# shgaurav1/DVG

Hardware: AMD Instinct MI355X
Metric: predicted frames/sec at 64x64, batch 64, 10-in/10-out (higher is better)
Workload: dtype f32; 1 GPU; Moving-MNIST 64x64 rollout (generate_frames.py make_gifs sample loop), vgg_64 + lstm + GP trigger sample at i%15==0, batch 64 per GPU, 10-in/10-out; model_family=vgg, batch_per_gpu=64, n_past=10, n_future=10, parallelism=replicas x1 (no data-path collective), launch=hipGraph replay, rollouts_in_flight=3, tile_policy=energy, loop_invariant_skip_halves=hoisted, upsample_conv3x3=as transposed 4x4/s2 conv, conv3x3_deep_layers=Winograd F(4x4,3x3) / F(2x2,3x3)

## Files before the change

dvg_amd/_lib.py:

```python
from __future__ import annotations

import ctypes as C
import os
import threading

_HERE = os.path.dirname(os.path.abspath(__file__))
LIB_PATH = os.environ.get("DVG_HIP_LIB") or os.path.join(_HERE, "csrc", "libdvg_hip.so")

_p = C.c_void_p
_i = C.c_int
_f = C.c_float
_d = C.c_double
_l = C.c_long

SIGNATURES = {
    "dvg_abi_version": (_i, []),
    "dvg_last_error": (C.c_char_p, []),
    "dvg_stream_capture_id": (_l, [_p]),
    "dvg_mfma_mode": (_i, []),
    "dvg_build_info": (C.c_char_p, []),
    "dvg_set_tile_policy": (None, [_i]),
    "dvg_tile_policy": (_i, []),
    "dvg_packed_row_floats": (_i, []),
    "dvg_pack_conv_weight": (_i, [_p, _p, _i, _i, _i, _i, _p]),
    "dvg_pack_convT_weight": (_i, [_p, _p, _i, _i, _i, _i, _p]),
    "dvg_unpack_conv_weight": (_i, [_p, _p, _i, _i, _i, _i, _p]),
    "dvg_unpack_convT_weight": (_i, [_p, _p, _i, _i, _i, _i, _p]),
    "dvg_conv_first_stats_rows": (_i, [_i, _i, _i, _i]),
    "dvg_pack_conv_weight_k16": (_i, [_p, _p, _i, _i, _i, _i, _i, _p]),
    "dvg_conv_splitk_v2": (_i, [_i, _i, _i, _i, _i, _i]),
    "dvg_conv_stats_rows_v2": (_i, [_i, _i, _i, _i, _i, _i, _i, _i]),
    "dvg_conv3x3_bn_act_v2": (_i, [_p, _p, _p, _p, _p, _p, _p, _p, _i, _i, _i, _i, _i, _i, _i, _i, _f, _p, _l, _p, _p, _i, _p]),
    "dvg_conv3x3_first_pair": (_i, [_p, _p, _p, _p, _p, _p, _p, _p, _p, _i, _i, _i, _i, _i, _f, _i, _p]),
    "dvg_conv4x4s2_bn_act_v2": (_i, [_p, _p, _p, _p, _p, _p, _i, _i, _i, _i, _i, _i, _f, _p, _l, _p]),
    "dvg_convT4x4s2_bn_act_v2": (_i, [_p, _p, _p, _p, _p, _p, _p, _i, _i, _i, _i, _i, _i, _i, _f, _p, _l, _p, _p, _i, _p]),
    "dvg_winograd_weight": (_i, [_p, _p, _i, _i, _i, _p]),
    "dvg_winograd_input": (_i, [_p, _p, _i, _i, _i, _i, _i, _i, _p]),
    "dvg_gemm_batched_k16": (_i, [_p, _p, _p, _i, _i, _i, _i, _i, _p]),
    "dvg_winograd_output": (_i, [_p, _p, _p, _p, _p, _i, _i, _i, _i, _i, _f, _i, _p, _i, _p]),
    "dvg_winograd_output_input": (_i, [_p, _p, _p, _p, _i, _i, _i, _i, _i, _f, _p, _p]),
    "dvg_stem_up_winograd_input": (_i, [_p, _i, _p, _i, _p, _p, _p, _i, _i, _i, _i, _f, _p]),
    "dvg_winograd_output_up_input": (_i, [_p, _p, _p, _p, _i, _i, _i, _i, _i, _f, _p]),
    "dvg_winograd_output_pool_input": (_i, [_p, _p, _p, _p, _p, _i, _i, _i, _i, _i, _f, _i, _p]),
    "dvg_conv3x3_first": (_i, [_p, _p, _p, _p, _p, _p, _i, _i, _i, _i, _i, _i, _f, _p]),
    "dvg_convT3x3_last": (_i, [_p, _p, _p, _p, _i, _i, _i, _i, _i, _i, _p]),
    "dvg_conv4x4s2_first": (_i, [_p, _p, _p, _p, _p, _p, _i, _i, _i, _i, _i, _i, _f, _p]),
    "dvg_convT4x4s2_last": (_i, [_p, _p, _p, _p, _p, _i, _i, _i, _i, _i, _i, _i, _p]),
    "dvg_moving_mnist_compose": (_i, [_p, _p, _p, _p, _i, _i, _i, _i, _i, _i, _p]),
    "dvg_clip_gather_u8": (_i, [_p, _p, _p, _l, _i, _i, _i, _i, _i, _i, _p]),
    "dvg_clip_gather_aug_u8": (_i, [_p, _p, _p, _p, _p, _l, _i, _i, _i, _i, _i, _i, _p]),
    "dvg_mnist_scale_u8": (_i, [_p, _p, _i, _i, _i, _p, _p, _p]),
    "dvg_moving_mnist_compose_u8": (_i, [_p, _p, _p, _p, _i, _i, _i, _i, _i, _i, _p]),
    "dvg_eval_frames": (_i, [_p, _p, _p, _p, _i, _i, _i, _p]),
    "dvg_eval_frames_finn": (_i, [_p, _p, _p, _p, _p, _i, _i, _i, _i, _p]),
    "dvg_pairwise_frame_mse": (_i, [_p, _p, _i, _l, _i, _l, _i, _p]),
    "dvg_frame_mosaic": (_i, [_p, _l, _p, _l, _p, _l, _i, _i, _i, _p] + [_i] * 9 + [_p, _i, _p, _i, _i, _p, _i, _i, _i, _i, _p, _p]),
    "dvg_adam_step": (_i, [_p, _p, _p, _p, _l, _f, _f, _f, _f, _f, _i, _p, _p]),
    "dvg_pixel_proj": (_i, [_p, _p, _p, _l, _i, _i, _p]),
    "dvg_convT_gather": (_i, [_p, _p, _p, _p, _i, _i, _i, _i, _i, _i, _p, _i, _p]),
    "dvg_channel_stats_rows": (_i, [_l]),
    "dvg_channel_stats": (_i, [_p, _p, _l, _i, _i, _p]),
    "dvg_bn_finalize": (_i, [_p, _i, _p, _p, _p, _p, _p, _p, _p, _p, _i, _d, _f, _f, _p, _i, _i, _p, _p]),
    "dvg_channel_stats_pivot": (_i, [_p, _p, _p, _l, _i, _i, _p]),
    "dvg_bn_finalize_pivot": (_i, [_p, _i, _p, _p, _p, _p, _p, _p, _p, _p, _p, _i, _d, _f, _f, _p, _i, _i, _p, _p]),
    "dvg_bn_running_update": (_i, [_p, _p, _i, _i, _f, _f, _f, _p, _p, _p, _i, _p]),
    "dvg_bn_act_apply": (_i, [_p, _p, _p, _p, _p, _i, _i, _i, _i, _i, _f, _i, _p]),
    "dvg_gemm_nt_bias_act": (_i, [_p, _p, _p, _p, _p, _p, _i, _i, _i, _i, _i, _i, _i, _i, _f, _i, _p]),
    "dvg_lstm_cell": (_i, [_p, _p, _p, _p, _p, _p, _p, _p, _p, _p, _i, _i, _p]),
    "dvg_lstm_cell_pre": (_i, [_p, _p, _p, _p, _p, _p, _p, _i, _i, _p]),
    "dvg_lstm_cell_bwd": (_i, [_p, _p, _p, _p, _p, _p, _p, _p, _p, _p, _i, _i, _p]),
    "dvg_lstm_cell_x": (_i, [_p, _i, _i, _p, _p, _p, _i, _p, _p, _p, _p, _i, _i, _p]),
    "dvg_gru_cell": (_i, [_p, _p, _p, _p, _p, _p, _p, _p, _i, _i, _p]),
    "dvg_gru_cell_pre": (_i, [_p, _p, _p, _p, _p, _p, _i, _i, _p]),
    "dvg_rnn_cell": (_i, [_p, _p, _p, _p, _p, _p, _p, _i, _i, _p]),
    "dvg_gru_gates_bwd": (_i, [_p, _p, _p, _p, _p, _p, _p, _i, _i, _p]),
    "dvg_stem_gemm": (_i, [_p, _i, _p, _i, _p, _p, _p, _i, _i, _i, _i, _i, _i, _f, _p]),
    "dvg_gp_precision": (_i, [_i, _i, _i]),
    "dvg_gp_bwd_precision": (_i, [_i, _i]),
    "dvg_gp_lds_bytes": (C.c_size_t, [_i, _i, _i]),
    "dvg_gp_predict": (_i, [_p] * 14 + [_i, _i, _i, _i, _f, _i, _i, _p]),
    "dvg_gp_step_group": (_i, [_i, _i, _i, _i]),
    "dvg_gp_bwd_lds_bytes": (C.c_size_t, [_i, _i]),
    "dvg_gp_bwd_chunk": (_i, [_i, _i]),
    "dvg_gemm_tn": (_i, [_p] * 5 + [_i] * 8 + [_p]),
    "dvg_gp_train_bwd": (_i, [_p] * 17 + [_i, _i, _i, _f, _i, _i, _p]),
    "dvg_sum_steps_multi": (_i, [_p, _p, _p, _i, _i, _p]),
    "dvg_gp_elbo": (_i, [_p, _p, _p, _p, _l, _l, _p, _p, _i, _i, _i, _i, _p]),
    "dvg_gp_elbo_bwd": (_i, [_p, _p, _p, _p, _l, _l, _p, _p, _p, _p, _p, _p, _p, _i, _i, _i, _i, _p]),
    "dvg_bn_act_bwd_rows": (_i, [_i, _i, _i, _i]),
    "dvg_bn_act_bwd_reduce": (_i, [_p, _p, _p, _p, _p, _p, _i, _i, _i, _i, _i, _f, _i, _p]),
    "dvg_bn_bwd_finalize": (_i, [_p, _i, _p, _p, _p, _p, _p, _p, _p, _p, _p, _i, _d, _i, _i, _i, _p]),
    "dvg_bn_act_bwd_reduce_centered": (_i, [_p, _p, _p, _p, _p, _p, _p, _i, _i, _i, _i, _i, _f, _i, _p]),
    "dvg_bn_bwd_finalize_centered": (_i, [_p, _i, _p, _p, _p, _p, _p, _p, _p, _p, _p, _i, _d, _i, _i, _i, _p]),
    "dvg_affine3_apply": (_i, [_p, _p, _p, _p, _p, _p, _l, _i, _p, _i, _i, _p]),
    "dvg_act_bwd": (_i, [_p, _p, _p, _l, _i, _f, _p]),
    "dvg_upsample2x_bwd": (_i, [_p, _p, _i, _i, _i, _i, _p]),
    "dvg_group_sum": (_i, [_p, _p, _p, _i, _i, _l, _p]),
    "dvg_colsum": (_i, [_p, _p, _i, _i, _i, _p]),
    "dvg_wgrad_finish": (_i, [_p, _i, _p, _i, _i, _i, _i, _i, _i, _i, _f, _p]),
    "dvg_k4_to_w3": (_i, [_p, _p, _i, _i, _i, _i, _f, _p]),
    "dvg_reduce_partials": (_i, [_p, _p, _i, _l, _p]),
    "dvg_conv_wgrad_splits": (_i, [_i, _i, _i, _i, _i, _i]),
    "dvg_conv_wgrad": (_i, [_i, _p, _p, _p, _p, _i, _i, _i, _i, _i, _i, _i, _p]),
    "dvg_conv_wgrad_splits_multi": (_i, [_i, _i, _i, _i, _i, _i, _i]),
    "dvg_conv_wgrad_multi": (_i, [_i, _i, _p, _p, _p, _p, _i, _i, _i, _i, _i, _i, _i, _p]),
    "dvg_winograd_wgrad_operands": (_i, [_p, _p, _p, _p, _i, _i, _i, _i, _i, _l, _l, _p]),
    "dvg_winograd_wgrad_splits": (_i, [_l, _i, _i]),
    "dvg_winograd_wgrad_gemm": (_i, [_p, _p, _p, _l, _i, _i, _p]),
    "dvg_winograd_wgrad_gemm_items": (_i, [_p, _p, _i, _l, _p, _i, _i, _p]),
    "dvg_winograd_wgrad_reduce": (_i, [_p, _i, _p, _i, _i, _p]),
    "dvg_wgrad_thin_rows": (_i, [_i, _i, _i, _i]),
    "dvg_wgrad_thin": (_i, [_p, _p, _p, _i, _i, _i, _i, _i, _i, _p]),
    "dvg_lstm_gates_bwd": (_i, [_p, _p, _p, _p, _p, _p, _p, _i, _i, _p]),
    "dvg_nchw_to_nhwc": (_i, [_p, _p, _i, _i, _i, _i, _p]),
    "dvg_nhwc_to_nchw": (_i, [_p, _p, _i, _i, _i, _i, _p]),
    "dvg_zero_tick": (_i, [_p, _l, _p, _p, _p, _p, _p]),
    "dvg_grad_sumsq_blocks": (_i, [_l]),
    "dvg_grad_sumsq": (_i, [_p, _l, _p, _p]),
    "dvg_grad_guard_finish": (_i, [_p, _i, _d, _i, _p, _p, _p]),
    "dvg_adam_step_guarded": (_i, [_p, _p, _p, _p, _l, _f, _f, _f, _f, _f, _i, _p, _p, _p, _p]),
    "dvg_ema_update_blocks": (_i, [_l]),
    "dvg_ema_update": (_i, [_p, _p, _l, _d, _p, _p, _p]),
    "dvg_lr_schedule_tick": (_i, [_i, _i, _i, _i, _d, _d, _p, _p, _p]),
    "dvg_adam_step_scheduled": (_i, [_p, _p, _p, _p, _l, _f, _f, _f, _f, _f, _i, _p, _p, _p, _p, _p]),
    "dvg_val_accumulate": (_i, [_p, _p, _p, _i, _i, _i, _p, _p, _p, _p]),
    "dvg_frame_losses_blocks": (_i, [_l]),
    "dvg_frame_losses": (_i, [_p, _p, _p, _p, _l, _i, _i, _p, _p, _p]),
    "dvg_mse_sum_grad": (_i, [_p, _p, _p, _p, _l, _f, _p]),
    "dvg_frame_losses_ext_blocks": (_i, [_i, _l, _i, _i]),
    "dvg_frame_losses_ext": (_i, [_p, _p, _p, _p, _i, _i, _l, _i, _i, _i, _f, _p, _p, _p, _p]),
    "dvg_gp_var_norms": (_i, [_p, _p, _i, _i, _p]),
    "dvg_gp_trigger_step": (_i, [_p, _i, _i, _i, _p, _i, _f, _p, _p, _p, _p, _i, _p]),
    "dvg_gp_trigger_replay": (_i, [_p, _i, _p, _i, _f, _p, _p, _p]),
    "dvg_gp_trigger_select": (_i, [_p, _p, _p, _p, _i, _i, _i, _l, _p, _p, _p, _p]),
    "dvg_debug_set_clockbuf": (None, [_p, C.c_uint]),
    "dvg_debug_set_gp_clockbuf": (None, [_p, C.c_uint]),
    "dvg_debug_set_wgrad_clockbuf": (None, [_p, C.c_uint]),
}

_lock = threading.Lock()
_lib = None


class DvgLibraryError(RuntimeError):
    pass


def lib() -> C.CDLL:
    global _lib
    if _lib is not None:
        return _lib
    with _lock:
        if _lib is not None:
            return _lib
        if not os.path.exists(LIB_PATH):
            raise DvgLibraryError(
                f"{LIB_PATH} not found: the HIP kernel library has not been built. "
                "Run `python -c 'import __graft_entry__ as g; g.build()'` (or `make -C dvg_amd/csrc`). "
                "There is no CPU/eager fallback for the DVG hot path.")
        try:
            import torch
            if torch.cuda.is_available():
                torch.cuda.init()
        except ImportError:
            pass
        try:
            handle = C.CDLL(LIB_PATH)
        except OSError as e:
            raise DvgLibraryError(f"cannot load {LIB_PATH}: {e}") from e
        for name, (res, args) in SIGNATURES.items():
            try:
                fn = getattr(handle, name)
            except AttributeError as e:
                raise DvgLibraryError(f"{LIB_PATH} lacks symbol {name}; rebuild it") from e
            fn.restype = res
            fn.argtypes = args
        _lib = handle
        return _lib


def build_info() -> dict:
    raw = lib().dvg_build_info().decode()
    d = {}
    for tok in raw.split():
        k, _, v = tok.partition("=")
        d[k] = int(v) if v.lstrip("-").isdigit() else v
    d["raw"] = raw
    d["path"] = LIB_PATH
    d["from_env"] = bool(os.environ.get("DVG_HIP_LIB"))
    shipped = {os.path.join(_HERE, "csrc", "libdvg_hip.so"), os.path.join(_HERE, "csrc", "libdvg_hip_f32mfma.so")}
    d["product"] = os.path.abspath(LIB_PATH) in shipped and d.get("variant", "") == ""
    return d


def check(code: int, what: str = "") -> None:
    if code != 0:
        msg = lib().dvg_last_error()
        raise RuntimeError(f"libdvg_hip {what} failed (code {code}): {msg.decode() if msg else '?'}")
```

dvg_amd/csrc/conv_igemm2.hip:

```cpp
#include <cstdlib>
#include <type_traits>

#include "dvg_common.h"

namespace dvg {

constexpr int DVG_GEMM_WGS_PER_CU = DVG_BF16X3 ? 3 : 4;
constexpr int DVG_GEMM128_WGS = DVG_BF16X3 ? 3 : 2;
constexpr int DVG_GEMM128_GT = DVG_BF16X3 ? 2 : 4;
constexpr int DVG_GEMM_GT = 4;
constexpr int DVG_GEMM128_MIN_WGS = 4 * 768;
[[maybe_unused]] constexpr int DVG_GEMM_NT2 = 256;
constexpr int DVG_TILE16_MIN_WGS = 256;

enum { M2_CONV3 = 0, M2_CONV4S2 = 1, M2_CONVT4S2 = 2, M2_GEMM = 3 };

struct Igemm2Params {
    const float* x;
    const float* skip;
    const float* w;
    const float* scale;
    const float* shift;
    float* y;
    float* y_pool;
    float* stats;
    int N, H, W, C1, C2, Cout, upsample, act;
    float slope;
    int tiles_y, tiles_x, tiles_n, nblk_n;
    int splitk;
    int cps;
    float* ws;
    const float* addend;
    unsigned long long* clk;
    unsigned clk_cap;
    int nb_group;
    int stage_prio;
    long w_image_stride;
    int gemm_ni;
    const int* add_map;
    int add_B;
    const float* first_frame;
    const float* first_w;
    const float* first_scale;
    const float* first_shift;
    float first_slope;
    int y_from;
};

__device__ __forceinline__ int addend_image(const int* __restrict__ add_map, int add_B, int n) {
    return add_map ? add_map[n / add_B] * add_B + n % add_B : n;
}

static unsigned long long* g_clk = nullptr;
static unsigned g_clk_cap = 0;

__device__ __attribute__((aligned(16))) float dvg_zero_slot[4] = {0.f, 0.f, 0.f, 0.f};

template <int MODE, int TI, int TH, int TW, int NT_ = 1, bool FIRST_ = false>
struct Cfg2 {
    static constexpr int NT = NT_;
    static constexpr bool FIRST = FIRST_;
    static constexpr bool GEMM = MODE == M2_GEMM;
    static constexpr int S = (MODE == M2_CONV4S2) ? 2 : 1;
    static constexpr bool PAR4 = MODE == M2_CONV4S2;
    static constexpr int SPAN = GEMM ? 1 : (PAR4 ? 2 : 3);
    static constexpr int HH = (TH - 1) + SPAN, HW = (TW - 1) + SPAN;
    static constexpr bool LAYOUT = !GEMM;
    static constexpr int HWP = !LAYOUT ? HW : (TW == 16 ? HW : (TW == 8 ? 12 : 6));
    static constexpr int IMG = (LAYOUT && TI == 4) ? (PAR4 ? 30 : 40) : HH * HWP;
    static_assert(IMG >= HH * HWP && HWP >= HW, "halo layout");
    static constexpr int HP = TI * IMG;
    static constexpr unsigned P0PACK = !LAYOUT ? 0x6420u
        : (PAR4 ? (TW == 16 ? 0x3650u : (TI == 4 ? 0x7430u : 0x6530u))
                : (TW == 16 ? 0x2640u : (TI == 4 ? 0x6530u : 0x4620u)));
    static constexpr int PK = !LAYOUT ? 1 : (PAR4 ? (TW == 16 ? 4 : 1) : (TW == 16 ? 5 : (TI == 4 ? 1 : 3)));
    static constexpr bool STORE_PERM = LAYOUT && DVG_BF16X3 != 0;
    static constexpr int hp_of(int slot) {
        return STORE_PERM ? ((slot & ~7) | (((slot & 3) << 1) | ((slot >> 2) & 1))) : slot;
    }
    static constexpr int row_c(int reg) { return 4 * (int)((P0PACK >> (4 * (reg >> 2))) & 15u) + (reg & 3); }
    static constexpr int BM = TI * TH * TW, MT = BM / 64, BN = 64 * NT;
    static constexpr int NTAPS = GEMM ? 1 : ((MODE == M2_CONV3) ? 9 : 16);
    static constexpr int GT = (MODE == M2_CONV3) ? 9 : (MODE == M2_CONV4S2 ? 4 : (GEMM ? (NT == 2 ? 2 : (BM == 128 ? DVG_GEMM128_GT : DVG_GEMM_GT)) : 4));
    static constexpr int NG = (MODE == M2_CONV4S2) ? 16 / GT : 1;
    static constexpr int CHUNKS_PER_STAGE = GEMM ? GT : 1;
    static constexpr bool X3 = DVG_BF16X3 != 0;
    static constexpr int KC = 16, LD = X3 ? (GEMM ? 24 : 28) : 20, LDB = X3 ? 24 : 20, WROW = DVG_WROW;
    static constexpr int NP = X3 ? 3 : 2, PSTEP = X3 ? 8 : 4;
    static constexpr int BLK4 = GT * 64 * WROW / 4;
    static constexpr int B_TILE4 = NT * BLK4;
    static constexpr int NLB = (B_TILE4 + 255) / 256;
    static_assert(NT == 1 || (DVG_BF16X3 != 0 && MODE == M2_GEMM && BLK4 % 256 == 0), "NT = 2: bf16-triple GEMM mode only");
    static constexpr int NLA1 = (HP * 4 + 255) / 256;
    static constexpr int NLA = NLA1 * (GEMM ? GT : 1);
    static constexpr int SLAB = NLA1 * 64 * LD;
    static constexpr int A_FLOATS = NLA * 64 * LD, B_FLOATS = GT * BN * LDB;
    static constexpr int FP_W = HW + 2, FP_FLOATS = (HH + 2) * FP_W, FIRST_FLOATS = FIRST ? FP_FLOATS : 0;
    static_assert(!FIRST || (MODE == M2_CONV3 && TI == 1 && NT == 1), "FIRST: 3x3 mode, one image per tile");
    static constexpr int LDS_BYTES = (A_FLOATS + B_FLOATS + FIRST_FLOATS) * 4;
    static constexpr bool CAN_SPLIT = !FIRST && !GEMM && TW != 16;
    static_assert(BM == 64 || BM == 128 || BM == 256, "BM");
};

template <int MODE, int TI, int TH, int TW, int NT = 1, bool FIRST = false>
__global__ __launch_bounds__(256, (MODE == M2_GEMM && TW == 8) ? DVG_GEMM_WGS_PER_CU : ((MODE == M2_GEMM && NT == 1) ? DVG_GEMM128_WGS : 2)) void conv_igemm2_kernel(const Igemm2Params p) {
    using C = Cfg2<MODE, TI, TH, TW, NT, FIRST>;
    constexpr int S = C::S, HH = C::HH, HW = C::HW, HP = C::HP, LD = C::LD, MT = C::MT, GT = C::GT, NG = C::NG,
                  BN = C::BN, NLA = C::NLA, NLA1 = C::NLA1, LDB = C::LDB, NP = C::NP, PSTEP = C::PSTEP, NLB = C::NLB;
    constexpr bool GEMM = C::GEMM, X3 = C::X3;
    extern __shared__ __attribute__((aligned(16))) float smem[];
    float* As = smem;
    float* Bs = smem + C::A_FLOATS;

    const int tid = threadIdx.x, lane = tid & 63, wave = tid >> 6;
    const int wm = wave >> 1, wn = wave & 1, l31 = lane & 31, hh = lane >> 5;

    unsigned lid = xcd_remap(blockIdx.x, gridDim.x);
    int par = 0;
    if (MODE == M2_CONVT4S2) { par = lid & 3; lid >>= 2; }
    const int split = lid % p.splitk;
    lid /= p.splitk;
    const int tiles_total = p.tiles_x * p.tiles_y * p.tiles_n;
    const unsigned lr = lid / p.nb_group;
    const int nb = (int)(lr / tiles_total) * p.nb_group + (int)(lid % p.nb_group);
    const unsigned tile_id = lr % tiles_total;
    unsigned t = tile_id;
    const int tx_i = t % p.tiles_x; t /= p.tiles_x;
    const int ty_i = t % p.tiles_y; t /= p.tiles_y;
    const int n0 = (int)t * (MODE == M2_GEMM ? p.gemm_ni : TI), y0 = ty_i * TH, x0 = tx_i * TW;
    const int yin0 = y0 * S - (GEMM ? 0 : 1), xin0 = x0 * S - (GEMM ? 0 : 1), nb0 = nb * BN;
    const float* const wbase = p.w + (GEMM ? (size_t)n0 * p.w_image_stride : 0);
    const int py = par >> 1, px = par & 1;
    const int Cin = p.C1 + p.C2;

    int a_base[MT];
#pragma unroll
    for (int mt = 0; mt < MT; ++mt) {
        const int lp = 4 * ((int)((C::P0PACK >> (4 * (l31 >> 3))) & 15u) ^ (((l31 >> 2) & 1) * C::PK)) + (l31 & 3);
        const int m = wm * (C::BM / 2) + mt * 32 + lp;
        const int ti = m / (TH * TW), r = m % (TH * TW);
        const int pos = ti * C::IMG + (r / TW) * C::HWP + r % TW;
        a_base[mt] = pos * LD + (X3 ? (hh ^ (GEMM ? (pos >> 3) & 1 : 0)) * 4 : hh * 8);
    }
    int b_base[NT];
#pragma unroll
    for (int nt = 0; nt < NT; ++nt) {
        const int col = (wn * NT + nt) * 32 + l31;
        b_base[nt] = ((col >> 6) * GT * 64 + (col & 63)) * LDB + (X3 ? (hh ^ ((l31 >> 3) & 1)) * 4 : hh * 8);
    }

    f32x16 acc[MT * NT];
#pragma unroll
    for (int mt = 0; mt < MT * NT; ++mt)
#pragma unroll
        for (int i = 0; i < 16; ++i) acc[mt][i] = 0.f;

    constexpr int NOFF = GEMM ? NLA1 : NLA;
    using aoff_t = typename std::conditional<GEMM || C::PAR4, int, long>::type;
    auto opaque = [](unsigned v) { asm("" : "+v"(v)); return v; };
    aoff_t offx[NOFF], offs[GEMM ? 1 : NLA];
    unsigned okmask = 0;
    static_assert(!C::PAR4 || NLA <= 4, "PAR4: four validity bits and two step bits per halo slot in one word");
    if (GEMM) offs[0] = 0;
#pragma unroll
    for (int i = 0; i < NLA; ++i) {
        const int idx = tid + (i % NLA1) * 256;
        const int hp = C::hp_of(idx >> 2), q = idx & 3;
        const int ti = hp / C::IMG, r = hp % C::IMG;
        const int hy = r / C::HWP, hx = r % C::HWP;
        const bool slot = hp < HP && hy < HH && hx < HW;
        if constexpr (C::PAR4) {
            const int n = n0 + ti, yy = yin0 + 2 * hy, xx = xin0 + 2 * hx;
            const bool in = slot && n < p.N;
#pragma unroll
            for (int par_ = 0; par_ < 4; ++par_) {
                const bool ok = in && (unsigned)(yy + (par_ >> 1)) < (unsigned)p.H && (unsigned)(xx + (par_ & 1)) < (unsigned)p.W;
                okmask |= ok ? (1u << (par_ * NLA + i)) : 0u;
            }
            const int cy0 = min(max(yy, 0), p.H - 1), cy1 = min(max(yy + 1, 0), p.H - 1);
            const int cx0 = min(max(xx, 0), p.W - 1), cx1 = min(max(xx + 1, 0), p.W - 1);
            okmask |= (in && cy1 != cy0) ? (1u << (16 + i)) : 0u;
            okmask |= (in && cx1 != cx0) ? (1u << (24 + i)) : 0u;
            offx[i] = in ? (int)((((long)n * p.H + cy0) * p.W + cx0) * p.C1 + q * 4) : 0;
            offs[i] = 0;
        } else {
        const int n = n0 + ti, yy = yin0 + hy, xx = xin0 + hx;
        const bool ok = slot && n < p.N && (unsigned)yy < (unsigned)p.H && (unsigned)xx < (unsigned)p.W;
        const int sh = p.upsample;
        okmask |= ok ? (1u << i) : 0u;
        if (!GEMM || i < NLA1)
            offx[GEMM ? i % NLA1 : i] = (aoff_t)(ok ? ((((long)(GEMM ? 0 : n) * (p.H >> sh) + (yy >> sh)) * (p.W >> sh) + (xx >> sh)) * p.C1 + q * 4) : 0);
        if (!GEMM) offs[i] = (ok && p.C2) ? ((((long)n * p.H + yy) * p.W + xx) * p.C2 + q * 4) : 0;
        }
    }
    auto tap_lds = [&](int grp, int tt) -> int {
        if (GEMM) return tt * C::SLAB;
        int th, tw;
        if (MODE == M2_CONV3) { th = tt / 3; tw = tt % 3; }
        else if (MODE == M2_CONV4S2) { th = tt >> 1; tw = tt & 1; }
        else { th = 1 + py - (tt >> 1); tw = 1 + px - (tt & 1); }
        return (th * C::HWP + tw) * LD;
    };
    long ld_a_off = GEMM ? (long)n0 * p.H * p.W * p.C1 : 0;
    const float* ld_w = wbase;
    float* const Fp = smem + C::A_FLOATS + C::B_FLOATS;
    f32x4 fw[FIRST ? 11 : 1];
    auto first_tile = [&](f32x4 (&ra)[NLA]) {
        if constexpr (FIRST) {
#pragma unroll
            for (int i = 0; i < NLA; ++i) {
                const int hp = min(C::hp_of((tid + i * 256) >> 2), HP - 1);
                const float* f = Fp + (hp / C::HWP) * C::FP_W + hp % C::HWP;
                f32x4 v = {0.f, 0.f, 0.f, 0.f};
#pragma unroll
                for (int t = 0; t < 9; ++t) {
                    const float px = f[(t / 3) * C::FP_W + t % 3];
#pragma unroll
                    for (int e = 0; e < 4; ++e) v[e] = fmaf(fw[t][e], px, v[e]);
                }
                const float okf = (float)((okmask >> i) & 1u);
#pragma unroll
                for (int e = 0; e < 4; ++e) {
                    const float a = v[e] * fw[9][e] + fw[10][e];
                    v[e] = fmaxf(a, a * p.first_slope) * okf;
                }
                ra[i] = v;
            }
        }
    };
    auto gload_a = [&](int c0, f32x4 (&ra)[NLA], const int par_ = 0) {
        if constexpr (FIRST) {
            const float* w = p.first_w + c0 + (tid & 3) * 4;
#pragma unroll
            for (int t = 0; t < 9; ++t) fw[t] = *reinterpret_cast<const f32x4*>(w + t * 64);
            fw[9] = *reinterpret_cast<const f32x4*>(p.first_scale + c0 + (tid & 3) * 4);
            fw[10] = *reinterpret_cast<const f32x4*>(p.first_shift + c0 + (tid & 3) * 4);
            return;
        }
        const bool from_x = GEMM || c0 < p.C1;
        const float* src = (from_x ? p.x + c0 : p.skip + (c0 - p.C1)) + (GEMM ? ld_a_off : 0);
#pragma unroll
        for (int i = 0; i < NLA; ++i) {
            if (GEMM) {
                ra[i] = *reinterpret_cast<const f32x4*>(src + offx[i % NLA1] + (i / NLA1) * 16);
            } else if (C::PAR4) {
                int off = offx[i];
                if (par_ >> 1) off += (int)opaque((okmask >> (16 + i)) & 1u) * (p.W * p.C1);
                if (par_ & 1) off += (int)opaque((okmask >> (24 + i)) & 1u) * p.C1;
                ra[i] = *reinterpret_cast<const f32x4*>(src + off);
            } else {
                const float* a = src + (from_x ? offx[GEMM ? 0 : i] : offs[GEMM ? 0 : i]);
                ra[i] = *reinterpret_cast<const f32x4*>(((okmask >> i) & 1u) ? a : dvg_zero_slot);
            }
        }
    };
    auto gload_b = [&](int chunk, int grp, f32x4 (&rb)[NLB]) {
        const float* tile;
        if (GEMM) tile = ld_w + ((size_t)nb * NT * (Cin / C::KC) + chunk) * (64 * C::WROW);
        else tile = wbase + (((size_t)chunk * (p.Cout >> 6) + nb) * C::NTAPS + (MODE == M2_CONVT4S2 ? par * 4 : grp * GT)) * (64 * C::WROW);
#pragma unroll
        for (int j = 0; j < NLB; ++j) {
            int i = tid + j * 256;
            if (C::B_TILE4 % 256) i = min(i, C::B_TILE4 - 1);
            const size_t blk = (NT > 1 && j * 256 >= C::BLK4) ? (size_t)(Cin / C::KC) * (64 * C::WROW / 4) - C::BLK4 : 0;
            rb[j] = reinterpret_cast<const f32x4*>(tile)[i + blk];
        }
    };
    auto lds_store_a = [&](f32x4 (&ra)[NLA], const int par_ = 0) {
        if constexpr (FIRST) first_tile(ra);
#pragma unroll
        for (int i = 0; i < NLA; ++i) {
            const int idx = tid + (i % NLA1) * 256;
            const int hp = C::hp_of(idx >> 2), q = idx & 3;
            if constexpr (C::PAR4) {
                const unsigned keep = 0u - opaque((okmask >> (par_ * NLA + i)) & 1u);
#pragma unroll
                for (int e = 0; e < 4; ++e) {
                    const float f = ra[i][e];
                    ra[i][e] = __builtin_bit_cast(float, __builtin_bit_cast(unsigned, f) & keep);
                }
            }
            if constexpr (X3) {
                u32x2_t h, m, l;
                unsigned t0, t1, t2;
                bf16x3_split_pair(ra[i][0], ra[i][1], t0, t1, t2);
                h[0] = t0; m[0] = t1; l[0] = t2;
                bf16x3_split_pair(ra[i][2], ra[i][3], t0, t1, t2);
                h[1] = t0; m[1] = t1; l[1] = t2;
                float* d = &As[(i / NLA1) * C::SLAB + hp * LD + ((q >> 1) ^ (GEMM ? (hp >> 3) & 1 : 0)) * 4 + (q & 1) * 2];
                *reinterpret_cast<u32x2_t*>(d) = h;
                *reinterpret_cast<u32x2_t*>(d + 8) = m;
                *reinterpret_cast<u32x2_t*>(d + 16) = l;
            } else {
                *reinterpret_cast<f32x4*>(&As[(i / NLA1) * C::SLAB + hp * LD + q * 4]) = ra[i];
            }
        }
    };
    auto lds_store_b = [&](const f32x4 (&rb)[NLB]) {
#pragma unroll
        for (int j = 0; j < NLB; ++j) {
            int i = tid + j * 256;
            if (C::B_TILE4 % 256) i = min(i, C::B_TILE4 - 1);
            if constexpr (X3) reinterpret_cast<f32x4*>(Bs)[i] = rb[j];
            else *reinterpret_cast<f32x4*>(&Bs[(i >> 2) * LDB + (i & 3) * 4]) = rb[j];
        }
    };

    constexpr int CPS = C::CHUNKS_PER_STAGE;
    const int chunk_begin = split * p.cps;
    const int chunk_end = min(Cin / C::KC, chunk_begin + p.cps);
    f32x4 ra[NLA], rb[NLB];
    unsigned long long clk0 = 0, wclk0 = 0;
    if (p.clk) {
        clk0 = clock64();
        wclk0 = wall_clock64();
    }
    if constexpr (FIRST) {
        const float* fr = p.first_frame + (size_t)n0 * p.H * p.W;
        for (int i = tid; i < C::FP_FLOATS; i += 256) {
            const int yy = yin0 - 1 + i / C::FP_W, xx = xin0 - 1 + i % C::FP_W;
            Fp[i] = ((unsigned)yy < (unsigned)p.H && (unsigned)xx < (unsigned)p.W) ? fr[(size_t)yy * p.W + xx] : 0.f;
        }
        __syncthreads();
    }
    gload_a(chunk_begin * C::KC, ra);
    gload_b(chunk_begin, 0, rb);
    lds_store_a(ra);
    lds_store_b(rb);
    __syncthreads();
    unsigned long long clk1 = 0;
    if (p.clk) clk1 = clock64();

    auto stage = [&](const int chunk, auto grp_c, auto has_next_c, const int nchunk_override = -1) __attribute__((always_inline)) {
        constexpr int grp = decltype(grp_c)::value;
        constexpr bool has_next = decltype(has_next_c)::value;
        constexpr int ngrp = (grp + 1) % NG;
        constexpr bool next_a = has_next && (ngrp == 0 || C::PAR4);
        const int nchunk = nchunk_override >= 0 ? nchunk_override : chunk + (ngrp == 0 ? CPS : 0);
        if constexpr (next_a) gload_a(nchunk * C::KC, ra, C::PAR4 ? ngrp : 0);
        if constexpr (has_next) gload_b(nchunk, ngrp, rb);

        f32x4 fa[2][MT][NP], fb[2][NT][NP];
        {
            const int ao = tap_lds(grp, 0);
#pragma unroll
            for (int j = 0; j < NP; ++j) {
#pragma unroll
                for (int mt = 0; mt < MT; ++mt)
                    fa[0][mt][j] = *reinterpret_cast<const f32x4*>(&As[a_base[mt] + ao + j * PSTEP]);
#pragma unroll
                for (int nt = 0; nt < NT; ++nt)
                    fb[0][nt][j] = *reinterpret_cast<const f32x4*>(&Bs[b_base[nt] + j * PSTEP]);
            }
        }
#pragma unroll
        for (int tt = 0; tt < GT; ++tt) {
            const int cur = tt & 1, nxt = cur ^ 1;
            constexpr bool LEAN = X3 && (NT == 2 || (GEMM && MT == 2));
            auto read_plane = [&](int j) {
                const int ao = tap_lds(grp, tt + 1);
#pragma unroll
                for (int mt = 0; mt < MT; ++mt)
                    fa[nxt][mt][j] = *reinterpret_cast<const f32x4*>(&As[a_base[mt] + ao + j * PSTEP]);
#pragma unroll
                for (int nt = 0; nt < NT; ++nt)
                    fb[nxt][nt][j] = *reinterpret_cast<const f32x4*>(&Bs[b_base[nt] + (tt + 1) * 64 * LDB + j * PSTEP]);
            };
            if (LEAN && tt + 1 < GT) read_plane(0);
            if (!LEAN && tt + 1 < GT) {
                const int ao = tap_lds(grp, tt + 1);
#pragma unroll
                for (int j = 0; j < NP; ++j) {
#pragma unroll
                    for (int mt = 0; mt < MT; ++mt)
                        fa[nxt][mt][j] = *reinterpret_cast<const f32x4*>(&As[a_base[mt] + ao + j * PSTEP]);
#pragma unroll
                    for (int nt = 0; nt < NT; ++nt)
                        fb[nxt][nt][j] = *reinterpret_cast<const f32x4*>(&Bs[b_base[nt] + (tt + 1) * 64 * LDB + j * PSTEP]);
                }
            }
            if (has_next && tt == GT - 1) {
                __syncthreads();
                if constexpr (next_a) lds_store_a(ra, C::PAR4 ? ngrp : 0);
                lds_store_b(rb);
            }
            if constexpr (X3) {
                auto mm = [&](int pa, int pb) {
#pragma unroll
                    for (int mt = 0; mt < MT; ++mt)
#pragma unroll
                        for (int nt = 0; nt < NT; ++nt)
                            acc[mt * NT + nt] = __builtin_amdgcn_mfma_f32_32x32x16_bf16(
                                __builtin_bit_cast(bf16x8_t, fa[cur][mt][pa]), __builtin_bit_cast(bf16x8_t, fb[cur][nt][pb]),
                                acc[mt * NT + nt], 0, 0, 0);
                };
                if constexpr (LEAN) {
                    mm(2, 0);
                    mm(0, 2);
                    if (tt + 1 < GT) read_plane(2);
                    mm(1, 1);
                    mm(1, 0);
                    mm(0, 1);
                    if (tt + 1 < GT) read_plane(1);
                    mm(0, 0);
                } else {
                    mm(2, 0);
                    mm(1, 1);
                    mm(0, 2);
                    mm(1, 0);
                    mm(0, 1);
                    mm(0, 0);
                }
            } else {
#pragma unroll
                for (int j = 0; j < 2; ++j)
#pragma unroll
                    for (int e = 0; e < 4; ++e)
#pragma unroll
                        for (int mt = 0; mt < MT; ++mt)
                            acc[mt] = __builtin_amdgcn_mfma_f32_32x32x2f32(fa[cur][mt][j][e], fb[cur][0][j][e], acc[mt], 0, 0, 0);
            }
            constexpr int NREAD = NP * (MT + NT), NMFMA = (X3 ? 6 : 8) * MT * NT, MPR = NMFMA >= 2 * NREAD ? 2 : 1;
            constexpr int NVMEM = (next_a ? (FIRST ? 11 : NLA) : 0) + (has_next ? NLB : 0);
            constexpr int VT0 = GT >= 9 ? 2 : 0;
            constexpr int SLOTS = (GT - 1 - VT0) > 0 ? (GT - 1 - VT0) : 1;
            constexpr int VNEED = (NVMEM + SLOTS - 1) / SLOTS;
            constexpr int VPT = VNEED > 2 ? VNEED : 2;
            constexpr int VTAPS = (NVMEM + VPT - 1) / VPT;
            if (tt == 0) __builtin_amdgcn_sched_group_barrier(0x100, NREAD, 0);
            if (LEAN && tt + 1 < GT) {
                constexpr int G = MT * NT, R = MT + NT;
#pragma unroll
                for (int r = 0; r < R; ++r) {
                    __builtin_amdgcn_sched_group_barrier(0x100, 1, 0);
                    __builtin_amdgcn_sched_group_barrier(0x008, 1, 0);
                }
                __builtin_amdgcn_sched_group_barrier(0x008, 2 * G - R, 0);
#pragma unroll
                for (int r = 0; r < R; ++r) {
                    __builtin_amdgcn_sched_group_barrier(0x100, 1, 0);
                    __builtin_amdgcn_sched_group_barrier(0x008, 1, 0);
                }
                __builtin_amdgcn_sched_group_barrier(0x008, 3 * G - R, 0);
#pragma unroll
                for (int r = 0; r < R; ++r) {
                    __builtin_amdgcn_sched_group_barrier(0x100, 1, 0);
                    __builtin_amdgcn_sched_group_barrier(0x008, 1, 0);
                }
            } else if (tt + 1 < GT) {
#pragma unroll
                for (int r = 0; r < NREAD; ++r) {
                    __builtin_amdgcn_sched_group_barrier(0x100, 1, 0);
                    __builtin_amdgcn_sched_group_barrier(0x008, MPR, 0);
                }
                if (NMFMA > MPR * NREAD) __builtin_amdgcn_sched_group_barrier(0x008, NMFMA - MPR * NREAD, 0);
            } else if (has_next) {
                constexpr int NW = (next_a ? NLA * (X3 ? 3 : 1) : 0) + NLB;
#pragma unroll
                for (int r = 0; r < NW; ++r) {
                    if (r < NMFMA) __builtin_amdgcn_sched_group_barrier(0x008, 1, 0);
                    __builtin_amdgcn_sched_group_barrier(0x200, 1, 0);
                }
                if (NMFMA > NW) __builtin_amdgcn_sched_group_barrier(0x008, NMFMA - NW, 0);
            } else {
                __builtin_amdgcn_sched_group_barrier(0x008, NMFMA, 0);
            }
            if (tt >= VT0 && tt < VT0 + VTAPS && tt + 1 < GT) __builtin_amdgcn_sched_group_barrier(0x020, VPT, 0);
        }

        if constexpr (has_next) __syncthreads();
    };
    using std::integral_constant;
    const bool prio_on = p.stage_prio != 0;
    auto set_prio = [&](int st) {
        if (!prio_on) return;
        switch (st & 3) {
            case 0: __builtin_amdgcn_s_setprio(3); break;
            case 1: __builtin_amdgcn_s_setprio(2); break;
            case 2: __builtin_amdgcn_s_setprio(1); break;
            default: __builtin_amdgcn_s_setprio(0); break;
        }
    };
    int chunk = chunk_begin, st = 0;
    if constexpr (GEMM) {
        const int spi = (chunk_end - chunk_begin) / CPS;
        const long a_img = (long)p.H * p.W * p.C1;
        const unsigned lane_off = (unsigned)(4 * hh * p.Cout + l31);
        float* const ybase = p.y + (size_t)n0 * p.H * p.W * p.Cout + nb0 + __builtin_amdgcn_readfirstlane(wn) * 32 * NT;
        const int wm_u = __builtin_amdgcn_readfirstlane(wm);
        for (int img = 0; img < p.gemm_ni; ++img) {
            for (int sg = 0; sg < spi; ++sg) {
                const bool wrap = sg == spi - 1, last = wrap && img == p.gemm_ni - 1;
                ld_a_off = (long)(n0 + img + (wrap ? 1 : 0)) * a_img;
                ld_w = wbase + (size_t)(img + (wrap ? 1 : 0)) * p.w_image_stride;
                const int nchunk = wrap ? chunk_begin : chunk_begin + (sg + 1) * CPS;
                set_prio(st++);
                if (last) stage(chunk_begin + sg * CPS, integral_constant<int, 0>{}, integral_constant<bool, false>{});
                else stage(chunk_begin + sg * CPS, integral_constant<int, 0>{}, integral_constant<bool, true>{}, nchunk);
            }
            float* const yb = ybase + (size_t)img * p.H * p.W * p.Cout;
#pragma unroll
            for (int mt = 0; mt < MT; ++mt) {
                const int mbase = wm_u * (C::BM / 2) + mt * 32;
#pragma unroll
                for (int nt = 0; nt < NT; ++nt)
#pragma unroll
                    for (int reg = 0; reg < 16; ++reg) {
                        const int mu = mbase + (reg & 3) + 8 * (reg >> 2);
                        float* const dst = (yb + (size_t)((y0 + mu / TW) * p.W + x0 + mu % TW) * p.Cout + nt * 32) + lane_off;
                        *dst = acc[mt * NT + nt][reg];
                        acc[mt * NT + nt][reg] = 0.f;
                    }
            }
        }
    } else {
    auto chunk_stages = [&](const int ch, auto last_c) __attribute__((always_inline)) {
        constexpr bool last = decltype(last_c)::value;
        set_prio(st++);
        stage(ch, integral_constant<int, 0>{}, integral_constant<bool, !(last && NG == 1)>{});
        if constexpr (NG >= 2) {
            set_prio(st++);
            stage(ch, integral_constant<int, 1>{}, integral_constant<bool, !(last && NG == 2)>{});
        }
        if constexpr (NG >= 4) {
            set_prio(st++);
            stage(ch, integral_constant<int, 2>{}, integral_constant<bool, true>{});
            set_prio(st++);
            stage(ch, integral_constant<int, 3>{}, integral_constant<bool, !last>{});
        }
        static_assert(NG == 1 || NG == 2 || NG == 4, "stages per chunk");
    };
    for (; chunk + CPS < chunk_end; chunk += CPS) chunk_stages(chunk, integral_constant<bool, false>{});
    chunk_stages(chunk, integral_constant<bool, true>{});
    }
    __builtin_amdgcn_s_setprio(0);
    unsigned long long clk_loop = 0;
    if (p.clk) clk_loop = clock64();
    auto clk_exit = [&]() {
        if (p.clk && threadIdx.x == 0 && blockIdx.x < p.clk_cap) {
            unsigned long long* d = p.clk + (size_t)blockIdx.x * 8;
            d[0] = clk0; d[1] = clk1; d[2] = clk_loop; d[3] = clock64(); d[4] = wclk0; d[5] = wall_clock64();
            unsigned xcc;
            asm volatile("s_getreg_b32 %0, hwreg(HW_REG_XCC_ID)" : "=s"(xcc));
            unsigned hwid;
            asm volatile("s_getreg_b32 %0, hwreg(HW_REG_HW_ID)" : "=s"(hwid));
            d[6] = xcc; d[7] = hwid;
        }
    };

    if constexpr (GEMM) {
        clk_exit();
        return;
    }
    int Ho, Wo;
    if (MODE == M2_CONV3 || MODE == M2_GEMM) { Ho = p.H; Wo = p.W; }
    else if (MODE == M2_CONV4S2) { Ho = p.H >> 1; Wo = p.W >> 1; }
    else { Ho = p.H * 2; Wo = p.W * 2; }
    const int c = nb0 + wn * 32 + l31;
    if (C::CAN_SPLIT && p.splitk > 1) {
        const size_t slab = (size_t)p.N * Ho * Wo * p.Cout;
        float* const wsp = p.ws + (size_t)split * slab;
#pragma unroll
        for (int mt = 0; mt < MT; ++mt)
#pragma unroll
            for (int reg = 0; reg < 16; ++reg) {
                const int m = wm * (C::BM / 2) + mt * 32 + (C::row_c(reg) ^ (hh * 4 * C::PK));
                const int tii = m / (TH * TW), r = m % (TH * TW);
                const int ty = r / TW, tx = r % TW;
                const int n = n0 + tii;
                int oy, ox;
                if (MODE == M2_CONVT4S2) { oy = 2 * (y0 + ty) + py; ox = 2 * (x0 + tx) + px; }
                else { oy = y0 + ty; ox = x0 + tx; }
                if (n < p.N) wsp[(((size_t)n * Ho + oy) * Wo + ox) * p.Cout + c] = acc[mt][reg];
            }
        clk_exit();
        return;
    }
    const float sc = p.scale ? p.scale[c] : 1.f, sf = p.shift ? p.shift[c] : 0.f;
    float s1 = 0.f, s2 = 0.f;
    float* const yb = p.y + (size_t)n0 * Ho * Wo * p.Cout + c;
    const bool want_y = !FIRST || n0 >= p.y_from;
    float* const pb = p.y_pool ? p.y_pool + (size_t)n0 * (Ho >> 1) * (Wo >> 1) * p.Cout + c : nullptr;
    const float* const ab = p.addend ? p.addend + (size_t)n0 * Ho * Wo * p.Cout + c : nullptr;
    long add_shift[TI];
#pragma unroll
    for (int t_ = 0; t_ < TI; ++t_) {
        const int n_ = min(n0 + t_, p.N - 1);
        add_shift[t_] = (ab != nullptr && p.add_map != nullptr)
                            ? (long)(addend_image(p.add_map, p.add_B, n_) - n_) * Ho * Wo * p.Cout : 0;
    }
    auto shift_of = [&](int tii) -> long {
        if (TI == 1) return add_shift[0];
        long v = add_shift[0];
#pragma unroll
        for (int t_ = 1; t_ < TI; ++t_) v = tii == t_ ? add_shift[t_] : v;
        return v;
    };
    const int hrow = hh * 4 * C::PK;
    auto epilogue = [&](auto act_c) {
        constexpr int ACT = decltype(act_c)::value;
#pragma unroll
        for (int mt = 0; mt < MT; ++mt) {
            float v[16];
            const int mbase = wm * (C::BM / 2) + mt * 32;
            const int ti0 = mbase / (TH * TW);
            if (ab != nullptr) {
                float av[16];
#pragma unroll
                for (int reg = 0; reg < 16; ++reg) {
                    const int m = mbase + (C::row_c(reg) ^ hrow);
                    const int tii = (TH * TW >= 32) ? ti0 : m / (TH * TW);
                    const int r = m % (TH * TW);
                    const int ty = r / TW, tx = r % TW;
                    int oy, ox;
                    if (MODE == M2_CONVT4S2) { oy = 2 * (y0 + ty) + py; ox = 2 * (x0 + tx) + px; }
                    else { oy = y0 + ty; ox = x0 + tx; }
                    av[reg] = (TI == 1 || n0 + tii < p.N) ? ab[(long)((tii * Ho + oy) * Wo + ox) * p.Cout + shift_of(tii)] : 0.f;
                }
#pragma unroll
                for (int reg = 0; reg < 16; ++reg) v[reg] = (acc[mt][reg] + av[reg]) * sc + sf;
            } else {
#pragma unroll
                for (int reg = 0; reg < 16; ++reg) v[reg] = acc[mt][reg] * sc + sf;
            }
#pragma unroll
            for (int reg = 0; reg < 16; ++reg) {
                const int row = C::row_c(reg) ^ hrow;
                const int m = mbase + row;
                const int tii = (TH * TW >= 32) ? ti0 : m / (TH * TW);
                const int r = m % (TH * TW);
                const int ty = r / TW, tx = r % TW;
                if (TI == 1 || n0 + tii < p.N) {
                    s1 += v[reg];
                    s2 += v[reg] * v[reg];
                    float o;
                    if constexpr (ACT == DVG_ACT_LRELU) o = v[reg] > 0.f ? v[reg] : v[reg] * p.slope;
                    else if constexpr (ACT == DVG_ACT_NONE) o = v[reg];
                    else o = apply_act(v[reg], p.act, p.slope);
                    v[reg] = o;
                    int oy, ox;
                    if (MODE == M2_CONVT4S2) { oy = 2 * (y0 + ty) + py; ox = 2 * (x0 + tx) + px; }
                    else { oy = y0 + ty; ox = x0 + tx; }
                    if (!FIRST || want_y) yb[((tii * Ho + oy) * Wo + ox) * p.Cout] = o;
                }
            }
            if (MODE == M2_CONV3 && (TW == 16 || TW == 8)) {
                if (pb != nullptr) {
                    constexpr int RY = (TW == 16 && !C::LAYOUT) ? 8 : 4;
#pragma unroll
                    for (int reg = 0; reg < 16; ++reg) {
                        const bool ty_even = (TW == 16 && !C::LAYOUT) ? ((reg >> 2) < 2) : (((reg >> 2) & 1) == 0);
                        if ((reg & 1) == 0 && ty_even) {
                            const int row = C::row_c(reg) ^ hrow;
                            const int r = (mbase + row) % (TH * TW);
                            const int ty = r / TW, tx = r % TW;
                            const float mx = fmaxf(fmaxf(v[reg], v[reg + 1]), fmaxf(v[reg + RY], v[reg + RY + 1]));
                            if (TI == 1 || n0 + ti0 < p.N)
                                pb[((ti0 * (Ho >> 1) + ((y0 + ty) >> 1)) * (Wo >> 1) + ((x0 + tx) >> 1)) * p.Cout] = mx;
                        }
                    }
                }
            }
        }
    };
    if (p.act == DVG_ACT_LRELU) epilogue(std::integral_constant<int, DVG_ACT_LRELU>{});
    else if (p.act == DVG_ACT_NONE) epilogue(std::integral_constant<int, DVG_ACT_NONE>{});
    else epilogue(std::integral_constant<int, -1>{});
    if (p.stats != nullptr) {
        float* red = smem;
        s1 += __shfl_xor(s1, 32);
        s2 += __shfl_xor(s2, 32);
        __syncthreads();
        if (wm == 1 && hh == 0) {
            red[wn * 64 + l31] = s1;
            red[wn * 64 + 32 + l31] = s2;
        }
        __syncthreads();
        if (wm == 0 && hh == 0) {
            const unsigned rowid = (MODE == M2_CONVT4S2 ? tile_id * 4 + par : tile_id);
            float* dst = p.stats + (size_t)rowid * 2 * p.Cout;
            dst[c] = s1 + red[wn * 64 + l31];
            dst[p.Cout + c] = s2 + red[wn * 64 + 32 + l31];
        }
    }
    clk_exit();
}

template <bool POOL>
__global__ __launch_bounds__(256) void splitk_finish_kernel(const float* __restrict__ ws, int S,
                                                            const float* __restrict__ scale,
                                                            const float* __restrict__ shift, float* __restrict__ y,
                                                            float* __restrict__ y_pool, float* __restrict__ stats, int N,
                                                            int H, int W, int C, int act, float slope,
                                                            int units_per_block, const float* __restrict__ addend,
                                                            const int* __restrict__ add_map, int add_B) {
    __shared__ float red[2 * 256 * 4];
    const int C4 = C >> 2;
    const int TC = C4 < 256 ? C4 : 256, TP = 256 / TC;
    const int tc = threadIdx.x % TC, tp = threadIdx.x / TC;
    const int Hu = POOL ? H >> 1 : H, Wu = POOL ? W >> 1 : W;
    const long units = (long)N * Hu * Wu, slab4 = (long)N * H * W * C4;
    const long u0 = (long)blockIdx.x * units_per_block, u1 = min(units, u0 + units_per_block);
    const int c4 = tc;
    const f32x4 sc = scale ? *reinterpret_cast<const f32x4*>(scale + c4 * 4) : f32x4{1.f, 1.f, 1.f, 1.f};
    const f32x4 sf = shift ? *reinterpret_cast<const f32x4*>(shift + c4 * 4) : f32x4{0.f, 0.f, 0.f, 0.f};
    f32x4 s1 = {0.f, 0.f, 0.f, 0.f}, s2 = {0.f, 0.f, 0.f, 0.f};
    for (long w_ = u0 + tp; w_ < u1; w_ += TP) {
        f32x4 mx;
#pragma unroll
        for (int q = 0; q < (POOL ? 4 : 1); ++q) {
            size_t off;
            if (POOL) {
                const int xp = w_ % Wu;
                long r = w_ / Wu;
                const int yp = r % Hu;
                const int n = r / Hu;
                off = (((size_t)n * H + 2 * yp + (q >> 1)) * W + 2 * xp + (q & 1)) * C4 + c4;
            } else {
                off = (size_t)w_ * C4 + c4;
            }
            f32x4 v = reinterpret_cast<const f32x4*>(ws)[off];
            {
                int s = 1;
                for (; s + 3 <= S; s += 3) {
                    f32x4 t[3];
#pragma unroll
                    for (int u = 0; u < 3; ++u) t[u] = reinterpret_cast<const f32x4*>(ws)[(size_t)(s + u) * slab4 + off];
#pragma unroll
                    for (int u = 0; u < 3; ++u)
#pragma unroll
                        for (int k = 0; k < 4; ++k) v[k] += t[u][k];
                }
                for (; s < S; ++s) {
                    const f32x4 t = reinterpret_cast<const f32x4*>(ws)[(size_t)s * slab4 + off];
#pragma unroll
                    for (int k = 0; k < 4; ++k) v[k] += t[k];
                }
            }
            if (addend != nullptr) {
                size_t aoff = off;
                if (add_map != nullptr) {
                    const long img4 = (long)H * W * C4;
                    const int n_ = (int)(off / img4);
                    aoff = off - (size_t)(n_ - addend_image(add_map, add_B, n_)) * img4;
                }
                const f32x4 t = reinterpret_cast<const f32x4*>(addend)[aoff];
#pragma unroll
                for (int k = 0; k < 4; ++k) v[k] += t[k];
            }
#pragma unroll
            for (int k = 0; k < 4; ++k) {
                const float u = v[k] * sc[k] + sf[k];
                s1[k] += u;
                s2[k] = fmaf(u, u, s2[k]);
                v[k] = apply_act(u, act, slope);
            }
            reinterpret_cast<f32x4*>(y)[off] = v;
            if (POOL) {
                if (q == 0) mx = v;
                else
#pragma unroll
                    for (int k = 0; k < 4; ++k) mx[k] = fmaxf(mx[k], v[k]);
            }
        }
        if (POOL) reinterpret_cast<f32x4*>(y_pool)[w_ * C4 + c4] = mx;
    }
    if (stats != nullptr) {
#pragma unroll
        for (int k = 0; k < 4; ++k) {
            red[(tp * TC + tc) * 4 + k] = s1[k];
            red[1024 + (tp * TC + tc) * 4 + k] = s2[k];
        }
        __syncthreads();
        if (tp == 0) {
            float* dst = stats + (size_t)blockIdx.x * 2 * C;
#pragma unroll
            for (int k = 0; k < 4; ++k) {
                float a = 0.f, b = 0.f;
                for (int r = 0; r < TP; ++r) {
                    a += red[(r * TC + tc) * 4 + k];
                    b += red[1024 + (r * TC + tc) * 4 + k];
                }
                dst[c4 * 4 + k] = a;
                dst[C + c4 * 4 + k] = b;
            }
        }
    }
}

static int finish_units_per_block(long units) {
    long upb = (units + 1023) / 1024;
    if (upb < 8) upb = 8;
    return (int)upb;
}

static int g_tile_policy = 0;
extern "C" void dvg_set_tile_policy(int energy) { g_tile_policy = energy ? 1 : 0; }
extern "C" int dvg_tile_policy(void) { return g_tile_policy; }

static int choose_splitk(long wgs, int nchunks) {
    if (wgs >= 384 || nchunks < 8) return 1;
    long s = 512 / wgs;
    if (s > 8) s = 8;
    if (s > nchunks / 4) s = nchunks / 4;
    return s < 2 ? 1 : (int)s;
}

template <int MODE, int TI, int TH, int TW, int NT = 1, bool FIRST = false>
static int launch2(Igemm2Params p, int Hg, int Wg, float* ws, long ws_floats, hipStream_t stream) {
    using C = Cfg2<MODE, TI, TH, TW, NT, FIRST>;
    if (Hg % TH || Wg % TW || p.Cout % C::BN) return fail(DVG_ERR_SHAPE, "conv_igemm2: tile does not divide shape");
    p.tiles_y = Hg / TH;
    p.tiles_x = Wg / TW;
    p.tiles_n = (p.N + TI - 1) / TI;
    if (MODE == M2_GEMM) {
        int ni = 1;
#if DVG_BF16X3
        if (TW == 8 && NT == 1) {
            const long w1 = (long)p.tiles_y * p.tiles_x * p.N * (p.Cout / C::BN), slots = 256L * DVG_GEMM_WGS_PER_CU;
            if (w1 % slots == 0 && w1 / slots >= 2 && w1 / slots <= 6 && p.N % (w1 / slots) == 0) ni = (int)(w1 / slots);
        }
#endif
        p.gemm_ni = ni;
        p.tiles_n = p.N / ni;
    }
    p.nblk_n = p.Cout / C::BN;
    p.clk = g_clk;
    p.clk_cap = g_clk_cap;
    const long wgs = (long)p.tiles_y * p.tiles_x * p.tiles_n * p.nblk_n * (MODE == M2_CONVT4S2 ? 4 : 1);
    {
        const long tiles = (long)p.tiles_y * p.tiles_x * p.tiles_n;
        const double per_xcd = (double)tiles * p.nblk_n / 8.0;
        const double wb = (double)C::NTAPS * (p.C1 + p.C2) * C::BN * 4, ib = (double)C::BM * (p.C1 + p.C2) * 4;
        int best = p.nblk_n;
        double cost = 1e300;
        for (int a = 1; a <= p.nblk_n; ++a) {
            if (p.nblk_n % a) continue;
            const double share_tiles = per_xcd / a;
            if (share_tiles > (double)tiles) continue;
            const double c = a * wb + (share_tiles < 1.0 ? 1.0 : share_tiles) * ib;
            if (c < cost) { cost = c; best = a; }
        }
        p.nb_group = best;
    }
    const int nchunks = (p.C1 + p.C2) / C::KC;
    int Ho, Wo;
    if (MODE == M2_CONV3 || MODE == M2_GEMM) { Ho = p.H; Wo = p.W; }
    else if (MODE == M2_CONV4S2) { Ho = p.H >> 1; Wo = p.W >> 1; }
    else { Ho = p.H * 2; Wo = p.W * 2; }
    const long out_floats = (long)p.N * Ho * Wo * p.Cout;
    int S = (ws != nullptr && C::CAN_SPLIT) ? choose_splitk(wgs, nchunks) : 1;
    if (S > 1 && (long)S * out_floats > ws_floats) return fail(DVG_ERR_SHAPE, "conv_igemm2: split-K workspace too small");
    p.cps = (nchunks + S - 1) / S;
    p.cps = (p.cps + C::CHUNKS_PER_STAGE - 1) / C::CHUNKS_PER_STAGE * C::CHUNKS_PER_STAGE;
    S = (nchunks + p.cps - 1) / p.cps;
    p.splitk = S;
    p.ws = ws;
    float* y_pool = p.y_pool;
    float* stats = p.stats;
    const unsigned grid = (unsigned)(wgs * S);
    p.stage_prio = (MODE == M2_CONV3 || grid <= 3 * 256) ? 1 : 0;
    static bool attr_set = false;
    if (!attr_set) {
        hipError_t e = hipFuncSetAttribute(reinterpret_cast<const void*>(&conv_igemm2_kernel<MODE, TI, TH, TW, NT, FIRST>),
                                           hipFuncAttributeMaxDynamicSharedMemorySize, C::LDS_BYTES);
        if (e != hipSuccess) return fail(DVG_ERR_HIP, "hipFuncSetAttribute: %s", hipGetErrorString(e));
        attr_set = true;
    }
    hipLaunchKernelGGL((conv_igemm2_kernel<MODE, TI, TH, TW, NT, FIRST>), dim3(grid), dim3(256), C::LDS_BYTES, stream, p);
    if (int e = check_launch("conv_igemm2")) return e;
    if (S > 1) {
        const bool pool = y_pool != nullptr;
        const long units = pool ? (long)p.N * (Ho / 2) * (Wo / 2) : (long)p.N * Ho * Wo;
        const int upb = finish_units_per_block(units);
        const unsigned fgrid = (unsigned)((units + upb - 1) / upb);
        if (pool)
            hipLaunchKernelGGL((splitk_finish_kernel<true>), dim3(fgrid), dim3(256), 0, stream, ws, S, p.scale, p.shift, p.y,
                               y_pool, stats, p.N, Ho, Wo, p.Cout, p.act, p.slope, upb, p.addend, p.add_map, p.add_B);
        else
            hipLaunchKernelGGL((splitk_finish_kernel<false>), dim3(fgrid), dim3(256), 0, stream, ws, S, p.scale, p.shift, p.y,
                               y_pool, stats, p.N, Ho, Wo, p.Cout, p.act, p.slope, upb, p.addend, p.add_map, p.add_B);
        return check_launch("splitk_finish");
    }
    return DVG_OK;
}


static int tile2(int mode, int N, int Hg, int Wg, int Cout, int* ti, int* th, int* tw) {
    const int par = mode == M2_CONVT4S2 ? 4 : 1;
    if (Hg == 4 && Wg == 4) { *ti = 4; *th = 4; *tw = 4; return 0; }
    if (Hg % 8 || Wg % 8) return -1;
    *ti = 1; *th = 8; *tw = 8;
    if (Wg % 16 == 0) {
        const long wgs = (long)N * (Hg / 8) * (Wg / 16) * (Cout / 64) * par;
        if (wgs >= (g_tile_policy ? DVG_TILE16_MIN_WGS : 512)) *tw = 16;
        if (mode == M2_GEMM && *tw == 16) {
            if (!DVG_BF16X3 || wgs < DVG_GEMM128_MIN_WGS) *tw = 8;
        }
    }
    return 0;
}

__global__ void pack_k16_kernel(const float* __restrict__ src, float* __restrict__ dst, int cout, int cin, int kh,
                                int kw, int transposed) {
    const long total = (long)cout * cin * kh * kw / 2;
    const int nblk = cout >> 6, taps = kh * kw;
    for (long i = blockIdx.x * (long)blockDim.x + threadIdx.x; i < total; i += (long)gridDim.x * blockDim.x) {
        const int k = (int)(i & 7) * 2;
        long r = i >> 3;
        const int co = r % cout; r /= cout;
        const int t = r % taps;
        const int chunk = r / taps;
        const int ci = chunk * 16 + k, a = t / kw, b = t % kw;
        const long j = transposed ? ((((long)ci * cout + co) * kh + (kh - 1 - a)) * kw + (kw - 1 - b))
                                  : ((((long)co * cin + ci) * kh + a) * kw + b);
        const long j1 = j + (transposed ? (long)cout * kh * kw : (long)kh * kw);
        int slot = t;
        if (transposed && kh == 4 && kw == 4) {
            const int py = a & 1, px = b & 1;
            slot = (py * 2 + px) * 4 + ((2 + py - a) >> 1) * 2 + ((2 + px - b) >> 1);
        } else if (kh == 4 && kw == 4) {
            slot = ((a & 1) * 2 + (b & 1)) * 4 + (a >> 1) * 2 + (b >> 1);
        }
        wrow_store_pair(dst, (((size_t)chunk * nblk + (co >> 6)) * taps + slot) * 64 + (co & 63), co & 63, k, src[j], src[j1]);
    }
    wrow_drain();
}

}

using namespace dvg;

extern "C" int dvg_mfma_mode(void) { return DVG_BF16X3 ? 1 : 0; }
extern "C" int dvg_packed_row_floats(void) { return DVG_WROW; }

extern "C" void dvg_debug_set_clockbuf(void* buf, unsigned records) {
    g_clk = (unsigned long long*)buf;
    g_clk_cap = buf ? records : 0;
}

extern "C" int dvg_pack_conv_weight_k16(const float* w, float* w_packed, int cout, int cin, int kh, int kw,
                                        int transposed, void* stream) {
    DVG_REQUIRE(w && w_packed, DVG_ERR_NULL, "dvg_pack_conv_weight_k16: NULL pointer");
    DVG_REQUIRE(cout > 0 && cout % 64 == 0 && cin > 0 && cin % 16 == 0 && kh > 0 && kw > 0, DVG_ERR_SHAPE,
                "dvg_pack_conv_weight_k16: Cin must be a multiple of 16, Cout of 64");
    const long total = (long)cout * cin * kh * kw / 2;
    long g = (total + 255) / 256;
    if (g > 4096) g = 4096;
    hipLaunchKernelGGL(pack_k16_kernel, dim3((unsigned)g), dim3(256), 0, (hipStream_t)stream, w, w_packed, cout, cin, kh,
                       kw, transposed);
    return check_launch("dvg_pack_conv_weight_k16");
}

static long v2_wgs(int mode, int N, int Hg, int Wg, int Cout, int ti, int th, int tw) {
    return (long)((N + ti - 1) / ti) * (Hg / th) * (Wg / tw) * (Cout / 64) * (mode == M2_CONVT4S2 ? 4 : 1);
}

static int v2_splits(int mode, int N, int Hg, int Wg, int Cout, int Cin, int ti, int th, int tw) {
    if (tw == 16) return 1;
    return choose_splitk(v2_wgs(mode, N, Hg, Wg, Cout, ti, th, tw), Cin / 16);
}

extern "C" int dvg_conv_splitk_v2(int mode, int N, int H, int W, int Cin, int Cout) {
    int Hg = H, Wg = W;
    if (mode == M2_CONV4S2) { Hg = H / 2; Wg = W / 2; }
    int ti, th, tw;
    if (Cin % 16 || Cout % 64 || tile2(mode, N, Hg, Wg, Cout, &ti, &th, &tw)) return -1;
    return v2_splits(mode, N, Hg, Wg, Cout, Cin, ti, th, tw);
}

extern "C" int dvg_conv_stats_rows_v2(int mode, int N, int H, int W, int Cin, int Cout, int pool, int with_workspace) {
    int Hg = H, Wg = W;
    if (mode == M2_CONV4S2) { Hg = H / 2; Wg = W / 2; }
    int ti, th, tw;
    if (tile2(mode, N, Hg, Wg, Cout, &ti, &th, &tw)) return -1;
    if (with_workspace && v2_splits(mode, N, Hg, Wg, Cout, Cin, ti, th, tw) > 1) {
        int Ho = H, Wo = W;
        if (mode == M2_CONV4S2) { Ho = H / 2; Wo = W / 2; }
        if (mode == M2_CONVT4S2) { Ho = 2 * H; Wo = 2 * W; }
        const long units = pool ? (long)N * (Ho / 2) * (Wo / 2) : (long)N * Ho * Wo;
        const int upb = finish_units_per_block(units);
        return (int)((units + upb - 1) / upb);
    }
    return ((N + ti - 1) / ti) * (Hg / th) * (Wg / tw) * (mode == M2_CONVT4S2 ? 4 : 1);
}

static int checks2(const Igemm2Params& p, const char* who) {
    DVG_REQUIRE(p.x && p.w && p.y, DVG_ERR_NULL, "%s: x/w/y must not be NULL", who);
    DVG_REQUIRE((p.skip != nullptr) == (p.C2 > 0), DVG_ERR_SHAPE, "%s: skip pointer / C2 mismatch", who);
    DVG_REQUIRE(p.N > 0 && p.H > 0 && p.W > 0, DVG_ERR_SHAPE, "%s: empty shape", who);
    DVG_REQUIRE(p.C1 > 0 && p.C1 % 16 == 0 && p.C2 % 16 == 0, DVG_ERR_SHAPE, "%s: C1=%d C2=%d must be multiples of 16",
                who, p.C1, p.C2);
    DVG_REQUIRE(p.Cout > 0 && p.Cout % 64 == 0, DVG_ERR_SHAPE, "%s: Cout=%d must be a multiple of 64", who, p.Cout);
    DVG_REQUIRE(aligned16(p.x) && aligned16(p.w) && aligned16(p.y) && aligned16(p.skip), DVG_ERR_ALIGN,
                "%s: pointers must be 16-byte aligned", who);
    DVG_REQUIRE(p.act >= DVG_ACT_NONE && p.act <= DVG_ACT_SIGMOID, DVG_ERR_SHAPE, "%s: bad act", who);
    return DVG_OK;
}

#define D2(MODE, TI_, TH_, TW_) \
    if (ti == TI_ && th == TH_ && tw == TW_)                                             \
        return launch2<MODE, TI_, TH_, TW_>(p, Hg, Wg, workspace, workspace_floats, (hipStream_t)stream);



extern "C" int dvg_conv3x3_bn_act_v2(const float* x, const float* skip, const float* w_k16, const float* scale,
                                     const float* shift, float* y, float* y_pool, float* stats, int N, int H, int W,
                                     int C1, int C2, int Cout, int upsample_x, int act, float slope,
                                     float* workspace, long workspace_floats, const float* addend,
                                     const int* addend_map, int addend_block, void* stream) {
    Igemm2Params p{x, skip, w_k16, scale, shift, y, y_pool, stats, N, H, W, C1, C2, Cout, upsample_x ? 1 : 0, act, slope,
                   0, 0, 0, 0, 0, 1, 0, nullptr};
    p.addend = addend;
    p.add_map = addend ? addend_map : nullptr;
    p.add_B = addend_block;
    DVG_REQUIRE(p.add_map == nullptr || (addend_block > 0 && N % addend_block == 0), DVG_ERR_SHAPE,
                "dvg_conv3x3_bn_act_v2: addend_block must divide N");
    if (int e = checks2(p, "dvg_conv3x3_bn_act_v2")) return e;
    DVG_REQUIRE(aligned16(addend) && (addend == nullptr || y_pool == nullptr), DVG_ERR_SHAPE,
                "dvg_conv3x3_bn_act_v2: addend must be 16-byte aligned and excludes the pooled output");
    DVG_REQUIRE(H % 8 == 0 && W % 8 == 0, DVG_ERR_SHAPE, "dvg_conv3x3_bn_act_v2: H=%d W=%d must be multiples of 8", H, W);
    int Hg = H, Wg = W, ti, th, tw;
    DVG_REQUIRE(tile2(M2_CONV3, N, Hg, Wg, Cout, &ti, &th, &tw) == 0 && ti == 1, DVG_ERR_SHAPE,
                "dvg_conv3x3_bn_act_v2: no tile for %dx%d", H, W);
    D2(M2_CONV3, 1, 8, 16)
    D2(M2_CONV3, 1, 8, 8)
    return fail(DVG_ERR_SHAPE, "dvg_conv3x3_bn_act_v2: no kernel");
}

extern "C" int dvg_conv3x3_first_pair(const float* frame, const float* w0, const float* scale0, const float* shift0,
                                      const float* w1_k16, const float* scale1, const float* shift1, float* y, float* y_pool,
                                      int N, int H, int W, int Cout, int act, float slope, int y_from, void* stream) {
    DVG_REQUIRE(frame && w0 && scale0 && shift0, DVG_ERR_NULL, "dvg_conv3x3_first_pair: NULL pointer");
    DVG_REQUIRE(y_from >= 0 && y_from <= N && (y_from == 0 || y_pool != nullptr) && (y != nullptr || y_from == N), DVG_ERR_SHAPE,
                "dvg_conv3x3_first_pair: y_from=%d needs 0 <= y_from <= N, a pooled output when > 0, y unless == N", y_from);
    float* const y_biased = y ? y - (size_t)y_from * H * W * Cout : y_pool;
    Igemm2Params p{frame , nullptr, w1_k16, scale1, shift1, y_biased, y_pool, nullptr, N, H, W, 64, 0, Cout, 0,
                   act, slope, 0, 0, 0, 0, 0, 1, 0, nullptr};
    p.first_frame = frame; p.first_w = w0; p.first_scale = scale0; p.first_shift = shift0; p.first_slope = 0.2f;
    p.y_from = y_from;
    if (int e = checks2(p, "dvg_conv3x3_first_pair")) return e;
    DVG_REQUIRE(H % 8 == 0 && W % 16 == 0 && (long)N * (H / 8) * (W / 16) * (Cout / 64) >= 512, DVG_ERR_SHAPE,
                "dvg_conv3x3_first_pair: H %% 8, W %% 16 and >= 512 workgroups needed (N=%d H=%d W=%d Cout=%d)", N, H, W, Cout);
    return launch2<M2_CONV3, 1, 8, 16, 1, true>(p, H, W, nullptr, 0, (hipStream_t)stream);
}

extern "C" int dvg_conv4x4s2_bn_act_v2(const float* x, const float* w_k16, const float* scale, const float* shift,
                                       float* y, float* stats, int N, int H, int W, int Cin, int Cout, int act,
                                       float slope, float* workspace, long workspace_floats, void* stream) {
    Igemm2Params p{x, nullptr, w_k16, scale, shift, y, nullptr, stats, N, H, W, Cin, 0, Cout, 0, act, slope, 0, 0, 0, 0, 0,
                   1, 0, nullptr};
    if (int e = checks2(p, "dvg_conv4x4s2_bn_act_v2")) return e;
    DVG_REQUIRE(H % 2 == 0 && W % 2 == 0, DVG_ERR_SHAPE, "dvg_conv4x4s2_bn_act_v2: odd input");
    DVG_REQUIRE((long)N * H * W * Cin < (1L << 31), DVG_ERR_SHAPE,
                "dvg_conv4x4s2_bn_act_v2: input of %d x %d x %d x %d floats too large (32-bit offsets)", N, H, W, Cin);
    int Hg = H / 2, Wg = W / 2, ti, th, tw;
    DVG_REQUIRE(tile2(M2_CONV4S2, N, Hg, Wg, Cout, &ti, &th, &tw) == 0, DVG_ERR_SHAPE,
                "dvg_conv4x4s2_bn_act_v2: unsupported map %dx%d", H, W);
    D2(M2_CONV4S2, 1, 8, 16)
    D2(M2_CONV4S2, 1, 8, 8)
    D2(M2_CONV4S2, 4, 4, 4)
    return fail(DVG_ERR_SHAPE, "dvg_conv4x4s2_bn_act_v2: no kernel");
}

extern "C" int dvg_convT4x4s2_bn_act_v2(const float* x, const float* skip, const float* w_k16, const float* scale,
                                        const float* shift, float* y, float* stats, int N, int H, int W, int C1,
                                        int C2, int Cout, int act, float slope, float* workspace, long workspace_floats,
                                        const float* addend, const int* addend_map, int addend_block, void* stream) {
    Igemm2Params p{x, skip, w_k16, scale, shift, y, nullptr, stats, N, H, W, C1, C2, Cout, 0, act, slope, 0, 0, 0, 0, 0,
                   1, 0, nullptr};
    p.addend = addend;
    p.add_map = addend ? addend_map : nullptr;
    p.add_B = addend_block;
    DVG_REQUIRE(p.add_map == nullptr || (addend_block > 0 && N % addend_block == 0), DVG_ERR_SHAPE,
                "dvg_convT4x4s2_bn_act_v2: addend_block must divide N");
    if (int e = checks2(p, "dvg_convT4x4s2_bn_act_v2")) return e;
    DVG_REQUIRE(aligned16(addend), DVG_ERR_ALIGN, "dvg_convT4x4s2_bn_act_v2: addend must be 16-byte aligned");
    int Hg = H, Wg = W, ti, th, tw;
    DVG_REQUIRE(tile2(M2_CONVT4S2, N, Hg, Wg, Cout, &ti, &th, &tw) == 0, DVG_ERR_SHAPE,
                "dvg_convT4x4s2_bn_act_v2: unsupported map %dx%d", H, W);
    D2(M2_CONVT4S2, 1, 8, 16)
    D2(M2_CONVT4S2, 1, 8, 8)
    D2(M2_CONVT4S2, 4, 4, 4)
    return fail(DVG_ERR_SHAPE, "dvg_convT4x4s2_bn_act_v2: no kernel");
}

extern "C" int dvg_gemm_batched_k16(const float* x, const float* w_k16, float* y, int NB, int H, int W, int Cin, int Cout,
                                    void* stream) {
    Igemm2Params p{x, nullptr, w_k16, nullptr, nullptr, y, nullptr, nullptr, NB, H, W, Cin, 0, Cout, 0, DVG_ACT_NONE, 0.f,
                   0, 0, 0, 0, 0, 1, 0, nullptr};
    if (int e = checks2(p, "dvg_gemm_batched_k16")) return e;
    DVG_REQUIRE(Cin % (16 * DVG_GEMM_GT) == 0 && H % 8 == 0 && W % 8 == 0, DVG_ERR_SHAPE,
                "dvg_gemm_batched_k16: Cin=%d must be a multiple of %d, H=%d W=%d multiples of 8", Cin, 16 * DVG_GEMM_GT, H, W);
    DVG_REQUIRE((long)H * W * Cin < (1L << 31), DVG_ERR_SHAPE, "dvg_gemm_batched_k16: image of %d x %d x %d floats too large", H, W, Cin);
    p.w_image_stride = (long)Cin / 16 * Cout * DVG_WROW;
    float* workspace = nullptr;
    const long workspace_floats = 0;
    int Hg = H, Wg = W, ti, th, tw;
    DVG_REQUIRE(tile2(M2_GEMM, NB, Hg, Wg, Cout, &ti, &th, &tw) == 0 && ti == 1, DVG_ERR_SHAPE,
                "dvg_gemm_batched_k16: no tile for %dx%d", H, W);
#if DVG_BF16X3
    if (g_tile_policy && Cout % 128 == 0 && Wg % 16 == 0 && (long)NB * (Hg / 8) * (Wg / 16) * (Cout / 128) >= DVG_GEMM_NT2)
        return launch2<M2_GEMM, 1, 8, 16, 2>(p, Hg, Wg, workspace, workspace_floats, (hipStream_t)stream);
#endif
    D2(M2_GEMM, 1, 8, 16)
    D2(M2_GEMM, 1, 8, 8)
    return fail(DVG_ERR_SHAPE, "dvg_gemm_batched_k16: no kernel");
}
```

dvg_amd/fused.py:

```python
from __future__ import annotations

import collections
import contextlib
import functools
import os
import types
import weakref

import torch
import torch.nn as nn

from . import _derived, ops, weights
from ._derived import derived, version_key as _ver
from .ops import ACT_LRELU, ACT_NONE, ACT_SIGMOID, ACT_TANH, MODE_CONV3, MODE_CONV4S2, MODE_CONVT4S2


WINOGRAD = int(os.environ.get("DVG_WINOGRAD", "4"))
if WINOGRAD not in (0, 2, 4):
    raise RuntimeError("DVG_WINOGRAD must be 0, 2 or 4")


_WINO_MIN_C = 64
_WINO_MAX_HW = 32


WINOGRAD_LAYER_OVERRIDE = {}


def winograd_tile(n, c, h, w, cout) -> int:
    if WINOGRAD_LAYER_OVERRIDE:
        forced = WINOGRAD_LAYER_OVERRIDE.get((c, h, cout))
        if forced is not None:
            return forced if (forced == 0 or ops.winograd_ok(n, c, h, w, cout, forced)) else 0
    if WINOGRAD >= 4 and c >= _WINO_MIN_C and h <= _WINO_MAX_HW and w <= _WINO_MAX_HW and ops.winograd_ok(n, c, h, w, cout, 4):
        return 4
    if WINOGRAD >= 2 and c >= 256 and ops.winograd_ok(n, c, h, w, cout, 2) and \
            ((h <= 8 and w <= 8) or (h <= 16 and w <= 16 and cout >= 256)):
        return 2
    return 0


UPCONV_WINOGRAD = True
_UPCONV_WINO_MAX = 16


def folded_affine(conv: nn.Module, bn: nn.BatchNorm2d):
    def build():
        with torch.no_grad():
            inv = torch.rsqrt(bn.running_var + bn.eps)
            scale = (bn.weight * inv) if bn.weight is not None else inv
            bias = conv.bias if conv.bias is not None else torch.zeros_like(bn.running_mean)
            shift = (bias - bn.running_mean) * scale
            if bn.bias is not None:
                shift = shift + bn.bias
            return scale.contiguous(), shift.contiguous()

    return derived(bn, "fold", (conv.bias, bn.weight, bn.bias, bn.running_mean, bn.running_var), build)


def _needs_grad(*ts) -> bool:
    return torch.is_grad_enabled() and any(
        t is not None and (t.t if isinstance(t, ops.SharedBlocks) else t).requires_grad for t in ts)


def _no_shared(skip, who):
    if isinstance(skip, ops.SharedBlocks):
        raise RuntimeError(f"{who}: shared skip blocks (time-batched decoder calls) are a training-path operand (autograd)")


def _bias(conv):
    return conv.bias.detach() if conv.bias is not None else None


Block = collections.namedtuple("Block", "raw mode finish cat dgrad")


def _raw_conv3(x, skip, wp, b, *, up=False, stats=False, addend=None):
    return ops.conv3x3(x, skip, wp, None, b, upsample=up, act=ACT_NONE, stats=stats, addend=addend)


def _raw_convT4s2(x, skip, wp, b, *, up=False, stats=False, addend=None):
    if up:
        raise RuntimeError("convT4s2: no fused upsampling")
    return ops.convT4x4s2(x, skip, wp, None, b, act=ACT_NONE, stats=stats, addend=addend)


def _raw_plain(name):
    def raw(x, skip, w, b, *, up=False, stats=False, addend=None):
        if skip is not None or up or addend is not None:
            raise RuntimeError(f"{name}: neither a concat conv nor an upsampling one")
        return getattr(ops, name)(x, w, None, b, act=ACT_NONE, stats=stats)
    return raw


def _dgrad_conv3(du, weight, lo, hi):
    n, c, h, w = du.shape
    m = winograd_tile(n, c, h, w, hi - lo)
    if m:
        return ops.conv3x3_winograd(du, weights.winograd(weight, m, lo, hi, dgrad=True), None, None, act=ACT_NONE)
    return ops.conv3x3(du, None, weights.packed(weight, True, lo, hi, 1), None, None, act=ACT_NONE)


def _dgrad_conv4s2(du, weight, lo, hi):
    return ops.convT4x4s2(du, None, weights.packed(weight, True, lo, hi, 1), None, None, act=ACT_NONE)


def _dgrad_convT4s2(du, weight, lo, hi):
    return ops.conv4x4s2(du, weights.packed(weight, False, lo, hi, 0), None, None, act=ACT_NONE)


BLOCKS = {
    "conv3": Block(_raw_conv3, MODE_CONV3, (0, 3, 3), 1, _dgrad_conv3),
    "conv4s2": Block(_raw_plain("conv4x4s2"), MODE_CONV4S2, (0, 4, 4), 1, _dgrad_conv4s2),
    "convT4s2": Block(_raw_convT4s2, MODE_CONVT4S2, (1, 4, 4), 0, _dgrad_convT4s2),
    "conv3_first": Block(_raw_plain("conv3x3_first"), None, (0, 3, 3), 1, None),
    "conv4s2_first": Block(_raw_plain("conv4x4s2_first"), None, (0, 4, 4), 1, None),
}


def block_weight(kind, weight, lo=None, hi=None):
    blk = BLOCKS[kind]
    return weight if blk.mode is None else weights.packed(weight, bool(blk.finish[0]), lo, hi, blk.cat)


def _skip_half(kind, skip, ps):
    return BLOCKS[kind].raw(skip, None, ps, None)


_scope = types.SimpleNamespace(passes=1, groups=None, trace=None, share=None)


@contextlib.contextmanager
def _scoped(result=None, **fields):
    prev = {k: getattr(_scope, k) for k in fields}
    vars(_scope).update(fields)
    try:
        yield result
    finally:
        vars(_scope).update(prev)


def bn_passes(k: int):
    return _scoped(passes=int(k))


def bn_momentum(bn, passes=None) -> float:
    m = bn.momentum if bn.momentum is not None else 0.1
    return 1.0 - (1.0 - m) ** (_scope.passes if passes is None else passes)


def bn_passes_now() -> int:
    return _scope.passes


_GROUP_STATS_RECOMPUTE = False


def bn_groups(groups: int, passes=(1, 1, 1)):
    return _scoped(groups=(int(groups),) + tuple(int(k) for k in passes) if groups > 1 else None)


def bn_groups_now() -> int:
    return _scope.groups[0] if _scope.groups else 1


def group_stats(st, u):
    g = bn_groups_now()
    if g == 1:
        return st
    if st is not None and getattr(st, "grouped", 0) == g:
        return st
    ti = getattr(st, "tile_images", 0) if st is not None else 0
    if ti and not _GROUP_STATS_RECOMPUTE and st.shape[0] % g == 0 and (u.shape[0] // g) % ti == 0:
        return st
    u2 = u if u.dim() == 2 else u.permute(0, 2, 3, 1).reshape(-1, u.shape[1])
    return ops.channel_stats(u2, g)


def bn_counter(bn):
    return bn.num_batches_tracked if (bn.track_running_stats and bn.num_batches_tracked is not None) else None


def bn_trace():
    trace = types.SimpleNamespace(entries=[])
    return _scoped(trace, trace=trace.entries)


def replay_bn_trace(entries) -> None:
    for bn, stats, count, passes, groups in entries:
        with _scoped(trace=None, groups=groups, passes=passes):
            _train_bn(bn, stats, count, synced=True)


_SYNC_BN = None


def set_sync_bn(dist=None, group=None) -> None:
    global _SYNC_BN
    if dist is None or not dist.is_initialized() or dist.get_world_size(group) <= 1:
        _SYNC_BN = None
    else:
        _SYNC_BN = (dist, group, dist.get_world_size(group))
    ops.set_sync_bn_state(_SYNC_BN)


def sync_bn_world() -> int:
    return _SYNC_BN[2] if _SYNC_BN is not None else 1


def _train_bn(bn: nn.BatchNorm2d, stats, count, save=False, synced=False):
    grouped, passes = _scope.groups, _scope.passes
    g = grouped[0] if grouped else 1
    if _SYNC_BN is not None and not synced:
        stats = ops.sync_partial_rows(stats, g)
        count = count * _SYNC_BN[2]
    if _scope.trace is not None:
        _scope.trace.append((bn, stats, count, passes, grouped))
    if grouped:
        _, p0, p1, p2 = grouped
        if passes != 1 or count % g:
            raise RuntimeError("grouped BatchNorm: bn_passes must be 1 and the groups must divide the batch")
        momentum, passes, momenta = 0.0, p0 + p2 + (g - 2) * p1, tuple(bn_momentum(bn, k) for k in (p0, p1, p2))
    else:
        momentum, momenta = bn_momentum(bn), None
    return ops.bn_finalize(stats, bn.weight.detach() if bn.weight is not None else None,
                           bn.bias.detach() if bn.bias is not None else None,
                           bn.running_mean if bn.track_running_stats else None,
                           bn.running_var if bn.track_running_stats else None, count // g, bn.eps, momentum, save=save,
                           num_batches_tracked=bn_counter(bn), passes=passes, groups=g, group_momenta=momenta)



SKIP_HOIST = os.environ.get("DVG_SKIP_HOIST", "1") != "0"
UPCONV_AS_CONVT = os.environ.get("DVG_UPCONV_AS_CONVT", "1") != "0"
_skip_seen = {}


_frozen = {}


def clear_skip_hoist_cache():
    _skip_seen.clear()
    _frozen.clear()


_derived.register("skip_hoist", clear_skip_hoist_cache, _skip_seen.values, skip_keyed=(_skip_seen, _frozen))


def declare_frozen_skips(skips) -> None:
    if not SKIP_HOIST:
        return
    for dead in [k for k, e in _frozen.items() if e[0]() is None]:
        del _frozen[dead]
    for s in skips:
        _frozen[id(s)] = (weakref.ref(s), s._version)


def share_skip_halves():
    return _scoped(share={})


def skip_share_scope():
    return _scope.share


def precompute_skip_half(conv, skip, kind: str) -> None:
    if not SKIP_HOIST or skip is None:
        return
    ctot = conv.weight.shape[BLOCKS[kind].cat]
    s = _skip_half(kind, skip, block_weight(kind, conv.weight, ctot - skip.shape[1], ctot))
    _skip_seen[(id(conv), id(skip))] = [weakref.ref(skip), skip._version, _ver(conv.weight), 1, s]


def _hoisted_skip(conv, x, skip, partial_fn, force=False):
    if skip is None or (not SKIP_HOIST and not force):
        return None
    k = (id(conv), id(skip))
    wkey = _ver(conv.weight)
    ent = _skip_seen.get(k)
    if ent is None or ent[0]() is not skip or ent[1] != skip._version or ent[2] != wkey:
        for dead in [kk for kk, e in _skip_seen.items() if e[0]() is None]:
            del _skip_seen[dead]
        if len(_skip_seen) > 64:
            _skip_seen.clear()
        _skip_seen[k] = ent = [weakref.ref(skip), skip._version, wkey, 1, None]
        fz = _frozen.get(id(skip))
        if not force and (fz is None or fz[0]() is not skip or fz[1] != skip._version):
            return None
    else:
        ent[3] += 1
    px, ps = weights.split_packed(conv.weight, x.shape[1], isinstance(conv, nn.ConvTranspose2d))
    if ent[4] is None:
        ent[4] = partial_fn(ps)
    return px, ent[4]


WINOGRAD_CHAIN = os.environ.get("DVG_WINOGRAD_CHAIN", "1") != "0"


_CHAIN_LEVEL = int(os.environ.get("DVG_WINOGRAD_CHAIN", "3"))


def _chain_to(conv_next, n, c, h, w, pool=False):
    if not (WINOGRAD_CHAIN and WINOGRAD >= 4 and conv_next is not None and not conv_next.training
            and isinstance(conv_next, nn.Conv2d) and conv_next.weight.shape[1] == c and tuple(conv_next.kernel_size) == (3, 3)):
        return False
    if pool:
        return (_CHAIN_LEVEL >= 2 and winograd_tile(n, c, h // 2, w // 2, conv_next.weight.shape[0]) == 4
                and ops.winograd_pool_chain_ok(n, c, h, w))
    if h > 16 and _CHAIN_LEVEL < 2:
        return False
    return winograd_tile(n, c, h, w, conv_next.weight.shape[0]) == 4 and ops.winograd_chain_ok(n, c, h, w)


def _from(res, y_from):
    if not y_from:
        return res
    y, yp = res
    return (y[y_from:] if y_from < y.shape[0] else None), yp


def _hoist_ready(conv, skip) -> bool:
    if not SKIP_HOIST or skip is None:
        return False
    ent = _skip_seen.get((id(conv), id(skip)))
    if ent is not None and ent[0]() is skip and ent[1] == skip._version and ent[2] == _ver(conv.weight):
        return True
    fz = _frozen.get(id(skip))
    return fz is not None and fz[0]() is skip and fz[1] == skip._version


def _chain_up_to(next_up, n, c, h, w, stem=False) -> bool:
    if next_up is None or torch.is_grad_enabled():
        return False
    conv_n, bn_n, skip_n = next_up
    if not (WINOGRAD_CHAIN and _CHAIN_LEVEL >= 3 and WINOGRAD >= 4 and UPCONV_WINOGRAD and isinstance(conv_n, nn.Conv2d)
            and tuple(conv_n.kernel_size) == (3, 3) and not conv_n.training and not bn_n.training and skip_n is not None
            and not isinstance(skip_n, ops.SharedBlocks)):
        return False
    if conv_n.weight.shape[1] - skip_n.shape[1] != c or tuple(skip_n.shape) != (n, skip_n.shape[1], 2 * h, 2 * w):
        return False
    return (2 * h <= _UPCONV_WINO_MAX and winograd_tile(n, c, 2 * h, 2 * w, conv_n.weight.shape[0]) == 4
            and ((h, w) == (4, 4) if stem else ops.winograd_up_chain_ok(n, c, h, w)) and _hoist_ready(conv_n, skip_n))


def _hand_over(next_conv, next_up, n, c, h, w, pool=False):
    if _chain_to(next_conv, n, c, h, w, pool):
        return True
    return "up" if not pool and _chain_up_to(next_up, n, c, h, w) else False


def _bn_act_train(bn, u, st, *, act, slope=0.2, pool=False):
    n, _, h, w = u.shape
    sc, sh = _train_bn(bn, group_stats(st, u), n * h * w)
    return ops.bn_act_apply(u, sc, sh, act=act, slope=slope, pool=pool, inplace=True)


def _train_block(kind, conv, bn, x, skip=None, *, up=False, act, slope, pool=False):
    u, st = BLOCKS[kind].raw(x, skip, block_weight(kind, conv.weight), _bias(conv), up=up, stats=True)
    return _bn_act_train(bn, u, st, act=act, slope=slope, pool=pool)


def conv3_bn_act(conv, bn, x, skip=None, *, upsample=False, pool=False, act=ACT_LRELU, slope=0.2, next_conv=None, y_from=0,
                 next_up=None):
    if y_from and (not pool or bn.training or _needs_grad(x, skip, conv.weight, bn.weight)):
        raise RuntimeError("conv3_bn_act: y_from is an eval-mode, no-grad option of the pooled form")
    if isinstance(x, ops.WinoV) and x.up:
        hs = None if (bn.training or not upsample or pool) else \
            _hoisted_skip(conv, x, skip, functools.partial(_skip_half, "conv3", skip), force=True)
        if hs is None:
            raise RuntimeError("conv3_bn_act: an upsampled WinoV needs the eval-mode concat conv with its skip half hoisted")
        sc, sh = folded_affine(conv, bn)
        n, c1, h, w = x.shape
        cout = conv.weight.shape[0]
        return ops.conv3x3_winograd(x, weights.winograd(conv.weight, 4, 0, c1), sc, sh, act=act, slope=slope, upsample=True,
                                    addend=hs[1], to_v=_hand_over(next_conv, None, n, cout, h, w))
    if isinstance(x, ops.WinoV):
        if bn.training or skip is not None or upsample:
            raise RuntimeError("conv3_bn_act: a WinoV input needs an eval-mode plain 3x3 layer")
        sc, sh = folded_affine(conv, bn)
        n, c, h, w = x.shape
        cout = conv.weight.shape[0]
        if winograd_tile(n, c, h, w, cout) != 4:
            raise RuntimeError("conv3_bn_act: WinoV handed to a layer that is not F(4x4,3x3)")
        return ops.conv3x3_winograd(x, weights.winograd(conv.weight, 4), sc, sh, act=act, slope=slope, pool=pool,
                                    to_v=_hand_over(next_conv, next_up, n, cout, h, w, pool), y_from=y_from)
    if _needs_grad(x, skip, conv.weight, bn.weight):
        from .autograd import conv_block_autograd
        return conv_block_autograd("conv3", conv, bn, x, skip, upsample=upsample, pool=pool, act=act, slope=slope)
    _no_shared(skip, "conv3_bn_act")
    if not bn.training:
        sc, sh = folded_affine(conv, bn)
        if not pool:
            hs = _hoisted_skip(conv, x, skip, functools.partial(_skip_half, "conv3", skip))
            if hs is not None:
                if upsample and UPCONV_WINOGRAD:
                    n_, c1_, hx_, wx_ = x.shape
                    cout_ = conv.weight.shape[0]
                    if 2 * hx_ <= _UPCONV_WINO_MAX and winograd_tile(n_, c1_, 2 * hx_, 2 * wx_, cout_) == 4:
                        to_v = not torch.is_grad_enabled() and _hand_over(next_conv, None, n_, cout_, 2 * hx_, 2 * wx_)
                        return ops.conv3x3_winograd(x, weights.winograd(conv.weight, 4, 0, c1_), sc, sh, act=act, slope=slope,
                                                    upsample=True, addend=hs[1], to_v=to_v)
                if upsample and UPCONV_AS_CONVT:
                    return ops.convT4x4s2(x, None, weights.k4_packed(conv.weight, x.shape[1]), sc, sh, act=act, slope=slope,
                                          addend=hs[1])
                return ops.conv3x3(x, None, hs[0], sc, sh, upsample=upsample, act=act, slope=slope, addend=hs[1])
        if skip is None and not upsample:
            n, c, h, w = x.shape
            cout = conv.weight.shape[0]
            m = winograd_tile(n, c, h, w, cout)
            if m:
                to_v = m == 4 and not torch.is_grad_enabled() and _hand_over(next_conv, next_up, n, cout, h, w, pool)
                return ops.conv3x3_winograd(x, weights.winograd(conv.weight, m), sc, sh, act=act, slope=slope, pool=pool,
                                            to_v=to_v, y_from=y_from)
        return _from(ops.conv3x3(x, skip, weights.packed(conv.weight), sc, sh, upsample=upsample, act=act, slope=slope,
                                 pool=pool), y_from)
    return _train_block("conv3", conv, bn, x, skip, up=upsample, act=act, slope=slope, pool=pool)


def conv3_first_bn_act(conv, bn, x_nchw, *, act=ACT_LRELU, slope=0.2):
    if _needs_grad(x_nchw, conv.weight, bn.weight):
        from .autograd import conv_block_autograd
        return conv_block_autograd("conv3_first", conv, bn, x_nchw, None, act=act, slope=slope)
    if not bn.training:
        sc, sh = folded_affine(conv, bn)
        return ops.conv3x3_first(x_nchw, conv.weight, sc, sh, act=act, slope=slope)
    return _train_block("conv3_first", conv, bn, x_nchw, act=act, slope=slope)


FIRST_PAIR = True


def first_pair_applies(conv0, bn0, conv1, bn1, x_nchw) -> bool:
    if not FIRST_PAIR or bn0.training or bn1.training or _needs_grad(x_nchw, conv0.weight, bn0.weight, conv1.weight, bn1.weight):
        return False
    n, nc, h, w = x_nchw.shape
    return conv0.out_channels == 64 and conv1.in_channels == 64 and ops.first_pair_ok(n, nc, h, w, conv1.out_channels)


def conv3_first_pair(conv0, bn0, conv1, bn1, x_nchw, *, pool=False, slope=0.2, y_from=0):
    sc0, sh0 = folded_affine(conv0, bn0)
    sc1, sh1 = folded_affine(conv1, bn1)
    return ops.conv3x3_first_pair(x_nchw, weights.first_pair_taps(conv0.weight), sc0, sh0, weights.packed(conv1.weight), sc1, sh1,
                                  slope=slope, pool=pool, y_from=y_from)


def conv4s2_bn_act(conv, bn, x, *, act=ACT_LRELU, slope=0.2):
    if _needs_grad(x, conv.weight, bn.weight):
        from .autograd import conv_block_autograd
        return conv_block_autograd("conv4s2", conv, bn, x, None, act=act, slope=slope)
    if not bn.training:
        sc, sh = folded_affine(conv, bn)
        return ops.conv4x4s2(x, weights.packed(conv.weight), sc, sh, act=act, slope=slope)
    return _train_block("conv4s2", conv, bn, x, act=act, slope=slope)


def conv4s2_first_bn_act(conv, bn, x_nchw, *, act=ACT_LRELU, slope=0.2):
    if _needs_grad(x_nchw, conv.weight, bn.weight):
        from .autograd import conv_block_autograd
        return conv_block_autograd("conv4s2_first", conv, bn, x_nchw, None, act=act, slope=slope)
    if not bn.training:
        sc, sh = folded_affine(conv, bn)
        return ops.conv4x4s2_first(x_nchw, conv.weight, sc, sh, act=act, slope=slope)
    return _train_block("conv4s2_first", conv, bn, x_nchw, act=act, slope=slope)


def convT4s2_bn_act(conv, bn, x, skip=None, *, act=ACT_LRELU, slope=0.2):
    if _needs_grad(x, skip, conv.weight, bn.weight):
        from .autograd import conv_block_autograd
        return conv_block_autograd("convT4s2", conv, bn, x, skip, act=act, slope=slope)
    _no_shared(skip, "convT4s2_bn_act")
    if not bn.training:
        sc, sh = folded_affine(conv, bn)
        hs = _hoisted_skip(conv, x, skip, functools.partial(_skip_half, "convT4s2", skip))
        if hs is not None:
            return ops.convT4x4s2(x, None, hs[0], sc, sh, act=act, slope=slope, addend=hs[1])
        return ops.convT4x4s2(x, skip, weights.packed(conv.weight, True), sc, sh, act=act, slope=slope)
    return _train_block("convT4s2", conv, bn, x, skip, act=act, slope=slope)


def head_bn_tanh(conv, bn, x):
    if _needs_grad(x, conv.weight, bn.weight):
        from .autograd import dense_block_autograd
        return dense_block_autograd("head", conv, bn, x, act=ACT_TANH)
    n, c, h, w = x.shape
    if (h, w) != tuple(conv.kernel_size):
        raise RuntimeError(f"encoder head expects a {conv.kernel_size} map, got {(h, w)}")
    gw = weights.gemm_operand(conv.weight, "head")
    a = x.permute(0, 2, 3, 1).reshape(n, h * w * c)
    k = a.shape[1]
    splitk = max(1, min(64, k // 128))
    if not bn.training:
        sc, sh = folded_affine(conv, bn)
        return ops.gemm_nt(a, gw, sc, sh, act=ACT_TANH, splitk=splitk)
    u = ops.gemm_nt(a, gw, None, _bias(conv), act=ACT_NONE, splitk=splitk)
    u4 = u.view(n, 1, 1, u.shape[1]).permute(0, 3, 1, 2)
    return _bn_act_train(bn, u4, ops.channel_stats(u, bn_groups_now()), act=ACT_TANH).reshape(n, u.shape[1])


def stem_bn_act(conv, bn, vec, *, act=ACT_LRELU, slope=0.2, next_up=None):
    if _needs_grad(vec, conv.weight, bn.weight):
        from .autograd import dense_block_autograd
        return dense_block_autograd("stem", conv, bn, vec, act=act, slope=slope)
    dim, cout, kh, kw = conv.weight.shape
    vec = vec.reshape(-1, dim)
    n = vec.shape[0]
    gw = weights.gemm_operand(conv.weight, "stem")
    if not bn.training:
        sc, sh = folded_affine(conv, bn)
        wt = weights.gemm_operand(conv.weight, "stem_t")
        if wt is not None and (kh, kw) == (4, 4) and cout % 16 == 0 and _chain_up_to(next_up, n, cout, 4, 4, stem=True):
            return ops.stem_up_winograd_input(vec, wt, dim, sc, sh, cout, act=act, slope=slope)
    out = ops.nhwc_empty(n, cout, kh, kw, vec.device)
    out2d = out.permute(0, 2, 3, 1).reshape(n, kh * kw * cout)
    if not bn.training:
        if wt is not None:
            ops.stem_gemm(vec, wt, dim, sc, sh, out2d, period=cout, act=act, slope=slope)
        else:
            ops.gemm_nt(vec, gw, sc, sh, act=act, slope=slope, period=cout, out=out2d)
        return out
    ops.gemm_nt(vec, gw, None, _bias(conv), act=ACT_NONE, period=cout, out=out2d)
    return _bn_act_train(bn, out, ops.channel_stats(out2d.view(n * kh * kw, cout), bn_groups_now()), act=act, slope=slope)


def convT3_last(conv, x, *, act=ACT_SIGMOID):
    if _needs_grad(x, conv.weight):
        from .autograd import last_layer_autograd
        return last_layer_autograd("convT3", conv, x, None, act=act)
    return ops.convT_last_two_step(x, None, conv.weight, _bias(conv), conv.weight.shape[1], 3, act=act)


def convT4s2_last(conv, x, skip, *, act=ACT_TANH):
    if _needs_grad(x, skip, conv.weight):
        from .autograd import last_layer_autograd
        return last_layer_autograd("convT4s2", conv, x, skip, act=act)
    _no_shared(skip, "convT4s2_last")
    return ops.convT_last_two_step(x, skip, conv.weight, _bias(conv), conv.weight.shape[1], 4, act=act)
```

dvg_amd/models/backbones.py:

```python
from __future__ import annotations

import torch
import torch.nn as nn

from .. import fused, ops
from ..ops import ACT_SIGMOID, ACT_TANH

_VGG_ENC = {
    64: [[("nc", 64), (64, 64)], [(64, 128), (128, 128)], [(128, 256), (256, 256), (256, 256)],
         [(256, 512), (512, 512), (512, 512)]],
    128: [[("nc", 64), (64, 64)], [(64, 128), (128, 128)], [(128, 256), (256, 256), (256, 256)],
          [(256, 512), (512, 512), (512, 512)], [(512, 512), (512, 512), (512, 512)]],
}
_VGG_DEC = {
    64: [[(1024, 512), (512, 512), (512, 256)], [(512, 256), (256, 256), (256, 128)], [(256, 128), (128, 64)],
         [(128, 64)]],
    128: [[(1024, 512), (512, 512), (512, 512)], [(1024, 512), (512, 512), (512, 256)],
          [(512, 256), (256, 256), (256, 128)], [(256, 128), (128, 64)], [(128, 64)]],
}
_DCGAN_ENC = {64: [("nc", 64), (64, 128), (128, 256), (256, 512)],
              128: [("nc", 64), (64, 128), (128, 256), (256, 512), (512, 512)]}
_DCGAN_DEC = {64: [(1024, 256), (512, 128), (256, 64)], 128: [(1024, 512), (1024, 256), (512, 128), (256, 64)]}


def _skip_nhwc(s):
    if isinstance(s, ops.SharedBlocks):
        return s.like(ops.to_nhwc(s.t))
    return ops.to_nhwc(s)


def _frame(x: torch.Tensor) -> torch.Tensor:
    if x.dim() != 4:
        raise RuntimeError(f"expected a (B,C,H,W) frame batch, got {tuple(x.shape)}")
    return x


class vgg_layer(nn.Module):

    def __init__(self, nin, nout):
        super().__init__()
        self.main = nn.Sequential(nn.Conv2d(nin, nout, 3, 1, 1), nn.BatchNorm2d(nout), nn.LeakyReLU(0.2, inplace=True))

    def forward(self, input):
        conv, bn = self.main[0], self.main[1]
        if conv.in_channels % 32:
            return fused.conv3_first_bn_act(conv, bn, _frame(input))
        return fused.conv3_bn_act(conv, bn, ops.to_nhwc(input))


class dcgan_conv(nn.Module):

    def __init__(self, nin, nout):
        super().__init__()
        self.main = nn.Sequential(nn.Conv2d(nin, nout, 4, 2, 1), nn.BatchNorm2d(nout), nn.LeakyReLU(0.2, inplace=True))

    def forward(self, input):
        conv, bn = self.main[0], self.main[1]
        if conv.in_channels % 32:
            return fused.conv4s2_first_bn_act(conv, bn, _frame(input))
        return fused.conv4s2_bn_act(conv, bn, ops.to_nhwc(input))


class dcgan_upconv(nn.Module):

    def __init__(self, nin, nout):
        super().__init__()
        self.main = nn.Sequential(nn.ConvTranspose2d(nin, nout, 4, 2, 1), nn.BatchNorm2d(nout),
                                  nn.LeakyReLU(0.2, inplace=True))

    def forward(self, input, skip=None):
        return fused.convT4s2_bn_act(self.main[0], self.main[1], ops.to_nhwc(input),
                                     None if skip is None else ops.to_nhwc(skip))


def _head(dim):
    return nn.Sequential(nn.Conv2d(512, dim, 4, 1, 0), nn.BatchNorm2d(dim), nn.Tanh())


def _stem(dim):
    return nn.Sequential(nn.ConvTranspose2d(dim, 512, 4, 1, 0), nn.BatchNorm2d(512), nn.LeakyReLU(0.2, inplace=True))


class VggEncoder(nn.Module):
    RES = 64

    def __init__(self, dim, nc=1):
        super().__init__()
        self.dim = dim
        plan = _VGG_ENC[self.RES]
        for s, stage in enumerate(plan, start=1):
            setattr(self, f"c{s}", nn.Sequential(*[vgg_layer(nc if a == "nc" else a, b) for a, b in stage]))
        setattr(self, f"c{len(plan) + 1}", _head(dim))
        self.mp = nn.MaxPool2d(kernel_size=2, stride=2, padding=0)

    def _stages(self):
        n = 1
        while hasattr(self, f"c{n + 1}"):
            n += 1
        return [getattr(self, f"c{s}") for s in range(1, n)], getattr(self, f"c{n}")

    def features(self, input, skips_from=0):
        stages, head = self._stages()
        skips = []
        h = _frame(input)
        k = int(skips_from)
        if k and (self.training or torch.is_grad_enabled()):
            raise RuntimeError("encoder: skips_from is an eval-mode, no-grad option")
        for si, stage in enumerate(stages):
            layers = list(stage)
            if si == 0 and len(layers) == 2 and fused.first_pair_applies(layers[0].main[0], layers[0].main[1],
                                                                         layers[1].main[0], layers[1].main[1], h):
                full, h = fused.conv3_first_pair(layers[0].main[0], layers[0].main[1], layers[1].main[0], layers[1].main[1], h,
                                                 pool=True, y_from=k)
                skips.append(full)
                continue
            for li, layer in enumerate(layers):
                conv, bn = layer.main[0], layer.main[1]
                last = li == len(layers) - 1
                if conv.in_channels % 32:
                    h = fused.conv3_first_bn_act(conv, bn, h)
                elif last:
                    nxt = stages[si + 1][0].main[0] if si + 1 < len(stages) else None
                    full, h = fused.conv3_bn_act(conv, bn, h, pool=True, next_conv=nxt, y_from=k)
                    skips.append(full)
                else:
                    h = fused.conv3_bn_act(conv, bn, h, next_conv=layers[li + 1].main[0])
        return fused.head_bn_tanh(head[0], head[1], h), skips

    def forward(self, input):
        h, skips = self.features(input)
        return h.view(-1, self.dim), skips

    def encode(self, input, skips_from=0):
        h, skips = self.features(input, skips_from)
        return h.view(-1, self.dim), skips


class VggDecoder(nn.Module):
    RES = 64

    def __init__(self, dim, nc=1):
        super().__init__()
        self.dim = dim
        plan = _VGG_DEC[self.RES]
        self.upc1 = _stem(dim)
        for s, stage in enumerate(plan, start=2):
            mods = [vgg_layer(a, b) for a, b in stage]
            if s == len(plan) + 1:
                mods += [nn.ConvTranspose2d(64, nc, 3, 1, 1), nn.Sigmoid()]
            setattr(self, f"upc{s}", nn.Sequential(*mods))
        self.up = nn.UpsamplingNearest2d(scale_factor=2)

    def forward(self, input):
        vec, skip = input
        n = 1
        while hasattr(self, f"upc{n + 1}"):
            n += 1
        sks = {s: _skip_nhwc(skip[n - s]) for s in range(2, n + 1)}
        fl = self.upc2[0]
        d = fused.stem_bn_act(self.upc1[0], self.upc1[1], vec,
                              next_up=(fl.main[0], fl.main[1], sks[2]) if isinstance(fl, vgg_layer) and n > 2 else None)
        for s in range(2, n + 1):
            sk = sks[s]
            first = True
            mods = list(getattr(self, f"upc{s}"))
            for li, layer in enumerate(mods):
                if isinstance(layer, vgg_layer):
                    nxt = mods[li + 1] if li + 1 < len(mods) and isinstance(mods[li + 1], vgg_layer) and s < n else None
                    nup = None
                    if nxt is None and li == len(mods) - 1 and s < n:
                        fl = getattr(self, f"upc{s + 1}")[0]
                        nup = (fl.main[0], fl.main[1], sks[s + 1])
                    if first:
                        d = fused.conv3_bn_act(layer.main[0], layer.main[1], d, sk, upsample=True,
                                               next_conv=None if nxt is None else nxt.main[0], next_up=nup)
                        first = False
                    else:
                        d = fused.conv3_bn_act(layer.main[0], layer.main[1], d,
                                               next_conv=None if nxt is None else nxt.main[0], next_up=nup)
                elif isinstance(layer, nn.ConvTranspose2d):
                    d = fused.convT3_last(layer, d, act=ACT_SIGMOID)
        return d

    @torch.no_grad()
    def precompute_frozen_skips(self, skip) -> None:
        n = 1
        while hasattr(self, f"upc{n + 1}"):
            n += 1
        for s in range(2, n + 1):
            first = next(l for l in getattr(self, f"upc{s}") if isinstance(l, vgg_layer))
            fused.precompute_skip_half(first.main[0], ops.to_nhwc(skip[n - s]), "conv3")


class VggGaussianEncoder(VggEncoder):

    def __init__(self, dim, output_size, nc=1):
        super().__init__(dim, nc)
        self.output_size = output_size
        self.mu_net = nn.Linear(dim, output_size)
        self.logvar_net = nn.Linear(dim, output_size)

    def reparameterize(self, mu, logvar):
        from .lstm import reparameterize
        return reparameterize(mu, logvar)

    def forward(self, input):
        from .lstm import linear
        h, skips = self.features(input)
        h = h.view(-1, self.dim)
        mu = linear(self.mu_net, h)
        logvar = linear(self.logvar_net, h)
        return self.reparameterize(mu, logvar), mu, logvar, skips


class DcganEncoder(nn.Module):
    RES = 64

    def __init__(self, dim, nc=1):
        super().__init__()
        self.dim = dim
        plan = _DCGAN_ENC[self.RES]
        for s, (a, b) in enumerate(plan, start=1):
            setattr(self, f"c{s}", dcgan_conv(nc if a == "nc" else a, b))
        setattr(self, f"c{len(plan) + 1}", _head(dim))

    def forward(self, input):
        return self.encode(input)

    def encode(self, input, skips_from=0):
        n = 1
        while hasattr(self, f"c{n + 1}"):
            n += 1
        h = _frame(input)
        k = int(skips_from)
        skips = []
        for s in range(1, n):
            layer = getattr(self, f"c{s}")
            conv, bn = layer.main[0], layer.main[1]
            h = fused.conv4s2_first_bn_act(conv, bn, h) if conv.in_channels % 32 else fused.conv4s2_bn_act(conv, bn, h)
            skips.append(h if not k else (h[k:] if k < h.shape[0] else None))
        head = getattr(self, f"c{n}")
        return fused.head_bn_tanh(head[0], head[1], h).view(-1, self.dim), skips


class DcganDecoder(nn.Module):
    RES = 64
    FINAL_ACT = ACT_TANH

    def __init__(self, dim, nc=1):
        super().__init__()
        self.dim = dim
        plan = _DCGAN_DEC[self.RES]
        self.upc1 = _stem(dim)
        for s, (a, b) in enumerate(plan, start=2):
            setattr(self, f"upc{s}", dcgan_upconv(a, b))
        final_act = nn.Tanh() if self.FINAL_ACT == ACT_TANH else nn.Sigmoid()
        setattr(self, f"upc{len(plan) + 2}", nn.Sequential(nn.ConvTranspose2d(128, nc, 4, 2, 1), final_act))

    def forward(self, input):
        vec, skip = input
        n = 1
        while hasattr(self, f"upc{n + 1}"):
            n += 1
        d = fused.stem_bn_act(self.upc1[0], self.upc1[1], vec)
        for s in range(2, n):
            layer = getattr(self, f"upc{s}")
            d = fused.convT4s2_bn_act(layer.main[0], layer.main[1], d, _skip_nhwc(skip[n - s]))
        last = getattr(self, f"upc{n}")
        act = ACT_SIGMOID if isinstance(last[1], nn.Sigmoid) else ACT_TANH
        return fused.convT4s2_last(last[0], d, _skip_nhwc(skip[0]), act=act)

    @torch.no_grad()
    def precompute_frozen_skips(self, skip) -> None:
        n = 1
        while hasattr(self, f"upc{n + 1}"):
            n += 1
        for s in range(2, n):
            fused.precompute_skip_half(getattr(self, f"upc{s}").main[0], ops.to_nhwc(skip[n - s]), "convT4s2")
        ops.precompute_skip_proj(ops.to_nhwc(skip[0]), getattr(self, f"upc{n}")[0].weight, 4)
```

dvg_amd/ops/__init__.py:

```python
from ._core import (
    ACT_NONE, ACT_LRELU, ACT_TANH, ACT_SIGMOID, MODE_CONV3, MODE_CONV4S2, MODE_CONVT4S2, _stream, KernelTimer,
    set_timer, _run, _p, _dev_f32, nhwc_empty, is_nhwc, to_nhwc, to_nchw, tile_policy,
)
from .conv import (
    pack_conv_weight, pack_convT_weight, packed_row_floats, pack_igemm_weight, _wp_dims, unpack_conv_weight,
    unpack_convT_weight, _splitk_ws, _SPLITK_WS, evict_captured_workspaces, _stats_buf, _tile_images, SharedBlocks,
    _MAP_CACHE, shared_map, group_sum, _check_addend, conv3x3, CONV4S2_MAX_FLOATS, conv4x4s2, convT4x4s2,
)
from .winograd import (
    winograd_weight, winograd_ok, WinoV, winograd_chain_ok, winograd_up_chain_ok, winograd_pool_chain_ok,
    conv3x3_winograd, stem_up_winograd_input,
)
from .edge import (
    conv3x3_first, first_pair_ok, conv3x3_first_pair, convT3x3_last, conv4x4s2_first, convT4x4s2_last, pixel_proj,
    _SKIP_PROJ_CACHE, clear_skip_proj_cache, _cached_skip_proj, _last_wmat, _last_wmat_cached,
    precompute_skip_proj, convT_last_two_step, eval_frames, eval_frames_finn, pairwise_frame_mse, moving_mnist_compose, clip_gather, clip_gather_aug, CLIP_MAX_SHIFT,
    mnist_scale_u8, moving_mnist_compose_u8, frame_mosaic, QUANT_TRUNC, QUANT_NEAREST,
    MOSAIC_BLACK, MOSAIC_RED, MOSAIC_GREEN, MOSAIC_SEL_NONE, MOSAIC_SEL_BEST, MOSAIC_SEL_PICK, MOSAIC_CELL_INTS,
)
from .dense import (
    gemm_nt, lstm_cell, lstm_cell_pre, lstm_cell_bwd, lstm_cell_x, stem_gemm, transpose2d, colsum, GEMM_TN_MAX_ROWS,
    gemm_tn, lstm_gates_bwd, gru_cell, gru_cell_pre, rnn_cell, gru_gates_bwd,
)
from .norm import (
    channel_stats, set_sync_bn_state, sync_bn_state, sync_partial_rows, bn_finalize, bn_act_apply, bn_act_bwd,
)
from .gp import (
    gp_predict, gp_var_norms, gp_trigger_step, gp_trigger_replay, gp_trigger_select, gp_elbo, gp_elbo_bwd,
    sum_steps, gp_step_group, gp_train_bwd,
)
from .backward import (
    _LOSS_W, frame_losses, FRAME_LOSS_KINDS, frame_losses_ext, mse_sum_grad, conv_wgrad_partial, conv_wgrad_partial_multi, winograd_wgrad_ok,
    winograd_wgrad_partial_multi, wgrad_finish, k4_to_w3, conv_wgrad, wgrad_thin, act_bwd, upsample2x_bwd, adam_step, adam_step_guarded,
)
from .guard import grad_sumsq_blocks, grad_sumsq, grad_guard_finish
from .ema import ema_update_blocks, ema_update
from .lr_schedule import LR_KINDS, lr_schedule_tick
from .validate import val_accumulators, val_accumulate
from .._lib import check, lib
```

dvg_amd/ops/conv.py:

```python
from __future__ import annotations

import torch

from .._derived import register
from .._lib import check, lib
from ._core import ACT_LRELU, MODE_CONV3, MODE_CONV4S2, MODE_CONVT4S2, _dev_f32, _p, _run, _stream, is_nhwc, nhwc_empty


def pack_conv_weight(w: torch.Tensor) -> torch.Tensor:
    _dev_f32(w, "pack_conv_weight")
    w = w.detach().contiguous()
    co, ci, kh, kw = w.shape
    out = torch.empty((kh * kw, co, ci), device=w.device, dtype=torch.float32)
    check(lib().dvg_pack_conv_weight(_p(w), _p(out), co, ci, kh, kw, _stream()), "pack_conv_weight")
    return out


def pack_convT_weight(w: torch.Tensor) -> torch.Tensor:
    _dev_f32(w, "pack_convT_weight")
    w = w.detach().contiguous()
    ci, co, kh, kw = w.shape
    out = torch.empty((kh * kw, co, ci), device=w.device, dtype=torch.float32)
    check(lib().dvg_pack_convT_weight(_p(w), _p(out), ci, co, kh, kw, _stream()), "pack_convT_weight")
    return out


def packed_row_floats() -> int:
    return int(lib().dvg_packed_row_floats())


def pack_igemm_weight(w: torch.Tensor, transposed: bool = False) -> torch.Tensor:
    _dev_f32(w, "pack_igemm_weight")
    w = w.detach().contiguous()
    if transposed:
        ci, co, kh, kw = w.shape
    else:
        co, ci, kh, kw = w.shape
    out = torch.empty((ci // 16, kh * kw, co, packed_row_floats()), device=w.device, dtype=torch.float32)
    check(lib().dvg_pack_conv_weight_k16(_p(w), _p(out), co, ci, kh, kw, int(transposed), _stream()), "pack_k16")
    return out


def _wp_dims(wp: torch.Tensor):
    if wp.dim() != 4 or wp.shape[3] != packed_row_floats():
        raise RuntimeError(f"packed igemm weight must be [Cin/16][taps][Cout][{packed_row_floats()}], got {tuple(wp.shape)}")
    return wp.shape[1], wp.shape[2], wp.shape[0] * 16


def unpack_conv_weight(wp: torch.Tensor, kh: int, kw: int) -> torch.Tensor:
    t, co, ci = wp.shape
    out = torch.empty((co, ci, kh, kw), device=wp.device, dtype=torch.float32)
    check(lib().dvg_unpack_conv_weight(_p(wp.contiguous()), _p(out), co, ci, kh, kw, _stream()), "unpack_conv_weight")
    return out


def unpack_convT_weight(wp: torch.Tensor, kh: int, kw: int) -> torch.Tensor:
    t, co, ci = wp.shape
    out = torch.empty((ci, co, kh, kw), device=wp.device, dtype=torch.float32)
    check(lib().dvg_unpack_convT_weight(_p(wp.contiguous()), _p(out), ci, co, kh, kw, _stream()),
          "unpack_convT_weight")
    return out


def _splitk_ws(mode, n, h, w, cin, cout, out_numel, device):
    s = lib().dvg_conv_splitk_v2(mode, n, h, w, cin, cout)
    if s <= 1:
        return None
    stream = torch.cuda.current_stream(device).cuda_stream
    key = (device.index if device.index is not None else torch.cuda.current_device(), stream, s * out_numel,
           lib().dvg_stream_capture_id(stream))
    ws = _SPLITK_WS.get(key)
    if ws is None:
        if len(_SPLITK_WS) > 256:
            _SPLITK_WS.clear()
        ws = _SPLITK_WS[key] = torch.empty(s * out_numel, device=device, dtype=torch.float32)
    return ws


_SPLITK_WS = {}
register("splitk_ws", _SPLITK_WS.clear, _SPLITK_WS.values)


def evict_captured_workspaces() -> None:
    for k in [k for k in _SPLITK_WS if k[-1] != 0]:
        del _SPLITK_WS[k]


def _stats_buf(rows: int, cout: int, device, tile_images: int = 0):
    if rows <= 0:
        raise RuntimeError("unsupported shape for fused BN statistics")
    st = torch.empty((rows, 2, cout), device=device, dtype=torch.float32)
    st.tile_images = tile_images
    return st


def _tile_images(mode, n, h, w, cin, cout, gh, gw, ws):
    if ws is not None and lib().dvg_conv_splitk_v2(mode, n, h, w, cin, cout) != 1:
        return 0
    return 4 if (gh, gw) == (4, 4) else 1


class SharedBlocks:
    __slots__ = ("t", "block", "map_dev", "map_host")

    def __init__(self, t, block, map_dev, map_host):
        self.t, self.block, self.map_dev, self.map_host = t, int(block), map_dev, tuple(map_host)

    @property
    def blocks(self):
        return self.t.shape[0] // self.block

    @property
    def groups(self):
        return len(self.map_host)

    def like(self, t):
        return SharedBlocks(t, self.block, self.map_dev, self.map_host)


_MAP_CACHE = {}
register("group_maps", _MAP_CACHE.clear, _MAP_CACHE.values)


def shared_map(map_host, device):
    key = (tuple(map_host), str(device))
    m = _MAP_CACHE.get(key)
    if m is None:
        if torch.cuda.is_current_stream_capturing():
            raise RuntimeError("shared_map: a new group map cannot be created while a hipGraph is being captured")
        m = _MAP_CACHE[key] = torch.tensor(list(map_host), dtype=torch.int32, device=device)
    return m


def group_sum(src, shared: "SharedBlocks"):
    _dev_f32(src, "group_sum")
    g, blk = shared.groups, shared.block
    if src.shape[0] != g * blk:
        raise RuntimeError(f"group_sum: {src.shape[0]} images are not {g} groups of {blk}")
    per_image = src.numel() // src.shape[0]
    if src.stride(0) != per_image:
        src = src.contiguous()
    dst = torch.empty_strided((shared.blocks * blk,) + tuple(src.shape[1:]), src.stride(), device=src.device,
                              dtype=torch.float32)
    elems = src.numel() // g
    check(lib().dvg_group_sum(_p(src), _p(shared.map_dev), _p(dst), g, shared.blocks, elems, _stream()), "group_sum")
    return dst


def _check_addend(addend, y, excluded):
    if addend is None:
        return None, None, 0
    if excluded:
        raise RuntimeError("addend excludes the pooled output")
    if isinstance(addend, SharedBlocks):
        t = addend.t
        _dev_f32(t, "addend")
        if (tuple(t.shape[1:]) != tuple(y.shape[1:]) or t.stride() != y.stride() or
                y.shape[0] != addend.groups * addend.block):
            raise RuntimeError(f"shared addend {tuple(t.shape)} x {addend.groups} groups does not match {tuple(y.shape)}")
        return t, addend.map_dev, addend.block
    _dev_f32(addend, "addend")
    if tuple(addend.shape) != tuple(y.shape) or addend.stride() != y.stride():
        raise RuntimeError(f"addend {tuple(addend.shape)} must match the output {tuple(y.shape)} (NHWC in memory)")
    return addend, None, 0


def conv3x3(x, skip, wp, scale, shift, *, upsample=False, act=ACT_LRELU, slope=0.2, pool=False, stats=False,
            addend=None):
    _dev_f32(x, "conv3x3.x")
    assert is_nhwc(x), "conv3x3: x must be NHWC in memory"
    n, c1, hx, wx = x.shape
    h, w = (hx * 2, wx * 2) if upsample else (hx, wx)
    c2 = 0
    if skip is not None:
        _dev_f32(skip, "conv3x3.skip")
        assert is_nhwc(skip), "conv3x3: skip must be NHWC in memory"
        c2 = skip.shape[1]
        if tuple(skip.shape) != (n, c2, h, w):
            raise RuntimeError(f"conv3x3: skip shape {tuple(skip.shape)} does not match {(n, c2, h, w)}")
    taps, cout, cin = _wp_dims(wp)
    if taps != 9 or cin != c1 + c2:
        raise RuntimeError(f"conv3x3: packed weight {tuple(wp.shape)} does not match Cin={c1 + c2}")
    y = nhwc_empty(n, cout, h, w, x.device)
    yp = nhwc_empty(n, cout, h // 2, w // 2, x.device) if pool else None
    addend, amap, ablk = _check_addend(addend, y, pool)
    ws = _splitk_ws(MODE_CONV3, n, h, w, cin, cout, y.numel(), x.device)
    if stats:
        rows = lib().dvg_conv_stats_rows_v2(MODE_CONV3, n, h, w, cin, cout, int(pool), int(ws is not None))
    st = _stats_buf(rows, cout, x.device, _tile_images(MODE_CONV3, n, h, w, cin, cout, h, w, ws)) if stats else None
    fl, by = 2.0 * n * h * w * cout * 9 * cin, 4.0 * (x.numel() + (skip.numel() if c2 else 0) + n * h * w * cout +
                                                      wp.numel())
    _run("conv3x3_igemm", fl, by, lib().dvg_conv3x3_bn_act_v2, _p(x), _p(skip), _p(wp), _p(scale), _p(shift), _p(y),
         _p(yp), _p(st), n, h, w, c1, c2, cout, int(upsample), act, slope, _p(ws), 0 if ws is None else ws.numel(),
         _p(addend), _p(amap), ablk, _stream())
    out = (y, yp) if pool else y
    return (out, st) if stats else out


CONV4S2_MAX_FLOATS = 1 << 31


def conv4x4s2(x, wp, scale, shift, *, act=ACT_LRELU, slope=0.2, stats=False):
    _dev_f32(x, "conv4x4s2.x")
    assert is_nhwc(x)
    n, cin, h, w = x.shape
    taps, cout, cin_w = _wp_dims(wp)
    if taps != 16 or cin_w != cin:
        raise RuntimeError(f"conv4x4s2: packed weight {tuple(wp.shape)} does not match Cin={cin}")
    y = nhwc_empty(n, cout, h // 2, w // 2, x.device)
    if x.numel() >= CONV4S2_MAX_FLOATS:
        per = (CONV4S2_MAX_FLOATS - 1) // (cin * h * w)
        per -= per % 8
        if per <= 0:
            raise RuntimeError(f"conv4x4s2: one image of {cin} x {h} x {w} exceeds the kernel's 32-bit offsets")
        runs = -(-n // per)
        per = min(per, -(-(-(-n // runs)) // 8) * 8)
        sts = []
        for lo in range(0, n, per):
            r = conv4x4s2(x[lo:lo + per], wp, scale, shift, act=act, slope=slope, stats=stats)
            y[lo:lo + per].copy_(r[0] if stats else r)
            if stats:
                sts.append(r[1])
        if not stats:
            return y
        st = torch.cat(sts)
        ti = {t.tile_images for t in sts}
        st.tile_images = ti.pop() if len(ti) == 1 else 0
        return y, st
    ws = _splitk_ws(MODE_CONV4S2, n, h, w, cin, cout, y.numel(), x.device)
    if stats:
        rows = lib().dvg_conv_stats_rows_v2(MODE_CONV4S2, n, h, w, cin, cout, 0, int(ws is not None))
    st = _stats_buf(rows, cout, x.device, _tile_images(MODE_CONV4S2, n, h, w, cin, cout, h // 2, w // 2, ws)) if stats else None
    fl, by = 2.0 * n * (h // 2) * (w // 2) * cout * 16 * cin, 4.0 * (x.numel() + y.numel() + wp.numel())
    _run("conv4x4s2_igemm", fl, by, lib().dvg_conv4x4s2_bn_act_v2, _p(x), _p(wp), _p(scale), _p(shift), _p(y), _p(st),
         n, h, w, cin, cout, act, slope, _p(ws), 0 if ws is None else ws.numel(), _stream())
    return (y, st) if stats else y


def convT4x4s2(x, skip, wp, scale, shift, *, act=ACT_LRELU, slope=0.2, stats=False, addend=None):
    _dev_f32(x, "convT4x4s2.x")
    assert is_nhwc(x)
    n, c1, h, w = x.shape
    c2 = 0
    if skip is not None:
        assert is_nhwc(skip)
        c2 = skip.shape[1]
        if tuple(skip.shape) != (n, c2, h, w):
            raise RuntimeError("convT4x4s2: skip shape mismatch")
    taps, cout, cin = _wp_dims(wp)
    if taps != 16 or cin != c1 + c2:
        raise RuntimeError(f"convT4x4s2: packed weight {tuple(wp.shape)} does not match Cin={c1 + c2}")
    y = nhwc_empty(n, cout, 2 * h, 2 * w, x.device)
    addend, amap, ablk = _check_addend(addend, y, False)
    ws = _splitk_ws(MODE_CONVT4S2, n, h, w, cin, cout, y.numel(), x.device)
    if stats:
        rows = lib().dvg_conv_stats_rows_v2(MODE_CONVT4S2, n, h, w, cin, cout, 0, int(ws is not None))
    st = _stats_buf(rows, cout, x.device, _tile_images(MODE_CONVT4S2, n, h, w, cin, cout, h, w, ws)) if stats else None
    fl = 2.0 * n * h * w * cout * 16 * cin
    by = 4.0 * (x.numel() + (skip.numel() if c2 else 0) + y.numel() + wp.numel())
    _run("convT4x4s2_igemm", fl, by, lib().dvg_convT4x4s2_bn_act_v2, _p(x), _p(skip), _p(wp), _p(scale), _p(shift),
         _p(y), _p(st), n, h, w, c1, c2, cout, act, slope, _p(ws), 0 if ws is None else ws.numel(), _p(addend),
         _p(amap), ablk, _stream())
    return (y, st) if stats else y
```

dvg_amd/ops/edge.py:

```python
from __future__ import annotations

import numpy as np
import torch

from .._derived import derived, register
from .._lib import check, lib
from ._core import ACT_LRELU, ACT_SIGMOID, ACT_TANH, _dev_f32, _p, _run, _stream, is_nhwc, nhwc_empty
from .conv import SharedBlocks, _stats_buf, _wp_dims


def conv3x3_first(x_nchw, w, scale, shift, *, act=ACT_LRELU, slope=0.2, stats=False):
    _dev_f32(x_nchw, "conv3x3_first.x")
    x = x_nchw if x_nchw.is_contiguous() else x_nchw.contiguous()
    n, nc, h, wd = x.shape
    w = w.detach()
    cout = w.shape[0]
    if tuple(w.shape) != (cout, nc, 3, 3) or not w.is_contiguous():
        raise RuntimeError("conv3x3_first: weight must be contiguous (Cout,nc,3,3)")
    y = nhwc_empty(n, cout, h, wd, x.device)
    st = _stats_buf(lib().dvg_conv_first_stats_rows(3, n, h, wd), cout, x.device, 1) if stats else None
    _run("conv3x3_first", 2.0 * n * h * wd * cout * 9 * nc, 4.0 * (x.numel() + n * h * wd * cout),
         lib().dvg_conv3x3_first, _p(x), _p(w), _p(scale), _p(shift), _p(y), _p(st), n, h, wd, nc, cout, act, slope,
         _stream())
    return (y, st) if stats else y


def first_pair_ok(n, nc, h, w, cout) -> bool:
    return nc == 1 and h % 8 == 0 and w % 16 == 0 and cout % 64 == 0 and n * (h // 8) * (w // 16) * (cout // 64) >= 512


def conv3x3_first_pair(x_nchw, w0, scale0, shift0, wp1, scale1, shift1, *, act=ACT_LRELU, slope=0.2, pool=False, y_from=0):
    _dev_f32(x_nchw, "conv3x3_first_pair.x")
    x = x_nchw if x_nchw.is_contiguous() else x_nchw.contiguous()
    n, nc, h, wd = x.shape
    taps, cout, cin = _wp_dims(wp1)
    w0 = w0.detach()
    if nc != 1 or tuple(w0.shape) != (9, 64) or not w0.is_contiguous() or (taps, cin) != (9, 64) or \
            not first_pair_ok(n, nc, h, wd, cout):
        raise RuntimeError(f"conv3x3_first_pair: unsupported shapes x {tuple(x.shape)} w0 {tuple(w0.shape)} wp1 {tuple(wp1.shape)}")
    if not 0 <= y_from <= n or (y_from and not pool):
        raise RuntimeError("conv3x3_first_pair: y_from needs the pooled output and 0 <= y_from <= N")
    y = nhwc_empty(n - y_from, cout, h, wd, x.device) if y_from < n else None
    yp = nhwc_empty(n, cout, h // 2, wd // 2, x.device) if pool else None
    flops = 2.0 * n * h * wd * (64 * 9 + cout * 9 * 64)
    _run("conv3x3_igemm", flops, 4.0 * (x.numel() + (0 if y is None else y.numel()) + (0 if yp is None else yp.numel()) + wp1.numel()),
         lib().dvg_conv3x3_first_pair, _p(x), _p(w0), _p(scale0), _p(shift0), _p(wp1), _p(scale1), _p(shift1), _p(y), _p(yp),
         n, h, wd, cout, act, slope, y_from, _stream(), alg_flops=flops)
    return (y, yp) if pool else y


def convT3x3_last(x, w, bias, nc, *, act=ACT_SIGMOID):
    _dev_f32(x, "convT3x3_last.x")
    assert is_nhwc(x)
    n, cin, h, wd = x.shape
    w = w.detach()
    if tuple(w.shape) != (cin, nc, 3, 3) or not w.is_contiguous():
        raise RuntimeError("convT3x3_last: weight must be contiguous (Cin,nc,3,3)")
    y = torch.empty((n, nc, h, wd), device=x.device, dtype=torch.float32)
    _run("convT3x3_last", 2.0 * n * h * wd * cin * 9 * nc, 4.0 * (x.numel() + y.numel()),
         lib().dvg_convT3x3_last, _p(x), _p(w), _p(bias), _p(y), n, h, wd, cin, nc, act, _stream())
    return y


def conv4x4s2_first(x_nchw, w, scale, shift, *, act=ACT_LRELU, slope=0.2, stats=False):
    _dev_f32(x_nchw, "conv4x4s2_first.x")
    x = x_nchw if x_nchw.is_contiguous() else x_nchw.contiguous()
    n, nc, h, wd = x.shape
    w = w.detach()
    cout = w.shape[0]
    if tuple(w.shape) != (cout, nc, 4, 4) or not w.is_contiguous():
        raise RuntimeError("conv4x4s2_first: weight must be contiguous (Cout,nc,4,4)")
    y = nhwc_empty(n, cout, h // 2, wd // 2, x.device)
    st = _stats_buf(lib().dvg_conv_first_stats_rows(4, n, h, wd), cout, x.device, 1) if stats else None
    _run("conv4x4s2_first", 2.0 * n * (h // 2) * (wd // 2) * cout * 16 * nc, 4.0 * (x.numel() + y.numel()),
         lib().dvg_conv4x4s2_first, _p(x), _p(w), _p(scale), _p(shift), _p(y), _p(st), n, h, wd, nc, cout, act, slope,
         _stream())
    return (y, st) if stats else y


def convT4x4s2_last(x, skip, w, bias, nc, *, act=ACT_TANH):
    _dev_f32(x, "convT4x4s2_last.x")
    assert is_nhwc(x)
    n, c1, h, wd = x.shape
    c2 = 0
    if skip is not None:
        assert is_nhwc(skip)
        c2 = skip.shape[1]
    w = w.detach()
    if tuple(w.shape) != (c1 + c2, nc, 4, 4) or not w.is_contiguous():
        raise RuntimeError("convT4x4s2_last: weight must be contiguous (Cin,nc,4,4)")
    y = torch.empty((n, nc, 2 * h, 2 * wd), device=x.device, dtype=torch.float32)
    _run("convT4x4s2_last", 2.0 * n * h * wd * (c1 + c2) * 16 * nc,
         4.0 * (x.numel() + (skip.numel() if c2 else 0) + y.numel()), lib().dvg_convT4x4s2_last, _p(x), _p(skip),
         _p(w), _p(bias), _p(y), n, h, wd, c1, c2, nc, act, _stream())
    return y


def pixel_proj(x, wm):
    assert is_nhwc(x)
    n, c, h, wd = x.shape
    t = wm.shape[0]
    d = torch.empty((n * h * wd, t), device=x.device, dtype=torch.float32)
    _run("pixel_proj", 2.0 * n * h * wd * c * t, 4.0 * (x.numel() + d.numel()), lib().dvg_pixel_proj, _p(x), _p(wm),
         _p(d), n * h * wd, c, t, _stream())
    return d


_SKIP_PROJ_CACHE = {}


def clear_skip_proj_cache():
    _SKIP_PROJ_CACHE.clear()


register("skip_proj", clear_skip_proj_cache, _SKIP_PROJ_CACHE.values, skip_keyed=(_SKIP_PROJ_CACHE,))


def _cached_skip_proj(skip, wm_fn, w):
    import weakref
    key = id(skip)
    ent = _SKIP_PROJ_CACHE.get(key)
    if ent is not None and ent[0]() is skip and ent[1] == skip._version and ent[2] == id(w) and ent[3] == w._version:
        return ent[4]
    d2 = pixel_proj(skip, wm_fn())
    if len(_SKIP_PROJ_CACHE) > 8:
        _SKIP_PROJ_CACHE.clear()
    _SKIP_PROJ_CACHE[key] = (weakref.ref(skip), skip._version, id(w), w._version, d2)
    return d2


def _last_wmat(wpart, t):
    return wpart.permute(2, 3, 1, 0).reshape(t, wpart.shape[0]).contiguous()


def _last_wmat_cached(w, lo, hi, t):
    return derived(w, ("wmat", lo, hi), (w,), lambda: _last_wmat(w.detach()[lo:hi], t))


def precompute_skip_proj(skip, w, ks: int) -> None:
    wdet = w.detach()
    c1 = wdet.shape[0] - skip.shape[1]
    t = ks * ks * wdet.shape[1]
    _cached_skip_proj(skip, lambda: _last_wmat_cached(w, c1, wdet.shape[0], t), w)


def convT_last_two_step(x, skip, w, bias, nc, ks, *, act):
    assert is_nhwc(x)
    n, c1, h, wd = x.shape
    wdet = w.detach()
    t = ks * ks * nc
    d1 = pixel_proj(x, _last_wmat_cached(w, 0, c1, t))
    d2 = None
    d2_map, d2_blk = None, 0
    if isinstance(skip, SharedBlocks):
        d2 = pixel_proj(skip.t, _last_wmat_cached(w, c1, wdet.shape[0], t))
        d2_map, d2_blk = skip.map_dev, skip.block
        if n != skip.groups * skip.block:
            raise RuntimeError("convT_last_two_step: shared skip does not match the batch")
    elif skip is not None:
        d2 = _cached_skip_proj(skip, lambda: _last_wmat_cached(w, c1, wdet.shape[0], t), w)
    s = 2 if ks == 4 else 1
    y = torch.empty((n, nc, s * h, s * wd), device=x.device, dtype=torch.float32)
    _run("convT_gather", 0.0, 4.0 * (d1.numel() * (2 if skip is not None else 1) + y.numel()), lib().dvg_convT_gather,
         _p(d1), _p(d2), _p(bias), _p(y), ks, n, h, wd, nc, act, _p(d2_map), d2_blk, _stream())
    return y


def eval_frames(gt, pred):
    _dev_f32(gt, "eval_frames.gt")
    _dev_f32(pred, "eval_frames.pred")
    if gt.shape != pred.shape or gt.dim() != 4:
        raise RuntimeError(f"eval_frames: shapes {tuple(gt.shape)} vs {tuple(pred.shape)}")
    gt = gt if gt.is_contiguous() else gt.contiguous()
    pred = pred if pred.is_contiguous() else pred.contiguous()
    b, c, h, w = gt.shape
    out = torch.empty((2, b, c), device=gt.device, dtype=torch.float32)
    _run("eval_frames", 0.0, 8.0 * gt.numel(), lib().dvg_eval_frames, _p(gt), _p(pred), _p(out[0]), _p(out[1]), b * c, h,
         w, _stream())
    return out[0].mean(1), out[1].mean(1)


def eval_frames_finn(gt, pred):
    _dev_f32(gt, "eval_frames_finn.gt")
    _dev_f32(pred, "eval_frames_finn.pred")
    if gt.shape != pred.shape or gt.dim() not in (4, 5):
        raise RuntimeError(f"eval_frames_finn: shapes {tuple(gt.shape)} vs {tuple(pred.shape)}")
    gt = gt if gt.is_contiguous() else gt.contiguous()
    pred = pred if pred.is_contiguous() else pred.contiguous()
    lead, (c, h, w) = tuple(gt.shape[:-3]), gt.shape[-3:]
    n = gt.numel() // (c * h * w)
    out = torch.empty((2, n, c), device=gt.device, dtype=torch.float32)
    mse = torch.empty(n, device=gt.device, dtype=torch.float32)
    _run("eval_frames_finn", 0.0, 8.0 * gt.numel(), lib().dvg_eval_frames_finn, _p(gt), _p(pred), _p(out[0]), _p(out[1]),
         _p(mse), n, c, h, w, _stream())
    if c == 1:
        return out[0].view(lead), out[1].view(lead), mse.view(lead)
    return out[0].mean(1).view(lead), out[1].mean(1).view(lead), mse.view(lead)


def pairwise_frame_mse(samples, lo=None, hi=None):
    _dev_f32(samples, "pairwise_frame_mse.samples")
    if samples.dim() != 6 or samples.numel() == 0 or not samples.is_contiguous():
        raise RuntimeError(f"pairwise_frame_mse: samples {tuple(samples.shape)} must be a contiguous non-empty (S,T,B,C,H,W) tensor")
    s, t, b = samples.shape[:3]
    d = samples[0, 0, 0].numel()
    lo, hi = 0 if lo is None else int(lo), t if hi is None else int(hi)
    if not 0 <= lo < hi <= t:
        raise RuntimeError(f"pairwise_frame_mse: step range [{lo}, {hi}) of {t} steps")
    if d >= 1 << 31 or (hi - lo) * b >= 1 << 31:
        raise RuntimeError(f"pairwise_frame_mse: {hi - lo}x{b} frames of {d} floats exceed the kernel's 32-bit counts")
    out = torch.empty((hi - lo, b, s, s), device=samples.device, dtype=torch.float32)
    n = (hi - lo) * b
    _run("pairwise_frame_mse", 3.0 * n * d * (s * (s - 1) // 2), 4.0 * n * d * s + 4.0 * out.numel(),
         lib().dvg_pairwise_frame_mse, _p(samples[0, lo]), _p(out), s, t * b * d, n, d, d, _stream())
    return out


QUANT_TRUNC, QUANT_NEAREST = 0, 1
MOSAIC_BLACK, MOSAIC_RED, MOSAIC_GREEN = 0, 1, 2
MOSAIC_SEL_NONE, MOSAIC_SEL_BEST, MOSAIC_SEL_PICK = 0, 1, 2
MOSAIC_CELL_INTS = 8


def frame_mosaic(sources, cells, *, nc, H, W, F, R, Cc, cell_h, cell_w, pad_y=0, pad_x=0, oy=0, ox=0, best=None,
                 picks=None, labels=None, quant=QUANT_TRUNC):
    srcs = list(sources) + [None] * (3 - len(sources))
    if len(srcs) != 3:
        raise RuntimeError("frame_mosaic: at most three sources")
    dev, counts = None, []
    for i, s in enumerate(srcs):
        if s is None:
            counts.append(0)
            continue
        _dev_f32(s, f"frame_mosaic.sources[{i}]")
        if not s.is_contiguous() or s.numel() == 0 or s.numel() % (nc * H * W):
            raise RuntimeError(f"frame_mosaic: source {i} {tuple(s.shape)} is not a contiguous run of {nc}x{H}x{W} images")
        counts.append(s.numel() // (nc * H * W))
        dev = s.device
    if dev is None:
        raise RuntimeError("frame_mosaic: no source")

    def aux(t, dtype, dim, name):
        if t is None:
            return
        if not t.is_cuda or t.dtype != dtype or t.dim() != dim or not t.is_contiguous() or t.numel() == 0:
            raise RuntimeError(f"frame_mosaic: {name} must be a contiguous {dim}-D {dtype} device tensor")
    best, picks = (None if t is None else t.contiguous() for t in (best, picks))
    aux(best, torch.int64, 1, "best")
    aux(picks, torch.int32, 2, "picks")
    aux(labels, torch.uint8, 3, "labels")
    if not cells.is_cuda or cells.dtype != torch.int32 or not cells.is_contiguous() or \
            cells.numel() != F * R * Cc * MOSAIC_CELL_INTS:
        raise RuntimeError(f"frame_mosaic: cells must be a contiguous int32 device tensor of {F}x{R}x{Cc}x{MOSAIC_CELL_INTS}")
    gh, gw = R * cell_h + (R - 1) * pad_y, Cc * cell_w + (Cc - 1) * pad_x
    out = torch.empty((F, gh, gw, 3), device=dev, dtype=torch.uint8)
    read = 4.0 * nc * H * W * F * R * Cc
    _run("frame_mosaic", 0.0, read + out.numel(), lib().dvg_frame_mosaic, _p(srcs[0]), counts[0], _p(srcs[1]), counts[1],
         _p(srcs[2]), counts[2], nc, H, W, _p(cells), F, R, Cc, cell_h, cell_w, pad_y, pad_x, oy, ox, _p(best),
         0 if best is None else best.shape[0], _p(picks), 0 if picks is None else picks.shape[0],
         0 if picks is None else picks.shape[1], _p(labels), *((0, 0, 0) if labels is None else labels.shape), quant,
         _p(out), _stream())
    return out


def moving_mnist_compose(sprites, ids, pos, seq_len, image_size):
    _dev_f32(sprites, "moving_mnist_compose.sprites")
    if ids.dtype != torch.int32 or pos.dtype != torch.int32 or not ids.is_cuda or not pos.is_cuda:
        raise RuntimeError("moving_mnist_compose: ids / pos must be int32 device tensors")
    ids, pos, sprites = ids.contiguous(), pos.contiguous(), sprites.contiguous()
    b, nd = ids.shape
    if tuple(pos.shape) != (b, nd, seq_len, 2):
        raise RuntimeError(f"moving_mnist_compose: pos shape {tuple(pos.shape)}")
    out = torch.empty((seq_len, b, 1, image_size, image_size), device=sprites.device, dtype=torch.float32)
    check(lib().dvg_moving_mnist_compose(_p(sprites), _p(ids), _p(pos), _p(out), sprites.shape[0], seq_len, b, nd,
                                         image_size, sprites.shape[1], _stream()), "dvg_moving_mnist_compose")
    return out


def clip_gather(pool, first, T, C):
    if not pool.is_cuda or pool.dtype != torch.uint8 or pool.dim() != 4 or not pool.is_contiguous():
        raise RuntimeError("clip_gather: pool must be a contiguous (n_frames,H,W,pool_c) uint8 GPU tensor - no CPU fallback")
    n, h, w, pc = pool.shape
    if not (isinstance(first, torch.Tensor) and first.is_cuda):
        first = torch.as_tensor(first)
        if first.dtype != torch.int64 or first.dim() != 1 or first.numel() == 0:
            raise RuntimeError("clip_gather: first must be a non-empty 1-D int64 sequence")
        if T < 1 or int(first.min()) < 0 or int(first.max()) + T > n:
            raise RuntimeError(f"clip_gather: clips of {T} frames at [{int(first.min())}, {int(first.max())}] leave the "
                               f"pool of {n} frames")
        first = first.to(pool.device)
    if first.dtype != torch.int64 or first.dim() != 1 or not first.is_contiguous() or first.device != pool.device:
        raise RuntimeError("clip_gather: first must be a contiguous 1-D int64 tensor on the pool's device")
    b = first.shape[0]
    out = torch.empty((max(T, 0), b, C, h, w), device=pool.device, dtype=torch.float32)
    _run("clip_gather", 0.0, float(T * b * h * w * pc) + 4.0 * out.numel(), lib().dvg_clip_gather_u8, _p(pool), _p(first),
         _p(out), n, T, b, C, h, w, pc, _stream())
    return out


CLIP_MAX_SHIFT = 16


def clip_gather_aug(pool, first, geom, photo, T, C):
    if not pool.is_cuda or pool.dtype != torch.uint8 or pool.dim() != 4 or not pool.is_contiguous():
        raise RuntimeError("clip_gather_aug: pool must be a contiguous (n_frames,H,W,pool_c) uint8 GPU tensor - no CPU fallback")
    n, h, w, pc = pool.shape

    def on_device(t):
        return isinstance(t, torch.Tensor) and t.is_cuda

    def host_array(t):
        return np.ascontiguousarray(t.numpy() if isinstance(t, torch.Tensor) else t)
    host = {}
    if not on_device(first):
        f = host_array(first)
        if f.dtype != np.int64 or f.ndim != 1 or f.size == 0:
            raise RuntimeError("clip_gather_aug: first must be a non-empty 1-D int64 sequence")
        if T < 1 or int(f.min()) < 0 or int(f.max()) + T > n:
            raise RuntimeError(f"clip_gather_aug: clips of {T} frames at [{int(f.min())}, {int(f.max())}] leave the pool of "
                               f"{n} frames")
        host["first"] = f
    if not on_device(geom):
        g = host_array(geom)
        if g.dtype != np.int32 or g.ndim != 2 or g.shape[1] != 4 or g.size == 0:
            raise RuntimeError("clip_gather_aug: geom must be a non-empty (B,4) int32 array [hflip, reverse, dy, dx]")
        if int(g[:, 2:].min()) < -CLIP_MAX_SHIFT or int(g[:, 2:].max()) > CLIP_MAX_SHIFT:
            raise RuntimeError(f"clip_gather_aug: a shift (dy, dx) beyond +-{CLIP_MAX_SHIFT} pixels")
        host["geom"] = g
    if not on_device(photo):
        ph = host_array(photo)
        if ph.dtype != np.float32 or ph.ndim != 2 or ph.shape[1] != 2 or ph.size == 0:
            raise RuntimeError("clip_gather_aug: photo must be a non-empty (B,2) float32 array [gain, bias]")
        if not np.isfinite(ph).all():
            raise RuntimeError("clip_gather_aug: gain / bias must be finite")
        host["photo"] = ph
    if len(host) == 3:
        a, b_ = host["first"].nbytes, host["first"].nbytes + host["geom"].nbytes
        buf = np.empty(b_ + host["photo"].nbytes, np.uint8)
        buf[:a], buf[a:b_], buf[b_:] = (host[k].reshape(-1).view(np.uint8) for k in ("first", "geom", "photo"))
        packed = torch.from_numpy(buf).to(pool.device)
        first, geom, photo = packed[:a].view(torch.int64), packed[a:b_].view(torch.int32).view(-1, 4), \
            packed[b_:].view(torch.float32).view(-1, 2)
    else:
        first, geom, photo = (torch.from_numpy(host[k]).to(pool.device) if k in host else t
                              for k, t in (("first", first), ("geom", geom), ("photo", photo)))
    if first.dtype != torch.int64 or first.dim() != 1 or not first.is_contiguous() or first.device != pool.device:
        raise RuntimeError("clip_gather_aug: first must be a contiguous 1-D int64 tensor on the pool's device")
    b = first.shape[0]
    if geom.dtype != torch.int32 or tuple(geom.shape) != (b, 4) or not geom.is_contiguous() or geom.device != pool.device:
        raise RuntimeError(f"clip_gather_aug: geom must be a contiguous ({b},4) int32 tensor on the pool's device")
    if photo.dtype != torch.float32 or tuple(photo.shape) != (b, 2) or not photo.is_contiguous() or photo.device != pool.device:
        raise RuntimeError(f"clip_gather_aug: photo must be a contiguous ({b},2) float32 tensor on the pool's device")
    out = torch.empty((max(T, 0), b, C, h, w), device=pool.device, dtype=torch.float32)
    _run("clip_gather_aug", 0.0, float(T * b * h * w * pc) + 4.0 * out.numel(), lib().dvg_clip_gather_aug_u8, _p(pool), _p(first),
         _p(geom), _p(photo), _p(out), n, T, b, C, h, w, pc, _stream())
    return out


def mnist_scale_u8(raw, out_size=32, tables=None):
    from .. import mnist
    if not raw.is_cuda or raw.dtype != torch.uint8 or raw.dim() != 3 or raw.shape[1] != raw.shape[2] or not raw.is_contiguous() \
            or raw.shape[0] == 0:
        raise RuntimeError("mnist_scale_u8: raw must be a contiguous non-empty (n,s,s) uint8 GPU tensor - no CPU fallback")
    n, s, _ = raw.shape
    if s > out_size or out_size > 64:
        raise RuntimeError(f"mnist_scale_u8: {s} -> {out_size}: only up-scaling to at most 64 is restated")
    if tables is None:
        tables = [torch.from_numpy(t).to(raw.device) for t in mnist.resize_tables(s, out_size)]
    xmin, coef = tables
    if any(t.dtype != torch.int32 or t.device != raw.device or not t.is_contiguous() for t in tables) or \
            tuple(xmin.shape) != (out_size,) or tuple(coef.shape) != (out_size, mnist.TAPS):
        raise RuntimeError("mnist_scale_u8: tables must be int32 (out,) and (out,3) tensors on raw's device")
    out = torch.empty((n, out_size, out_size), device=raw.device, dtype=torch.uint8)
    _run("mnist_scale_u8", 0.0, float(raw.numel() + out.numel()), lib().dvg_mnist_scale_u8, _p(raw), _p(out), n, s, out_size,
         _p(xmin), _p(coef), _stream())
    return out


def moving_mnist_compose_u8(sprites, ids, pos, seq_len, image_size):
    if not sprites.is_cuda or sprites.dtype != torch.uint8 or sprites.dim() != 3 or sprites.shape[1] != sprites.shape[2] \
            or not sprites.is_contiguous():
        raise RuntimeError("moving_mnist_compose_u8: sprites must be a contiguous (N,D,D) uint8 GPU tensor - no CPU fallback")
    n, d, _ = sprites.shape
    if not (isinstance(ids, torch.Tensor) and ids.is_cuda):
        ids, pos = torch.as_tensor(ids), torch.as_tensor(pos)
        if ids.numel() == 0 or pos.numel() == 0 or int(ids.min()) < 0 or int(ids.max()) >= n:
            raise RuntimeError(f"moving_mnist_compose_u8: ids outside the pool of {n} digits")
        if int(pos.min()) < 0 or int(pos.max()) > image_size - d:
            raise RuntimeError(f"moving_mnist_compose_u8: pos outside [0, {image_size - d}]: a digit would leave the canvas")
        if ids.dtype != torch.int32 or pos.dtype != torch.int32:
            raise RuntimeError("moving_mnist_compose_u8: ids / pos must be int32")
        ids, pos = ids.to(sprites.device), pos.to(sprites.device)
    if ids.dtype != torch.int32 or not isinstance(pos, torch.Tensor) or pos.dtype != torch.int32 or ids.dim() != 2 \
            or ids.device != sprites.device or pos.device != sprites.device:
        raise RuntimeError("moving_mnist_compose_u8: ids (B,ND) / pos must be int32 tensors on the pool's device")
    ids, pos = ids.contiguous(), pos.contiguous()
    b, nd = ids.shape
    if tuple(pos.shape) != (b, nd, seq_len, 2):
        raise RuntimeError(f"moving_mnist_compose_u8: pos shape {tuple(pos.shape)}")
    out = torch.empty((seq_len, b, 1, image_size, image_size), device=sprites.device, dtype=torch.float32)
    check(lib().dvg_moving_mnist_compose_u8(_p(sprites), _p(ids), _p(pos), _p(out), n, seq_len, b, nd, image_size, d,
                                            _stream()), "dvg_moving_mnist_compose_u8")
    return out
```

include/dvg_hip.h:

```cpp
#ifndef DVG_HIP_H
#define DVG_HIP_H

#include <stddef.h>
#include <stdint.h>

#ifdef __cplusplus
extern "C" {
#endif

#define DVG_OK 0
#define DVG_ERR_SHAPE 1
#define DVG_ERR_NULL 2
#define DVG_ERR_HIP 3
#define DVG_ERR_ALIGN 4

#define DVG_ACT_NONE 0
#define DVG_ACT_LRELU 1
#define DVG_ACT_TANH 2
#define DVG_ACT_SIGMOID 3

int dvg_abi_version(void);
const char* dvg_last_error(void);
long dvg_stream_capture_id(void* stream);

int dvg_pack_conv_weight(const float* w_oihw, float* w_packed, int cout, int cin, int kh, int kw, void* stream);

int dvg_pack_convT_weight(const float* w_iohw, float* w_packed, int cin, int cout, int kh, int kw, void* stream);

int dvg_unpack_conv_weight(const float* w_packed, float* w_oihw, int cout, int cin, int kh, int kw, void* stream);
int dvg_unpack_convT_weight(const float* w_packed, float* w_iohw, int cin, int cout, int kh, int kw, void* stream);

#define DVG_MODE_CONV3 0
#define DVG_MODE_CONV4S2 1
#define DVG_MODE_CONVT4S2 2
int dvg_conv_first_stats_rows(int ks, int N, int H, int W);

int dvg_mfma_mode(void);
int dvg_packed_row_floats(void);
const char* dvg_build_info(void);
void dvg_set_tile_policy(int energy);
int dvg_tile_policy(void);
int dvg_pack_conv_weight_k16(const float* w, float* w_packed, int cout, int cin, int kh, int kw, int transposed, void* stream);
int dvg_conv_splitk_v2(int mode, int N, int H, int W, int Cin, int Cout);
int dvg_conv_stats_rows_v2(int mode, int N, int H, int W, int Cin, int Cout, int pool, int with_workspace);
int dvg_conv3x3_bn_act_v2(const float* x, const float* skip, const float* w_k16, const float* scale, const float* shift, float* y,
                          float* y_pool, float* stats, int N, int H, int W, int C1, int C2, int Cout, int upsample_x, int act,
                          float slope, float* workspace, long workspace_floats, const float* addend,
                          const int* addend_map, int addend_block, void* stream);
int dvg_conv3x3_first_pair(const float* frame, const float* w0, const float* scale0, const float* shift0,
                           const float* w1_k16, const float* scale1, const float* shift1, float* y, float* y_pool,
                           int N, int H, int W, int Cout, int act, float slope,
                           int y_from ,
                           void* stream);
int dvg_conv4x4s2_bn_act_v2(const float* x, const float* w_k16, const float* scale, const float* shift, float* y, float* stats,
                            int N, int H, int W, int Cin, int Cout, int act, float slope, float* workspace, long workspace_floats,
                            void* stream);
int dvg_convT4x4s2_bn_act_v2(const float* x, const float* skip, const float* w_k16,
                             const float* scale, const float* shift, float* y, float* stats,
                             int N, int H, int W, int C1, int C2, int Cout, int act, float slope,
                             float* workspace, long workspace_floats, const float* addend,
                             const int* addend_map , int addend_block, void* stream);

int dvg_winograd_weight(const float* w_oihw, float* u_k16, int cout, int cin, int m, void* stream);
int dvg_winograd_input(const float* x, float* v, int N, int H, int W, int C, int m, int upsample, void* stream);
int dvg_gemm_batched_k16(const float* x, const float* w_k16, float* y, int NB, int H, int W, int Cin, int Cout,
                         void* stream);
int dvg_winograd_output(const float* mm, const float* scale, const float* shift, float* y, float* y_pool, int N, int H,
                        int W, int C, int act, float slope, int m, const float* addend,
                        int y_from , void* stream);
int dvg_winograd_output_input(const float* mm, const float* scale, const float* shift, float* v_next, int N, int H, int W,
                              int C, int act, float slope, const float* addend ,
                              void* stream);
int dvg_stem_up_winograd_input(const float* vec, int ldv, const float* w_kn, int KP, const float* scale, const float* shift,
                               float* v_next, int M, int C, int K, int act, float slope, void* stream);
int dvg_winograd_output_up_input(const float* mm, const float* scale, const float* shift, float* v_next, int N, int H, int W,
                                 int C, int act, float slope, void* stream);
int dvg_winograd_output_pool_input(const float* m, const float* scale, const float* shift, float* y, float* v_next, int N,
                                   int H, int W, int C, int act, float slope, int y_from, void* stream);

int dvg_conv3x3_first(const float* x_nchw, const float* w_oihw, const float* scale, const float* shift, float* y, float* stats,
                      int N, int H, int W, int nc, int Cout, int act, float slope, void* stream);

int dvg_convT3x3_last(const float* x, const float* w_iohw, const float* bias, float* y_nchw, int N, int H, int W, int Cin,
                      int nc, int act, void* stream);

int dvg_conv4x4s2_first(const float* x_nchw, const float* w_oihw, const float* scale, const float* shift, float* y, float* stats,
                        int N, int H, int W, int nc, int Cout, int act, float slope, void* stream);

int dvg_convT4x4s2_last(const float* x, const float* skip, const float* w_iohw, const float* bias, float* y_nchw, int N, int H,
                        int W, int C1, int C2, int nc, int act, void* stream);

int dvg_pixel_proj(const float* in, const float* w, float* out, long P, int C, int T, void* stream);

int dvg_convT_gather(const float* d1, const float* d2, const float* bias, float* y_nchw, int ks,
                     int N, int H, int W, int nc, int act,
                     const int* d2_map ,
                     int d2_block, void* stream);


int dvg_channel_stats_rows(long rows);
int dvg_channel_stats(const float* u, float* stats_partial, long rows, int C, int groups, void* stream);
int dvg_channel_stats_pivot(const float* u, float* stats_partial, const float* pivot, long rows, int C, int groups,
                            void* stream);

int dvg_bn_finalize(const float* stats_partial, int nrows, const float* gamma,
                    const float* beta, float* scale, float* shift, float* running_mean,
                    float* running_var, float* save_mean, float* save_invstd,
                    int C, double count, float eps, float momentum,
                    int64_t* num_batches_tracked , int nbt_inc, int groups,
                    float* group_var, void* stream);
int dvg_bn_finalize_pivot(const float* stats_partial, int nrows, const float* pivot, const float* gamma,
                          const float* beta, float* scale, float* shift, float* running_mean, float* running_var,
                          float* save_mean, float* save_invstd, int C, double count, float eps, float momentum,
                          int64_t* num_batches_tracked, int nbt_inc, int groups, float* group_var, void* stream);
int dvg_bn_running_update(const float* mean, const float* unbiased_var, int groups, int C, float mom_first, float mom_mid,
                          float mom_last, float* running_mean, float* running_var, int64_t* num_batches_tracked,
                          int nbt_inc, void* stream);

int dvg_bn_act_apply(const float* u, const float* scale, const float* shift, float* y,
                     float* y_pool, int N, int H, int W, int C, int act, float slope,
                     int group_images, void* stream);

int dvg_gemm_nt_bias_act(const float* a, const float* w, const float* scale, const float* shift, float* out, float* workspace,
                         int M, int N, int K, int lda, int ldo, int period, int splitk, int act, float slope,
                         int accumulate , void* stream);

int dvg_lstm_cell(const float* x, const float* h, const float* c, const float* w_ih, const float* w_hh, const float* b_ih,
                  const float* b_hh, float* h_out, float* c_out, float* gates_out, int B, int H, void* stream);

int dvg_lstm_cell_pre(const float* pre, const float* h, const float* c, const float* w_hh, float* h_out,
                      float* c_out, float* gates_out, int B, int H, void* stream);
int dvg_lstm_cell_bwd(const float* dh_a, const float* dh_b, const float* dc, const float* gates,
                      const float* c_prev, const float* c_new, const float* w_hh_t, float* dG, float* dc_prev,
                      float* dh_prev, int B, int H, void* stream);

int dvg_lstm_cell_x(const float* x, int ldx, int Kx, const float* h, const float* c, const float* w_x, int Kxp,
                    const float* w_hh, const float* bias, float* h_out, float* c_out, int B, int H, void* stream);

int dvg_gru_cell(const float* x, const float* h, const float* w_ih, const float* w_hh, const float* b_ih, const float* b_hh,
                 float* h_out, float* acts_out, int B, int H, void* stream);
int dvg_gru_cell_pre(const float* pre, const float* h, const float* w_hh, const float* b_hn, float* h_out, float* acts_out,
                     int B, int H, void* stream);
int dvg_rnn_cell(const float* x, const float* h, const float* w_ih, const float* w_hh, const float* b_ih, const float* b_hh,
                 float* h_out, int B, int H, void* stream);
int dvg_gru_gates_bwd(const float* dh_a, const float* dh_b, const float* acts, const float* h_prev, float* dGi, float* dGh,
                      float* dh_prev, int B, int H, void* stream);

int dvg_stem_gemm(const float* vec, int ldv, const float* w_kn, int KP, const float* scale, const float* shift,
                  float* out, int ldo, int M, int N, int K, int period, int act, float slope, void* stream);


int dvg_gp_precision(int B, int M, int need_cov);
size_t dvg_gp_lds_bytes(int B, int M, int need_cov);
int dvg_gp_predict(const float* h, const float* z, const float* var_mean, const float* chol_var, const float* mean_const,
                   const float* outputscale, const float* lengthscale, const float* noise, const float* eps, float* mean,
                   float* var, float* sample, float* cov, float* kl, int B, int D, int M, int train_mode, float jitter,
                   int param_period ,
                   int step_group ,
                   void* stream);
int dvg_gp_step_group(int B, int S, int P, int M);


int dvg_bn_act_bwd_rows(int N, int H, int W, int pool);
int dvg_bn_act_bwd_reduce(const float* dy, const float* dyp, const float* y, const float* u,
                          float* dp, float* partial, int N, int H, int W, int C, int act,
                          float slope, int groups, void* stream);
int dvg_bn_act_bwd_reduce_centered(const float* dy, const float* dyp, const float* y, const float* u, const float* mean,
                                   float* dp, float* partial, int N, int H, int W, int C, int act, float slope,
                                   int groups, void* stream);
int dvg_bn_bwd_finalize(const float* partial, int nrows, const float* gamma, const float* mean,
                        const float* invstd, float* coefA, float* coefB, float* coefC,
                        float* dgamma, float* dbeta, float* dbias, int C, double count,
                        int train, int accumulate , int groups, void* stream);
int dvg_bn_bwd_finalize_centered(const float* partial, int nrows, const float* gamma, const float* mean,
                                 const float* invstd, float* coefA, float* coefB, float* coefC,
                                 float* dgamma, float* dbeta, float* dbias, int C, double count,
                                 int train, int accumulate, int groups, void* stream);
int dvg_affine3_apply(const float* dp, const float* u, const float* A, const float* B,
                      const float* Cc, float* du, long n, int C, float* sum, int sum_mode,
                      int groups , void* stream);
int dvg_group_sum(const float* src, const int* map, float* dst, int groups, int blocks, long block_elems, void* stream);
int dvg_act_bwd(const float* dy, const float* y, float* dpre, long n, int act, float slope,
                void* stream);
int dvg_upsample2x_bwd(const float* dxu, float* dx, int N, int H, int W, int C, void* stream);
int dvg_colsum(const float* a, float* out, int rows, int C, int accumulate , void* stream);
int dvg_reduce_partials(const float* partial, float* out, int S, long n, void* stream);

int dvg_conv_wgrad_splits(int mode, int N, int H, int W, int Cin, int Cout);
int dvg_conv_wgrad(int mode, const float* x, const float* skip, const float* dout,
                   float* partial, int N, int H, int W, int C1, int C2, int Cout,
                   int upsample_x, void* stream);
int dvg_conv_wgrad_splits_multi(int mode, int N, int H, int W, int Cin, int Cout, int items);
int dvg_conv_wgrad_multi(int mode, int items, const float* const* x, const float* const* skip,
                         const float* const* dout, float* partial, int N, int H, int W, int C1, int C2,
                         int Cout, int upsample_x, void* stream);

int dvg_winograd_wgrad_operands(const float* x, const float* dy, float* v, float* dm, int N, int H, int W, int Cin,
                                int Cout, long t_total, long t_off, void* stream);
int dvg_winograd_wgrad_splits(long t_total, int Cin, int Cout);
int dvg_winograd_wgrad_gemm(const float* dm, const float* v, float* partial, long t_total, int Cin, int Cout, void* stream);
int dvg_winograd_wgrad_gemm_items(const float* dm, const float* const* v_items, int items, long tiles_per_item,
                                  float* partial, int Cin, int Cout, void* stream);
int dvg_winograd_wgrad_reduce(const float* partial, int S, float* packed, int Cin, int Cout, void* stream);

int dvg_wgrad_finish(const float* partial, int S, float* dst, int kind, int kh, int kw, int cout, int cin, int ctot,
                     int c_lo, float beta, void* stream);
int dvg_k4_to_w3(const float* dk4_packed, float* dw, int cout, int c1, int ctot, int c_lo, float beta, void* stream);

int dvg_wgrad_thin_rows(int ks, int N, int Hi, int Wi);
int dvg_wgrad_thin(const float* inp_nchw, const float* dout_nhwc, float* partial, int ks, int N,
                   int Hi, int Wi, int nc, int C, void* stream);

int dvg_moving_mnist_compose(const float* sprites, const int* ids, const int* pos, float* out, int n_sprites, int T,
                             int B, int num_digits, int image_size, int digit_size, void* stream);

int dvg_clip_gather_u8(const uint8_t* pool, const int64_t* first, float* out, int64_t n_frames, int T, int B, int C, int H,
                       int W, int pool_c, void* stream);
int dvg_clip_gather_aug_u8(const uint8_t* pool, const int64_t* first, const int32_t* geom, const float* photo, float* out,
                           int64_t n_frames, int T, int B, int C, int H, int W, int pool_c, void* stream);

int dvg_mnist_scale_u8(const uint8_t* raw, uint8_t* out, int n, int in_size, int out_size, const int* xmin, const int* coef,
                       void* stream);

int dvg_moving_mnist_compose_u8(const uint8_t* sprites, const int* ids, const int* pos, float* out, int n_sprites, int T,
                                int B, int num_digits, int image_size, int digit_size, void* stream);

int dvg_eval_frames(const float* gt, const float* pred, float* ssim, float* psnr, int n_images, int H, int W,
                    void* stream);

int dvg_eval_frames_finn(const float* gt, const float* pred, float* ssim, float* psnr, float* mse, int n_frames, int C, int H,
                         int W, void* stream);

int dvg_pairwise_frame_mse(const float* samples, float* out, int S, long sample_stride, int frames, long frame_stride, int D,
                           void* stream);

#define DVG_MOSAIC_CELL_INTS 8
#define DVG_MOSAIC_BLACK 0
#define DVG_MOSAIC_RED 1
#define DVG_MOSAIC_GREEN 2
#define DVG_MOSAIC_SEL_NONE 0
#define DVG_MOSAIC_SEL_BEST 1
#define DVG_MOSAIC_SEL_PICK 2
#define DVG_QUANT_TRUNC 0
#define DVG_QUANT_NEAREST 1
int dvg_frame_mosaic(const float* src0, long n0, const float* src1, long n1, const float* src2, long n2, int nc, int H,
                     int W, const int* cells, int F, int R, int Cc, int cell_h, int cell_w, int pad_y, int pad_x, int oy,
                     int ox, const long* best, int n_best, const int* picks, int n_pick_rows, int pick_k,
                     const unsigned char* labels, int n_labels, int lh, int lw, int quant, unsigned char* out,
                     void* stream);

int dvg_adam_step(float* param, const float* grad, float* exp_avg, float* exp_avg_sq, long n, float lr, float beta1,
                  float beta2, float eps, float weight_decay, int step, const int* step_dev, void* stream);

int dvg_gemm_tn(const float* a, const float* b, float* out, float* colsum0, float* colsum1, int R, int M, int N,
                int lda, int ldb, int ldo, int accumulate, int colsum_accumulate, void* stream);
int dvg_lstm_gates_bwd(const float* dh, const float* dc, const float* gates, const float* c_prev, const float* c_new, float* dG,
                       float* dc_prev, int B, int H, void* stream);

int dvg_gp_bwd_precision(int B, int M);
size_t dvg_gp_bwd_lds_bytes(int B, int M);
int dvg_gp_bwd_chunk(int B, int M);
int dvg_gp_train_bwd(const float* h, const float* z, const float* var_mean, const float* chol_var, const float* mean_const,
                     const float* outputscale, const float* lengthscale, const float* gmean, const float* gvar, const float* gkl,
                     float* dh, float* dz, float* dm, float* dls, float* dc, float* ds, float* dell, int B, int D, int M,
                     float jitter, int param_period ,
                     int step_group ,
                     void* stream);
int dvg_sum_steps_multi(const float* const* src, float* const* dst, const long* n, int count, int S, void* stream);

int dvg_gp_elbo(const float* mean, const float* var, const float* kl, const float* target, long t_stride_d,
                long t_stride_b, const float* raw_noise, float* elbo, int B, int D, int num_data,
                int noise_period , void* stream);
int dvg_gp_elbo_bwd(const float* mean, const float* var, const float* kl, const float* target, long t_stride_d, long t_stride_b,
                    const float* raw_noise, const float* gelbo, float* gmean, float* gvar, float* gkl, float* gtarget,
                    float* graw_noise, int B, int D, int num_data, int noise_period, void* stream);

int dvg_nchw_to_nhwc(const float* x, float* y, int N, int C, int H, int W, void* stream);
int dvg_nhwc_to_nchw(const float* x, float* y, int N, int C, int H, int W, void* stream);

void dvg_debug_set_clockbuf(void* buf, unsigned records);
void dvg_debug_set_gp_clockbuf(void* buf, unsigned records);
void dvg_debug_set_wgrad_clockbuf(void* buf, unsigned records);

int dvg_gp_var_norms(const float* var, float* norms, int D, int B, void* stream);
int dvg_gp_trigger_step(const float* var, int D, int B, int col, float* ctx, int window, float coef, int* flag, float* values,
                        float* thresholds, int* flags, int slot, void* stream);
int dvg_gp_trigger_replay(const float* values, int n, const float* ctx0, int window, float coef, int* flags, float* thresholds,
                          void* stream);
int dvg_gp_trigger_select(const int* flag, const float* sample_db, const float* h_pred, float* vec, int D, int B, int n_state,
                          long state_elems, const float* const* state_old, const float* const* state_new,
                          float* const* state_out, void* stream);

int dvg_frame_losses_blocks(long elems);
int dvg_frame_losses(const float* pred, const float* target, float* sums, float* dpred, long n, int S, int K, const float* w,
                     float* partial, void* stream);
int dvg_mse_sum_grad(const float* a, const float* b, float* sum, float* da, long n, float scale, void* stream);

int dvg_frame_losses_ext_blocks(int S, long planes, int H, int W);
int dvg_frame_losses_ext(const float* pred, const float* target, float* sums, float* dpred, int S, int K, long planes, int H, int W,
                         int kind, float eps, const float* w_pix, const float* w_gdl, float* partial, void* stream);

int dvg_zero_tick(float* g, long n, int* t0, int* t1, int* t2, int* t3, void* stream);

int dvg_grad_sumsq_blocks(long n);
int dvg_grad_sumsq(const float* g, long n, double* partials, void* stream);
int dvg_grad_guard_finish(const double* partials, int nblocks, double max_norm, int skip, float* stat, int* counters, void* stream);
int dvg_adam_step_guarded(float* param, const float* grad, float* exp_avg, float* exp_avg_sq, long n, float lr, float beta1, float beta2,
                          float eps, float weight_decay, int step, const int* step_dev, const float* stat, int* skips_dev, void* stream);
int dvg_lr_schedule_tick(int kind, int W, int N, int K, double R, double G, int* iter_dev, float* scale_dev, void* stream);
int dvg_adam_step_scheduled(float* param, const float* grad, float* exp_avg, float* exp_avg_sq, long n, float lr, float beta1,
                            float beta2, float eps, float weight_decay, int step, const int* step_dev, const float* stat,
                            int* skips_dev, const float* lr_scale_dev, void* stream);

int dvg_ema_update_blocks(long n);
int dvg_ema_update(float* ema, const float* param, long n, double decay, const int* updates_dev, double* partials, void* stream);

int dvg_val_accumulate(const float* ssim, const float* psnr, const float* mse, int B, int S, int T, double* acc, long long* cnt,
                       int* best, void* stream);

#ifdef __cplusplus
}
#endif
#endif
```

Measured before the change: 51550 frames/s.

## Fuse last-layer pixel projection into the upsampling transposed-conv epilogue

Adds a PROJ variant of the transposed 4x4/s2 implicit-GEMM kernel. It stages the 64-channel activated output tile in LDS and multiplies it by the last layer's 9*nc x 64 projection matrix with MFMA, writing only the projected per-pixel vectors. This avoids writing and re-reading the full 64-channel 64x64 decoder activation and removes a separate pixel_proj launch. Separately, the hoisted skip half of a concat conv3 now uses the Winograd path when applicable. Risks include the extra LDS and register pressure from the projection weights, and split-K being disabled for this variant.

```diff
diff --git a/dvg_amd/_lib.py b/dvg_amd/_lib.py
--- a/dvg_amd/_lib.py
+++ b/dvg_amd/_lib.py
@@ -34,6 +34,7 @@
     "dvg_conv3x3_first_pair": (_i, [_p, _p, _p, _p, _p, _p, _p, _p, _p, _i, _i, _i, _i, _i, _f, _i, _p]),
     "dvg_conv4x4s2_bn_act_v2": (_i, [_p, _p, _p, _p, _p, _p, _i, _i, _i, _i, _i, _i, _f, _p, _l, _p]),
     "dvg_convT4x4s2_bn_act_v2": (_i, [_p, _p, _p, _p, _p, _p, _p, _i, _i, _i, _i, _i, _i, _i, _f, _p, _l, _p, _p, _i, _p]),
+    "dvg_convT4x4s2_bn_act_proj": (_i, [_p, _p, _p, _p, _p, _p, _i, _i, _i, _i, _i, _i, _i, _f, _p, _p, _i, _p]),
     "dvg_winograd_weight": (_i, [_p, _p, _i, _i, _i, _p]),
     "dvg_winograd_input": (_i, [_p, _p, _i, _i, _i, _i, _i, _i, _p]),
     "dvg_gemm_batched_k16": (_i, [_p, _p, _p, _i, _i, _i, _i, _i, _p]),
diff --git a/dvg_amd/csrc/conv_igemm2.hip b/dvg_amd/csrc/conv_igemm2.hip
--- a/dvg_amd/csrc/conv_igemm2.hip
+++ b/dvg_amd/csrc/conv_igemm2.hip
@@ -45,6 +45,9 @@
     const float* first_shift;
     float first_slope;
     int y_from;
+    const float* proj_w;
+    float* proj_out;
+    int proj_T;
 };
 
 __device__ __forceinline__ int addend_image(const int* __restrict__ add_map, int add_B, int n) {
@@ -56,10 +59,11 @@
 
 __device__ __attribute__((aligned(16))) float dvg_zero_slot[4] = {0.f, 0.f, 0.f, 0.f};
 
-template <int MODE, int TI, int TH, int TW, int NT_ = 1, bool FIRST_ = false>
+template <int MODE, int TI, int TH, int TW, int NT_ = 1, bool FIRST_ = false, bool PROJ_ = false>
 struct Cfg2 {
     static constexpr int NT = NT_;
     static constexpr bool FIRST = FIRST_;
+    static constexpr bool PROJ = PROJ_;
     static constexpr bool GEMM = MODE == M2_GEMM;
     static constexpr int S = (MODE == M2_CONV4S2) ? 2 : 1;
     static constexpr bool PAR4 = MODE == M2_CONV4S2;
@@ -98,13 +102,15 @@
     static constexpr int FP_W = HW + 2, FP_FLOATS = (HH + 2) * FP_W, FIRST_FLOATS = FIRST ? FP_FLOATS : 0;
     static_assert(!FIRST || (MODE == M2_CONV3 && TI == 1 && NT == 1), "FIRST: 3x3 mode, one image per tile");
     static constexpr int LDS_BYTES = (A_FLOATS + B_FLOATS + FIRST_FLOATS) * 4;
-    static constexpr bool CAN_SPLIT = !FIRST && !GEMM && TW != 16;
+    static constexpr bool CAN_SPLIT = !FIRST && !GEMM && TW != 16 && !PROJ;
     static_assert(BM == 64 || BM == 128 || BM == 256, "BM");
+    static_assert(!PROJ || (MODE == M2_CONVT4S2 && TI == 1 && NT == 1 && !FIRST && BM * 64 <= A_FLOATS + B_FLOATS),
+                  "PROJ: transposed-conv mode, one image per tile, the staged tile fits the stage buffers");
 };
 
-template <int MODE, int TI, int TH, int TW, int NT = 1, bool FIRST = false>
+template <int MODE, int TI, int TH, int TW, int NT = 1, bool FIRST = false, bool PROJ = false>
 __global__ __launch_bounds__(256, (MODE == M2_GEMM && TW == 8) ? DVG_GEMM_WGS_PER_CU : ((MODE == M2_GEMM && NT == 1) ? DVG_GEMM128_WGS : 2)) void conv_igemm2_kernel(const Igemm2Params p) {
-    using C = Cfg2<MODE, TI, TH, TW, NT, FIRST>;
+    using C = Cfg2<MODE, TI, TH, TW, NT, FIRST, PROJ>;
     constexpr int S = C::S, HH = C::HH, HW = C::HW, HP = C::HP, LD = C::LD, MT = C::MT, GT = C::GT, NG = C::NG,
                   BN = C::BN, NLA = C::NLA, NLA1 = C::NLA1, LDB = C::LDB, NP = C::NP, PSTEP = C::PSTEP, NLB = C::NLB;
     constexpr bool GEMM = C::GEMM, X3 = C::X3;
@@ -597,6 +603,24 @@
         return v;
     };
     const int hrow = hh * 4 * C::PK;
+    [[maybe_unused]] float* const Ps = smem;
+    [[maybe_unused]] constexpr int PNT = 3;
+    [[maybe_unused]] const int i16 = lane & 15, kq = lane >> 4;
+    [[maybe_unused]] f32x4 pw[PROJ ? PNT : 1][PROJ ? 4 : 1];
+    constexpr bool PW_EARLY = TW == 16;
+    auto load_pw = [&]() {
+        if constexpr (PROJ) {
+#pragma unroll
+            for (int nt = 0; nt < PNT; ++nt)
+#pragma unroll
+                for (int j = 0; j < 4; ++j)
+                    pw[nt][j] = *reinterpret_cast<const f32x4*>(p.proj_w + min(nt * 16 + i16, p.proj_T - 1) * 64 + 16 * j + 4 * kq);
+        }
+    };
+    if constexpr (PROJ) {
+        if (PW_EARLY) load_pw();
+        __syncthreads();
+    }
     auto epilogue = [&](auto act_c) {
         constexpr int ACT = decltype(act_c)::value;
 #pragma unroll
@@ -641,7 +665,8 @@
                     int oy, ox;
                     if (MODE == M2_CONVT4S2) { oy = 2 * (y0 + ty) + py; ox = 2 * (x0 + tx) + px; }
                     else { oy = y0 + ty; ox = x0 + tx; }
-                    if (!FIRST || want_y) yb[((tii * Ho + oy) * Wo + ox) * p.Cout] = o;
+                    if constexpr (PROJ) Ps[m * 64 + ((((wn * 32 + l31) >> 2) ^ (m & 15)) << 2) + (l31 & 3)] = o;
+                    else if (!FIRST || want_y) yb[((tii * Ho + oy) * Wo + ox) * p.Cout] = o;
                 }
             }
             if (MODE == M2_CONV3 && (TW == 16 || TW == 8)) {
@@ -666,6 +691,42 @@
     if (p.act == DVG_ACT_LRELU) epilogue(std::integral_constant<int, DVG_ACT_LRELU>{});
     else if (p.act == DVG_ACT_NONE) epilogue(std::integral_constant<int, DVG_ACT_NONE>{});
     else epilogue(std::integral_constant<int, -1>{});
+    if constexpr (PROJ) {
+        if (!PW_EARLY) load_pw();
+        __syncthreads();
+        const int T = p.proj_T;
+#pragma unroll
+        for (int it = 0; it < C::BM / 64; ++it) {
+            const int tile = wave + 4 * it;
+            const float* const prow = Ps + (tile * 16 + i16) * 64;
+            f32x4 a[4];
+#pragma unroll
+            for (int j = 0; j < 4; ++j) a[j] = *reinterpret_cast<const f32x4*>(prow + (((4 * j + kq) ^ i16) << 2));
+            const int m0 = tile * 16 + 4 * kq;
+            long orow[4];
+#pragma unroll
+            for (int r = 0; r < 4; ++r) {
+                const int oy = 2 * (y0 + (m0 + r) / TW) + py, ox = 2 * (x0 + (m0 + r) % TW) + px;
+                orow[r] = (((long)n0 * Ho + oy) * Wo + ox) * T;
+            }
+#pragma unroll
+            for (int nt = 0; nt < PNT; ++nt) {
+                if (nt * 16 >= T) break;
+                f32x4 d = {0.f, 0.f, 0.f, 0.f};
+#pragma unroll
+                for (int j = 0; j < 4; ++j)
+#pragma unroll
+                    for (int e = 0; e < 4; ++e) d = __builtin_amdgcn_mfma_f32_16x16x4f32(a[j][e], pw[nt][j][e], d, 0, 0, 0);
+                const int col = nt * 16 + i16;
+                if (col < T) {
+#pragma unroll
+                    for (int r = 0; r < 4; ++r) p.proj_out[orow[r] + col] = d[r];
+                }
+            }
+        }
+        clk_exit();
+        return;
+    }
     if (p.stats != nullptr) {
         float* red = smem;
         s1 += __shfl_xor(s1, 32);
@@ -806,9 +867,9 @@
     return s < 2 ? 1 : (int)s;
 }
 
-template <int MODE, int TI, int TH, int TW, int NT = 1, bool FIRST = false>
+template <int MODE, int TI, int TH, int TW, int NT = 1, bool FIRST = false, bool PROJ = false>
 static int launch2(Igemm2Params p, int Hg, int Wg, float* ws, long ws_floats, hipStream_t stream) {
-    using C = Cfg2<MODE, TI, TH, TW, NT, FIRST>;
+    using C = Cfg2<MODE, TI, TH, TW, NT, FIRST, PROJ>;
     if (Hg % TH || Wg % TW || p.Cout % C::BN) return fail(DVG_ERR_SHAPE, "conv_igemm2: tile does not divide shape");
     p.tiles_y = Hg / TH;
     p.tiles_x = Wg / TW;
@@ -862,12 +923,12 @@
     p.stage_prio = (MODE == M2_CONV3 || grid <= 3 * 256) ? 1 : 0;
     static bool attr_set = false;
     if (!attr_set) {
-        hipError_t e = hipFuncSetAttribute(reinterpret_cast<const void*>(&conv_igemm2_kernel<MODE, TI, TH, TW, NT, FIRST>),
+        hipError_t e = hipFuncSetAttribute(reinterpret_cast<const void*>(&conv_igemm2_kernel<MODE, TI, TH, TW, NT, FIRST, PROJ>),
                                            hipFuncAttributeMaxDynamicSharedMemorySize, C::LDS_BYTES);
         if (e != hipSuccess) return fail(DVG_ERR_HIP, "hipFuncSetAttribute: %s", hipGetErrorString(e));
         attr_set = true;
     }
-    hipLaunchKernelGGL((conv_igemm2_kernel<MODE, TI, TH, TW, NT, FIRST>), dim3(grid), dim3(256), C::LDS_BYTES, stream, p);
+    hipLaunchKernelGGL((conv_igemm2_kernel<MODE, TI, TH, TW, NT, FIRST, PROJ>), dim3(grid), dim3(256), C::LDS_BYTES, stream, p);
     if (int e = check_launch("conv_igemm2")) return e;
     if (S > 1) {
         const bool pool = y_pool != nullptr;
@@ -1085,6 +1146,35 @@
     return fail(DVG_ERR_SHAPE, "dvg_convT4x4s2_bn_act_v2: no kernel");
 }
 
+extern "C" int dvg_convT4x4s2_bn_act_proj(const float* x, const float* w_k16, const float* scale, const float* shift,
+                                          const float* proj_w, float* proj_out, int T, int N, int H, int W, int C1, int Cout,
+                                          int act, float slope, const float* addend, const int* addend_map, int addend_block,
+                                          void* stream) {
+    const char* who = "dvg_convT4x4s2_bn_act_proj";
+    DVG_REQUIRE(x && w_k16 && proj_w && proj_out, DVG_ERR_NULL, "%s: x / w / proj_w / proj_out must not be NULL", who);
+    DVG_REQUIRE(N > 0 && H > 0 && W > 0, DVG_ERR_SHAPE, "%s: empty shape", who);
+    DVG_REQUIRE(C1 > 0 && C1 % 16 == 0, DVG_ERR_SHAPE, "%s: C1=%d must be a multiple of 16", who, C1);
+    DVG_REQUIRE(Cout == 64, DVG_ERR_SHAPE, "%s: Cout=%d must be 64 (one column block holds every channel of a pixel)", who, Cout);
+    DVG_REQUIRE(T >= 1 && T <= 48, DVG_ERR_SHAPE, "%s: T=%d must be in 1..48", who, T);
+    DVG_REQUIRE(aligned16(x) && aligned16(w_k16) && aligned16(proj_w) && aligned16(addend), DVG_ERR_ALIGN,
+                "%s: pointers must be 16-byte aligned", who);
+    DVG_REQUIRE(act >= DVG_ACT_NONE && act <= DVG_ACT_SIGMOID, DVG_ERR_SHAPE, "%s: bad act", who);
+    Igemm2Params p{x, nullptr, w_k16, scale, shift, nullptr, nullptr, nullptr, N, H, W, C1, 0, Cout, 0, act, slope, 0, 0, 0, 0, 0,
+                   1, 0, nullptr};
+    p.addend = addend;
+    p.add_map = addend ? addend_map : nullptr;
+    p.add_B = addend_block;
+    DVG_REQUIRE(p.add_map == nullptr || (addend_block > 0 && N % addend_block == 0), DVG_ERR_SHAPE, "%s: addend_block must divide N", who);
+    p.proj_w = proj_w;
+    p.proj_out = proj_out;
+    p.proj_T = T;
+    int ti, th, tw;
+    DVG_REQUIRE(tile2(M2_CONVT4S2, N, H, W, Cout, &ti, &th, &tw) == 0 && ti == 1, DVG_ERR_SHAPE,
+                "%s: unsupported map %dx%d (multiples of 8 needed)", who, H, W);
+    if (tw == 16) return launch2<M2_CONVT4S2, 1, 8, 16, 1, false, true>(p, H, W, nullptr, 0, (hipStream_t)stream);
+    return launch2<M2_CONVT4S2, 1, 8, 8, 1, false, true>(p, H, W, nullptr, 0, (hipStream_t)stream);
+}
+
 extern "C" int dvg_gemm_batched_k16(const float* x, const float* w_k16, float* y, int NB, int H, int W, int Cin, int Cout,
                                     void* stream) {
     Igemm2Params p{x, nullptr, w_k16, nullptr, nullptr, y, nullptr, nullptr, NB, H, W, Cin, 0, Cout, 0, DVG_ACT_NONE, 0.f,
diff --git a/dvg_amd/fused.py b/dvg_amd/fused.py
--- a/dvg_amd/fused.py
+++ b/dvg_amd/fused.py
@@ -123,7 +123,12 @@
     return weight if blk.mode is None else weights.packed(weight, bool(blk.finish[0]), lo, hi, blk.cat)
 
 
-def _skip_half(kind, skip, ps):
+def _skip_half(kind, skip, ps, conv=None):
+    if kind == "conv3" and conv is not None and not conv.training and not torch.is_grad_enabled():
+        n, c, h, w = skip.shape
+        ctot = conv.weight.shape[1]
+        if winograd_tile(n, c, h, w, conv.weight.shape[0]) == 4:
+            return ops.conv3x3_winograd(skip, weights.winograd(conv.weight, 4, ctot - c, ctot), None, None, act=ACT_NONE)
     return BLOCKS[kind].raw(skip, None, ps, None)
 
 
@@ -233,6 +238,7 @@
 
 SKIP_HOIST = os.environ.get("DVG_SKIP_HOIST", "1") != "0"
 UPCONV_AS_CONVT = os.environ.get("DVG_UPCONV_AS_CONVT", "1") != "0"
+LAST_PROJ_FUSED = True
 _skip_seen = {}
 
 
@@ -268,7 +274,7 @@
     if not SKIP_HOIST or skip is None:
         return
     ctot = conv.weight.shape[BLOCKS[kind].cat]
-    s = _skip_half(kind, skip, block_weight(kind, conv.weight, ctot - skip.shape[1], ctot))
+    s = _skip_half(kind, skip, block_weight(kind, conv.weight, ctot - skip.shape[1], ctot), conv)
     _skip_seen[(id(conv), id(skip))] = [weakref.ref(skip), skip._version, _ver(conv.weight), 1, s]
 
 
@@ -361,13 +367,22 @@
     return _bn_act_train(bn, u, st, act=act, slope=slope, pool=pool)
 
 
+def _last_proj_applies(next_last, conv, x) -> bool:
+    if not LAST_PROJ_FUSED or next_last is None or torch.is_grad_enabled() or not isinstance(next_last, nn.ConvTranspose2d):
+        return False
+    w = next_last.weight
+    return (conv.weight.shape[0] == 64 and w.shape[0] == 64 and tuple(w.shape[2:]) == (3, 3) and 9 * w.shape[1] <= ops.PROJ_MAX_T
+            and tuple(next_last.stride) == (1, 1) and tuple(next_last.padding) == (1, 1) and x.shape[2] % 8 == 0
+            and x.shape[3] % 8 == 0)
+
+
 def conv3_bn_act(conv, bn, x, skip=None, *, upsample=False, pool=False, act=ACT_LRELU, slope=0.2, next_conv=None, y_from=0,
-                 next_up=None):
+                 next_up=None, next_last=None):
     if y_from and (not pool or bn.training or _needs_grad(x, skip, conv.weight, bn.weight)):
         raise RuntimeError("conv3_bn_act: y_from is an eval-mode, no-grad option of the pooled form")
     if isinstance(x, ops.WinoV) and x.up:
         hs = None if (bn.training or not upsample or pool) else \
-            _hoisted_skip(conv, x, skip, functools.partial(_skip_half, "conv3", skip), force=True)
+            _hoisted_skip(conv, x, skip, functools.partial(_skip_half, "conv3", skip, conv=conv), force=True)
         if hs is None:
             raise RuntimeError("conv3_bn_act: an upsampled WinoV needs the eval-mode concat conv with its skip half hoisted")
         sc, sh = folded_affine(conv, bn)
@@ -392,7 +407,7 @@
     if not bn.training:
         sc, sh = folded_affine(conv, bn)
         if not pool:
-            hs = _hoisted_skip(conv, x, skip, functools.partial(_skip_half, "conv3", skip))
+            hs = _hoisted_skip(conv, x, skip, functools.partial(_skip_half, "conv3", skip, conv=conv))
             if hs is not None:
                 if upsample and UPCONV_WINOGRAD:
                     n_, c1_, hx_, wx_ = x.shape
@@ -402,6 +417,12 @@
                         return ops.conv3x3_winograd(x, weights.winograd(conv.weight, 4, 0, c1_), sc, sh, act=act, slope=slope,
                                                     upsample=True, addend=hs[1], to_v=to_v)
                 if upsample and UPCONV_AS_CONVT:
+                    if _last_proj_applies(next_last, conv, x):
+                        w_last = next_last.weight
+                        d = ops.convT4x4s2_proj(x, weights.k4_packed(conv.weight, x.shape[1]), sc, sh,
+                                                ops._last_wmat_cached(w_last, 0, 64, 9 * w_last.shape[1]), act=act, slope=slope,
+                                                addend=hs[1])
+                        return ops.LastProj(d, (x.shape[0], 64, 2 * x.shape[2], 2 * x.shape[3]), w_last)
                     return ops.convT4x4s2(x, None, weights.k4_packed(conv.weight, x.shape[1]), sc, sh, act=act, slope=slope,
                                           addend=hs[1])
                 return ops.conv3x3(x, None, hs[0], sc, sh, upsample=upsample, act=act, slope=slope, addend=hs[1])
@@ -524,6 +545,8 @@
 
 
 def convT3_last(conv, x, *, act=ACT_SIGMOID):
+    if isinstance(x, ops.LastProj):
+        return ops.convT_last_two_step(x, None, conv.weight, _bias(conv), conv.weight.shape[1], 3, act=act)
     if _needs_grad(x, conv.weight):
         from .autograd import last_layer_autograd
         return last_layer_autograd("convT3", conv, x, None, act=act)
diff --git a/dvg_amd/models/backbones.py b/dvg_amd/models/backbones.py
--- a/dvg_amd/models/backbones.py
+++ b/dvg_amd/models/backbones.py
@@ -172,8 +172,9 @@
                         fl = getattr(self, f"upc{s + 1}")[0]
                         nup = (fl.main[0], fl.main[1], sks[s + 1])
                     if first:
+                        nlast = mods[li + 1] if li + 1 < len(mods) and isinstance(mods[li + 1], nn.ConvTranspose2d) else None
                         d = fused.conv3_bn_act(layer.main[0], layer.main[1], d, sk, upsample=True,
-                                               next_conv=None if nxt is None else nxt.main[0], next_up=nup)
+                                               next_conv=None if nxt is None else nxt.main[0], next_up=nup, next_last=nlast)
                         first = False
                     else:
                         d = fused.conv3_bn_act(layer.main[0], layer.main[1], d,
diff --git a/dvg_amd/ops/__init__.py b/dvg_amd/ops/__init__.py
--- a/dvg_amd/ops/__init__.py
+++ b/dvg_amd/ops/__init__.py
@@ -6,6 +6,7 @@
     pack_conv_weight, pack_convT_weight, packed_row_floats, pack_igemm_weight, _wp_dims, unpack_conv_weight,
     unpack_convT_weight, _splitk_ws, _SPLITK_WS, evict_captured_workspaces, _stats_buf, _tile_images, SharedBlocks,
     _MAP_CACHE, shared_map, group_sum, _check_addend, conv3x3, CONV4S2_MAX_FLOATS, conv4x4s2, convT4x4s2,
+    PROJ_MAX_T, convT4x4s2_proj,
 )
 from .winograd import (
     winograd_weight, winograd_ok, WinoV, winograd_chain_ok, winograd_up_chain_ok, winograd_pool_chain_ok,
@@ -14,7 +15,7 @@
 from .edge import (
     conv3x3_first, first_pair_ok, conv3x3_first_pair, convT3x3_last, conv4x4s2_first, convT4x4s2_last, pixel_proj,
     _SKIP_PROJ_CACHE, clear_skip_proj_cache, _cached_skip_proj, _last_wmat, _last_wmat_cached,
-    precompute_skip_proj, convT_last_two_step, eval_frames, eval_frames_finn, pairwise_frame_mse, moving_mnist_compose, clip_gather, clip_gather_aug, CLIP_MAX_SHIFT,
+    precompute_skip_proj, LastProj, convT_last_two_step, eval_frames, eval_frames_finn, pairwise_frame_mse, moving_mnist_compose, clip_gather, clip_gather_aug, CLIP_MAX_SHIFT,
     mnist_scale_u8, moving_mnist_compose_u8, frame_mosaic, QUANT_TRUNC, QUANT_NEAREST,
     MOSAIC_BLACK, MOSAIC_RED, MOSAIC_GREEN, MOSAIC_SEL_NONE, MOSAIC_SEL_BEST, MOSAIC_SEL_PICK, MOSAIC_CELL_INTS,
 )
diff --git a/dvg_amd/ops/conv.py b/dvg_amd/ops/conv.py
--- a/dvg_amd/ops/conv.py
+++ b/dvg_amd/ops/conv.py
@@ -262,3 +262,37 @@
          _p(y), _p(st), n, h, w, c1, c2, cout, act, slope, _p(ws), 0 if ws is None else ws.numel(), _p(addend),
          _p(amap), ablk, _stream())
     return (y, st) if stats else y
+
+
+PROJ_MAX_T = 48
+
+
+def convT4x4s2_proj(x, wp, scale, shift, wm, *, act=ACT_LRELU, slope=0.2, addend=None):
+    _dev_f32(x, "convT4x4s2_proj.x")
+    _dev_f32(wm, "convT4x4s2_proj.wm")
+    assert is_nhwc(x)
+    n, c1, h, w = x.shape
+    taps, cout, cin = _wp_dims(wp)
+    if taps != 16 or cin != c1:
+        raise RuntimeError(f"convT4x4s2_proj: packed weight {tuple(wp.shape)} does not match Cin={c1}")
+    t = wm.shape[0]
+    if cout != 64 or tuple(wm.shape) != (t, 64) or not wm.is_contiguous() or not 1 <= t <= PROJ_MAX_T or h % 8 or w % 8:
+        raise RuntimeError(f"convT4x4s2_proj: needs Cout = 64, wm (T <= {PROJ_MAX_T}, 64) and a map of multiples of 8; got Cout="
+                           f"{cout}, wm {tuple(wm.shape)}, x {tuple(x.shape)}")
+    amap, ablk = None, 0
+    if addend is not None:
+        if isinstance(addend, SharedBlocks):
+            if n != addend.groups * addend.block:
+                raise RuntimeError("convT4x4s2_proj: shared addend does not match the batch")
+            amap, ablk, addend = addend.map_dev, addend.block, addend.t
+        elif addend.shape[0] != n:
+            raise RuntimeError("convT4x4s2_proj: addend does not match the batch")
+        _dev_f32(addend, "convT4x4s2_proj.addend")
+        if tuple(addend.shape[1:]) != (64, 2 * h, 2 * w) or not is_nhwc(addend):
+            raise RuntimeError(f"convT4x4s2_proj: addend {tuple(addend.shape)} must be NHWC (.,64,{2 * h},{2 * w})")
+    d = torch.empty((n * 4 * h * w, t), device=x.device, dtype=torch.float32)
+    fl = 2.0 * n * h * w * cout * 16 * cin + 2.0 * n * 4 * h * w * cout * t
+    by = 4.0 * (x.numel() + wp.numel() + wm.numel() + (n * 4 * h * w * cout if addend is not None else 0) + d.numel())
+    _run("convT4x4s2_igemm", fl, by, lib().dvg_convT4x4s2_bn_act_proj, _p(x), _p(wp), _p(scale), _p(shift), _p(wm), _p(d), t,
+         n, h, w, c1, cout, act, slope, _p(addend), _p(amap), ablk, _stream())
+    return d
diff --git a/dvg_amd/ops/edge.py b/dvg_amd/ops/edge.py
--- a/dvg_amd/ops/edge.py
+++ b/dvg_amd/ops/edge.py
@@ -144,12 +144,24 @@
     _cached_skip_proj(skip, lambda: _last_wmat_cached(w, c1, wdet.shape[0], t), w)
 
 
+class LastProj:
+
+    def __init__(self, d, shape, w):
+        self.d, self.shape, self.w = d, tuple(shape), w
+
+
 def convT_last_two_step(x, skip, w, bias, nc, ks, *, act):
-    assert is_nhwc(x)
-    n, c1, h, wd = x.shape
     wdet = w.detach()
     t = ks * ks * nc
-    d1 = pixel_proj(x, _last_wmat_cached(w, 0, c1, t))
+    if isinstance(x, LastProj):
+        if x.w is not w or tuple(x.d.shape) != (x.shape[0] * x.shape[2] * x.shape[3], t):
+            raise RuntimeError("convT_last_two_step: the projection handed over was made for another last layer")
+        n, c1, h, wd = x.shape
+        d1 = x.d
+    else:
+        assert is_nhwc(x)
+        n, c1, h, wd = x.shape
+        d1 = pixel_proj(x, _last_wmat_cached(w, 0, c1, t))
     d2 = None
     d2_map, d2_blk = None, 0
     if isinstance(skip, SharedBlocks):
@@ -160,7 +172,7 @@
     elif skip is not None:
         d2 = _cached_skip_proj(skip, lambda: _last_wmat_cached(w, c1, wdet.shape[0], t), w)
     s = 2 if ks == 4 else 1
-    y = torch.empty((n, nc, s * h, s * wd), device=x.device, dtype=torch.float32)
+    y = torch.empty((n, nc, s * h, s * wd), device=d1.device, dtype=torch.float32)
     _run("convT_gather", 0.0, 4.0 * (d1.numel() * (2 if skip is not None else 1) + y.numel()), lib().dvg_convT_gather,
          _p(d1), _p(d2), _p(bias), _p(y), ks, n, h, wd, nc, act, _p(d2_map), d2_blk, _stream())
     return y
diff --git a/include/dvg_hip.h b/include/dvg_hip.h
--- a/include/dvg_hip.h
+++ b/include/dvg_hip.h
@@ -55,11 +55,11 @@
 int dvg_conv4x4s2_bn_act_v2(const float* x, const float* w_k16, const float* scale, const float* shift, float* y, float* stats,
                             int N, int H, int W, int Cin, int Cout, int act, float slope, float* workspace, long workspace_floats,
                             void* stream);
-int dvg_convT4x4s2_bn_act_v2(const float* x, const float* skip, const float* w_k16,
-                             const float* scale, const float* shift, float* y, float* stats,
-                             int N, int H, int W, int C1, int C2, int Cout, int act, float slope,
-                             float* workspace, long workspace_floats, const float* addend,
-                             const int* addend_map , int addend_block, void* stream);
+int dvg_convT4x4s2_bn_act_v2(const float* x, const float* skip, const float* w_k16, const float* scale, const float* shift, float* y,
+                             float* stats, int N, int H, int W, int C1, int C2, int Cout, int act, float slope, float* workspace,
+                             long workspace_floats, const float* addend, const int* addend_map , int addend_block, void* stream);
+int dvg_convT4x4s2_bn_act_proj(const float* x, const float* w_k16, const float* scale, const float* shift, const float* proj_w, float* proj_out, int T,
+                               int N, int H, int W, int C1, int Cout, int act, float slope, const float* addend, const int* addend_map, int addend_block, void* stream);
 
 int dvg_winograd_weight(const float* w_oihw, float* u_k16, int cout, int cin, int m, void* stream);
 int dvg_winograd_input(const float* x, float* v, int N, int H, int W, int C, int m, int upsample, void* stream);
```

Measured after the change: 52540 frames/s (median of 6 runs). 1.02x the previous value.
